# KumarRobotics/top_down_renderer

Hardware: AMD Instinct MI355X
Metric: particle-updates/sec (render+score+resample) (higher is better)
Workload: dtype f32

## Files before the change

include/tdr.h:

```cpp
#ifndef TDR_H_
#define TDR_H_

#include <stddef.h>
#include <stdint.h>

#ifdef __cplusplus
extern "C" {
#endif

#define TDR_OK 0
#define TDR_ERR_ARG (-1)
#define TDR_ERR_HIP (-2)
#define TDR_ERR_NOMEM (-3)

#define TDR_MAX_CLASSES 15
#define TDR_ST_FIELDS 7
enum { TDR_ST_INIT_X = 0, TDR_ST_INIT_Y = 1, TDR_ST_DX = 2, TDR_ST_DY = 3, TDR_ST_THETA = 4, TDR_ST_SCALE = 5,
       TDR_ST_HAVE_INIT = 6 };

typedef struct tdr_state {
  float init_x_px, init_y_px, dx_m, dy_m, theta, scale;
  uint8_t have_init;
  uint8_t pad_[3];
} tdr_state;
// ... 106 lines not shown
                          const int32_t* perm, float uniform_scale, int init_search, float* raw_w, float* workspace,
                          void* stream);

size_t tdr_score_cart_workspace_floats(int ncls, int rows, int cols, int64_t n, int64_t n_total);
int tdr_k_score_cart(const tdr_map_desc* map, const float* scan_pk, int rows, int cols, float res,
                     const tdr_filter_params* fp, float* st, int64_t cap, int64_t n, int64_t n_total,
                     const int32_t* perm, float* raw_w, float* workspace, void* stream);
size_t tdr_score_cart_init_workspace_floats(int ncls, int rows, int cols, int64_t n, int64_t n_total);
int tdr_k_score_cart_init(const tdr_map_desc* map, const float* scan_pk, int rows, int cols, float res,
                          const tdr_filter_params* fp, float* st, int64_t cap, int64_t n, int64_t n_total,
                          float* workspace, void* stream);

int tdr_k_propagate(float* st, int64_t cap, int64_t n, float* last_dist, float tx, float ty, float omega,
                    int scale_freeze, float pos_cov, float theta_cov, const float* z4, uint64_t seed, uint64_t step,
                    int64_t index_base, void* stream);
void* tdr_rng_create(uint32_t seed);
void tdr_rng_destroy(void* rng);
float tdr_rng_uniform_host(void* rng);
int tdr_propagate_normals_host(void* rng, int64_t n, int scale_freeze, float* z4_out);
#define TDR_RNG_STATE_WORDS 640
size_t tdr_rng_dev_workspace_bytes(int64_t n);
int tdr_k_rng_propagate_normals(uint32_t* state, int64_t n, int64_t lo, int64_t hi, int scale_freeze, float* z4_out,
                                void* workspace, void* stream);
int tdr_k_rng_uniform(uint32_t* state, float* out_dev, void* stream);
int tdr_rng_get_state_host(void* rng, uint32_t* words);
int tdr_rng_set_state_host(void* rng, const uint32_t* words);
typedef struct tdr_rng_pipe tdr_rng_pipe;
int tdr_rng_pipe_create(int64_t n_max, tdr_rng_pipe** out);
void tdr_rng_pipe_destroy(tdr_rng_pipe* p);
int tdr_rng_pipe_on_device(const tdr_rng_pipe* p);
int tdr_rng_pipe_from_host(tdr_rng_pipe* p, void* host_rng, void* stream);
int tdr_rng_pipe_to_host(tdr_rng_pipe* p, void* host_rng, void* stream);
int tdr_rng_pipe_normals(tdr_rng_pipe* p, int64_t n, int64_t lo, int64_t hi, int scale_freeze, const float** z4_out,
                         void* stream);
int tdr_rng_pipe_uniform(tdr_rng_pipe* p, const float** shift_out, void* stream);
int tdr_init_particle_host(void* rng, const float* class_maps, int ncls, int rows, int cols, float resolution,
                           const tdr_filter_params* fp, tdr_state* out);
int tdr_init_particles_host(void* rng, const float* class_maps, int ncls, int rows, int cols, float resolution,
                            const tdr_filter_params* fp, int max_num, tdr_state* out, int64_t* n_out);
int64_t tdr_init_particles_count(const tdr_filter_params* fp, int max_num);
size_t tdr_init_workspace_bytes(void);
int tdr_k_init_particles(uint32_t* rng_state_dev, const tdr_map_desc* map, const tdr_filter_params* fp, int max_num,
                         int64_t lo, int64_t hi, float* st, int64_t cap, int64_t* n_out, void* workspace, void* stream);
int tdr_rng_pipe_init_particles(tdr_rng_pipe* p, const tdr_map_desc* map, const tdr_filter_params* fp, int max_num,
                                int64_t lo, int64_t hi, float* st, int64_t cap, int64_t* n_out, void* workspace,
                                void* stream);

#define TDR_UW_INFO_FLOATS 65536
int tdr_k_update_weights(const float* raw_w, const float* last_dist, int64_t n, float* w_out, float* info_out,
                         void* stream);

int tdr_config_prefix_small(int on);
int64_t tdr_prefix_workspace_bytes(int64_t n);
int tdr_k_prefix(const float* w, int64_t n, float* runmax_out, void* workspace, void* stream);
int tdr_k_prefix_mode(const float* w, int64_t n, int mode, float* runmax_out, float* prefix_out, void* workspace,
                      void* stream);
int tdr_k_resample(const float* runmax, int64_t n, int64_t n_new, float shift, int64_t i_begin, int64_t i_end,
                   int32_t* idx_out, void* stream);
int tdr_k_resample_dev(const float* runmax, int64_t n, int64_t n_new, const float* shift_dev, int64_t i_begin, int64_t i_end,
                       int32_t* idx_out, void* stream);
int tdr_k_gather_states(const float* src, int64_t src_cap, int64_t src_shard, const int32_t* idx, int64_t n_new,
                        float* dst, int64_t dst_cap, void* stream);

int tdr_k_shard_pack2(const float* a, const float* b, int64_t nl, float* out, void* stream);
int tdr_k_shard_unpack2(const float* in, int world, int64_t nl, float* a_glob, float* b_glob, void* stream);
int tdr_k_unshard_states(const float* in, int world, int64_t nl, float* st, int64_t cap, void* stream);

int tdr_k_local_map_polar(const tdr_map_desc* map, const float* tab, int nb, int nr, float cx, float cy, float scale,
                          float res, float* dists_out, uint8_t* mask_out, void* stream);
int tdr_k_local_map_cart(const tdr_map_desc* map, int rows, int cols, float cx, float cy, float rot, float res,
                         float* dists_out, uint8_t* mask_out, void* stream);

int tdr_k_active_diffs(const tdr_map_desc* map, const float* tab, int nb, int nr, float res, const float* centres,
                       const int32_t* shifts, int K, int ncand, double* sums_out, void* stream);
int tdr_active_candidates_host(const float* preds, int K, int nb, float* centres, float* dists, float* thetas,
                               int32_t* shifts, int* ntheta_out, int* ndist_out);

#define TDR_MEAN_COV_FLOATS 4800
int tdr_k_mean_cov(const float* st, int64_t cap, int64_t n, const float* about, float* out, void* stream);
int tdr_k_set_scale(float* st, int64_t cap, int64_t n, const float* scale_dev, void* stream);
int tdr_k_save_ml_state(const float* info, const float* st, int64_t cap, int64_t src_shard, int64_t n, float* out12,
                        void* stream);
int tdr_k_shift_init(float* st, int64_t cap, int64_t n, float dx, float dy, void* stream);

int tdr_config_compact(int on);
int tdr_config_shift_uniform(int mode);
float tdr_config_shift_uniform_span(float cells);
int tdr_config_ray_split(int k);
int tdr_config_cart_skip(int on);
int tdr_config_init_mfma(int on);
int tdr_config_uw_waves(int on);
int64_t tdr_shift_uniform_launches(void);

int tdr_profile_enable(int on);
int tdr_profile_score_ms(double* total_ms, int64_t* launches);
int tdr_profile_shares(double* dense_ms, double* scattered_ms, int64_t* scattered_particles);
int tdr_profile_variants(int64_t out[16]);

int64_t tdr_config_tuning(const char* name, int64_t value);
int tdr_su_tail_plan(int nchunks, int k, int q, int row, int* group, int* s0, int* s1);
size_t tdr_k_su_order_workspace_ints(int64_t n, int nb);
int64_t tdr_k_su_order_slots(int64_t n, int nb);
int tdr_k_su_order(const float* st, int64_t cap, int64_t n, const int32_t* perm, int nb, float span, int32_t* workspace,
                   int32_t* slots_out, int32_t* keys_out, int32_t* counts_out, int* bucket_out, void* stream);
int tdr_selftest_score(void);
int tdr_k_selftest_round(const float* x, int64_t n, float limit, int32_t* out, void* stream);
int tdr_libm_variant(void);
int tdr_libm_force_variant(int variant);
int tdr_sincosf_host(const float* x, int64_t n, int variant, float* sin_out, float* cos_out);
int tdr_k_selftest_sincos(const float* x, int64_t n, float* sin_out, float* cos_out, void* stream);
int tdr_logf_host(const float* x, int64_t n, float* out);
int tdr_k_selftest_logf(const float* x, int64_t n, float* out, void* stream);
int tdr_k_selftest_atan2(const float* y, const float* x, int64_t n, float* out, void* stream);

int tdr_k_states_aos_to_soa(const tdr_state* aos, int64_t n, float* st, int64_t cap, void* stream);
int tdr_k_states_soa_to_aos(const float* st, int64_t cap, int64_t n, tdr_state* aos, void* stream);
size_t tdr_locality_tmp_ints(int64_t n, int map_rows, int map_cols);
int tdr_k_locality_order(const float* st, int64_t cap, int64_t n, int map_rows, int map_cols, int32_t* perm_out,
                         int32_t* keys_tmp, void* stream);
size_t tdr_locality_pose_tmp_ints(int64_t n);
int tdr_k_locality_order_pose(const float* st, int64_t cap, int64_t n, int map_rows, int map_cols, float theta_radius,
                              int32_t* perm_out, int32_t* keys_tmp, void* stream);

typedef struct tdr_map tdr_map;
typedef struct tdr_renderer tdr_renderer;
typedef struct tdr_filter tdr_filter;

int tdr_map_create(tdr_map** out);
void tdr_map_destroy(tdr_map* m);
int tdr_map_set(tdr_map* m, const float* class_maps, const uint8_t* class_mask, int ncls, int rows, int cols,
                float resolution, int center_x, int center_y);
int tdr_map_set_labels(tdr_map* m, const uint8_t* label_img, int img_h, int img_w, const int32_t* flatten_lut,
                       int lut_size, int ncls, float resolution, int center_x, int center_y);
int tdr_map_update_labels_incremental(tdr_map* m, const uint8_t* label_img, int img_h, int img_w,
                                      const int32_t* flatten_lut, int lut_size, int ncls, float resolution, int center_x,
                                      int center_y, int64_t* changed_cells);
int tdr_map_patch_labels(tdr_map* m, const uint8_t* patch, int y0, int x0, int h, int w, int center_x, int center_y,
                         int64_t* changed_cells);
int tdr_map_get_desc(const tdr_map* m, tdr_map_desc* out);
int tdr_map_sample_pts_polar(tdr_map* m, int nb, int nr, float ang_res);
int tdr_map_polar_shape(const tdr_map* m, int* nb, int* nr);
int tdr_map_set_window(tdr_map* m, int rows, int cols);
int tdr_map_window_shape(const tdr_map* m, int* rows, int* cols);
int tdr_map_info(const tdr_map* m, int* ncls, int* rows, int* cols, float* resolution, int* have_map);
int tdr_map_center(const tdr_map* m, int* center_x, int* center_y);
int tdr_map_local_map(tdr_map* m, int polar, float cx, float cy, float scale_or_rot, float res, int rows, int cols,
                      float* dists_out, uint8_t* mask_out);
int tdr_map_classes_at_point(const tdr_map* m, int px, int py, uint32_t* class_bits);
int tdr_map_best_rel_pos(tdr_map* m, const float* preds, int K, float best_rel_pos[2], float* best_diff);
int tdr_map_local_geo_map(tdr_map* m, int polar, float cx, float cy, float scale_or_rot, float res, int rows, int cols,
                          float* dists_out);
int tdr_map_load_cache(tdr_map* m, const char* cache_dir, const char* map_path, int num_classes, float resolution,
                       int center_x, int center_y, int* loaded);
int tdr_map_save_cache(tdr_map* m, const char* cache_dir, const char* map_path);
int tdr_map_save_rasters(tdr_map* m, const char* dir);
int tdr_png_read_gray8_host(const char* path, uint8_t* px_out, int64_t capacity, int* w, int* h);
int tdr_png_write_gray8_host(const char* path, const uint8_t* px, int w, int h);
int tdr_map_load_rasters(tdr_map* m, const char* dir, int num_classes, float resolution, int center_x, int center_y);
#define TDR_SVG_NO_KEY 0xFFFFFFFFu
int tdr_svg_parse_host(const char* path, float size_out[2], int64_t* n_poly, int64_t* n_vert, uint32_t* keys_out,
                       int64_t* offsets_out, float* verts_out);
int tdr_map_load_polygons(tdr_map* m, const float* verts, const int64_t* poly_offsets, const int32_t* poly_class,
                          int64_t n_poly, int width, int height, int num_classes, const int32_t* exclusive, int n_excl,
                          float resolution, int center_x, int center_y, uint8_t* planes_out);
int tdr_polygon_planes(const float* verts, const int64_t* poly_offsets, const int32_t* poly_class, int64_t n_poly,
                       int width, int height, int num_classes, const int32_t* exclusive, int n_excl, float resolution,
// ... 153 lines not shown
```

top_down_renderer_amd/_lib.py:

```python
import ctypes as C
import os

_PKG = os.path.dirname(os.path.abspath(__file__))
SO_PATH = os.environ.get("TDR_LIB_PATH") or os.path.join(_PKG, "libtdr_hip.so")

TDR_ST_FIELDS = 7
TDR_MAX_CLASSES = 15
TDR_SVG_NO_KEY = 0xFFFFFFFF


class FilterParamsC(C.Structure):
    _fields_ = [
        ("pos_cov", C.c_float), ("theta_cov", C.c_float), ("regularization", C.c_float),
        ("init_pos_px_x", C.c_float), ("init_pos_px_y", C.c_float), ("init_pos_px_cov", C.c_float),
        ("init_pos_m_x", C.c_float), ("init_pos_m_y", C.c_float),
        ("init_pos_deg_theta", C.c_float), ("init_pos_deg_cov", C.c_float),
        ("force_on_map", C.c_int32),
        ("fixed_scale", C.c_float), ("scale_log_min", C.c_float), ("scale_log_max", C.c_float),
        ("num_classes", C.c_int32),
        ("class_weights", C.c_float * 16),
    ]


class MapDescC(C.Structure):
# ... 99 lines not shown
    "tdr_score_workspace_floats": (C.c_size_t, [_i, _i, _i, _i64, _i64]),
    "tdr_k_score_polar": (_i, [C.POINTER(MapDescC), _vp, _vp, _i, _i, _f, C.POINTER(FilterParamsC), _vp, _i64, _i64,
                               _i64, _vp, _f, _i, _vp, _vp, _vp]),
    "tdr_k_active_diffs": (_i, [C.POINTER(MapDescC), _vp, _i, _i, _f, _vp, _vp, _i, _i, _vp, _vp]),
    "tdr_active_candidates_host": (_i, [_vp, _i, _i, _vp, _vp, _vp, _vp, C.POINTER(_i), C.POINTER(_i)]),
    "tdr_logf_host": (_i, [_vp, _i64, _vp]),
    "tdr_k_selftest_logf": (_i, [_vp, _i64, _vp, _vp]),
    "tdr_rng_pipe_create": (_i, [_i64, C.POINTER(_vp)]),
    "tdr_rng_pipe_destroy": (None, [_vp]),
    "tdr_rng_pipe_on_device": (_i, [_vp]),
    "tdr_rng_pipe_from_host": (_i, [_vp, _vp, _vp]),
    "tdr_rng_pipe_to_host": (_i, [_vp, _vp, _vp]),
    "tdr_rng_pipe_normals": (_i, [_vp, _i64, _i64, _i64, _i, C.POINTER(_vp), _vp]),
    "tdr_rng_pipe_uniform": (_i, [_vp, C.POINTER(_vp), _vp]),
    "tdr_rng_dev_workspace_bytes": (C.c_size_t, [_i64]),
    "tdr_k_rng_propagate_normals": (_i, [_vp, _i64, _i64, _i64, _i, _vp, _vp, _vp]),
    "tdr_k_rng_uniform": (_i, [_vp, _vp, _vp]),
    "tdr_rng_get_state_host": (_i, [_vp, _vp]),
    "tdr_rng_set_state_host": (_i, [_vp, _vp]),
    "tdr_k_resample_dev": (_i, [_vp, _i64, _i64, _vp, _i64, _i64, _vp, _vp]),
    "tdr_score_ctx_create": (_i, [C.POINTER(_vp)]),
    "tdr_score_ctx_destroy": (None, [_vp]),
    "tdr_score_ctx_span": (C.c_float, [_vp]),
    "tdr_score_ctx_trial_calls": (_i64, [_vp]),
    "tdr_config_tuning": (_i64, [C.c_char_p, _i64]),
    "tdr_su_tail_plan": (_i, [_i, _i, _i, _i, C.POINTER(_i), C.POINTER(_i), C.POINTER(_i)]),
    "tdr_k_su_order_workspace_ints": (C.c_size_t, [_i64, _i]),
    "tdr_k_su_order_slots": (_i64, [_i64, _i]),
    "tdr_k_su_order": (_i, [_vp, _i64, _i64, _vp, _i, _f, _vp, _vp, _vp, _vp, C.POINTER(_i), _vp]),
    "tdr_selftest_score": (_i, []),
    "tdr_profile_variants": (_i, [C.POINTER(_i64)]),
    "tdr_score_ctx_set_polar_factors": (_i, [_vp, _vp, _i, _i]),
    "tdr_polar_factors_host": (_i, [_i, _i, _f, _f, _vp]),
    "tdr_k_score_polar_ctx": (_i, [C.POINTER(MapDescC), _vp, _vp, _i, _i, _f, C.POINTER(FilterParamsC), _vp, _i64, _i64,
                                   _i64, _vp, _f, _i, _vp, _vp, _vp, _vp]),
    "tdr_score_geo_workspace_floats": (C.c_size_t, [_i, _i, _i, _i64, _i64]),
    "tdr_k_score_polar_geo": (_i, [C.POINTER(MapDescC), C.POINTER(MapDescC), _vp, _vp, _vp, _f, _f, _i, _i, _f,
                                   C.POINTER(FilterParamsC), _vp, _i64, _i64, _i64, _vp, _f, _i, _vp, _vp, _vp]),
    "tdr_score_cart_workspace_floats": (C.c_size_t, [_i, _i, _i, _i64, _i64]),
    "tdr_k_score_cart": (_i, [C.POINTER(MapDescC), _vp, _i, _i, _f, C.POINTER(FilterParamsC), _vp, _i64, _i64, _i64,
                              _vp, _vp, _vp, _vp]),
    "tdr_score_cart_init_workspace_floats": (C.c_size_t, [_i, _i, _i, _i64, _i64]),
    "tdr_k_score_cart_init": (_i, [C.POINTER(MapDescC), _vp, _i, _i, _f, C.POINTER(FilterParamsC), _vp, _i64, _i64, _i64,
                                   _vp, _vp]),
    "tdr_k_propagate": (_i, [_vp, _i64, _i64, _vp, _f, _f, _f, _i, _f, _f, _vp, _u64, _u64, _i64, _vp]),
    "tdr_rng_create": (_vp, [_u32]),
    "tdr_rng_destroy": (None, [_vp]),
    "tdr_rng_uniform_host": (_f, [_vp]),
    "tdr_propagate_normals_host": (_i, [_vp, _i64, _i, _vp]),
    "tdr_k_update_weights": (_i, [_vp, _vp, _i64, _vp, _vp, _vp]),
    "tdr_prefix_workspace_bytes": (_i64, [_i64]),
    "tdr_k_prefix": (_i, [_vp, _i64, _vp, _vp, _vp]),
    "tdr_k_prefix_mode": (_i, [_vp, _i64, _i, _vp, _vp, _vp, _vp]),
    "tdr_k_resample": (_i, [_vp, _i64, _i64, _f, _i64, _i64, _vp, _vp]),
    "tdr_k_gather_states": (_i, [_vp, _i64, _i64, _vp, _i64, _vp, _i64, _vp]),
    "tdr_init_particles_host": (_i, [_vp, _vp, _i, _i, _i, _f, C.POINTER(FilterParamsC), _i, _vp, C.POINTER(C.c_int64)]),
    "tdr_init_particles_count": (_i64, [C.POINTER(FilterParamsC), _i]),
    "tdr_init_workspace_bytes": (C.c_size_t, []),
    "tdr_k_init_particles": (_i, [_vp, C.POINTER(MapDescC), C.POINTER(FilterParamsC), _i, _i64, _i64, _vp, _i64,
                                  C.POINTER(C.c_int64), _vp, _vp]),
    "tdr_rng_pipe_init_particles": (_i, [_vp, C.POINTER(MapDescC), C.POINTER(FilterParamsC), _i, _i64, _i64, _vp, _i64,
                                         C.POINTER(C.c_int64), _vp, _vp]),
    "tdr_k_mean_cov": (_i, [_vp, _i64, _i64, _vp, _vp, _vp]),
    "tdr_k_sample_ml_states": (_i, [_vp, _i64, _i64, _i, _vp, _vp]),
    "tdr_gmm_fit_host": (_i, [_vp, _i, _i, _i, _vp, _vp, _vp, _vp]),
    "tdr_gmm_select_host": (_i, [_vp, _i, _i64, _vp, _i, _vp, _vp]),
    "tdr_adaptive_count_host": (_i64, [_vp, _i, _i64, _i64]),
    "tdr_filter_compute_gmm": (_i, [_vp]),
    "tdr_filter_get_gmm": (_i, [_vp, _i, _vp, _vp, _vp]),
    "tdr_filter_adaptive_count": (_i64, [_vp]),
    "tdr_filter_step_count": (_i64, [_vp]),
    "tdr_filter_num_gaussians": (_i, [_vp]),
    "tdr_filter_set_num_gaussians": (_i, [_vp, _i]),
    "tdr_gmm_workspace_bytes": (C.c_size_t, [_i, _i]),
    "tdr_gmm_out_doubles": (_i, [_i]),
    "tdr_k_gmm_samples": (_i, [_vp, _i, _vp, _vp]),
    "tdr_k_gmm_fit": (_i, [_vp, _i, _i, _i, _vp, _vp, _vp]),
    "tdr_k_gmm_fit_jobs": (_i, [_vp, _i, _vp]),
    "tdr_k_gmm_pick": (_i, [_vp, _i, _vp]),
    "tdr_gmm_candidates_host": (_i, [_i, _i64, _i, _i, _vp]),
    "tdr_filter_compute_gmm_device": (_i, [_vp]),
    "tdr_batch_compute_gmm": (_i, [_vp, _i, _vp]),
    "tdr_k_save_ml_state": (_i, [_vp, _vp, _i64, _i64, _i64, _vp, _vp]),
    "tdr_k_shard_pack2": (_i, [_vp, _vp, _i64, _vp, _vp]),
    "tdr_k_shard_unpack2": (_i, [_vp, _i, _i64, _vp, _vp, _vp]),
    "tdr_k_unshard_states": (_i, [_vp, _i, _i64, _vp, _i64, _vp]),
    "tdr_comm_rccl_unique_id": (_i, [_vp]),
    "tdr_comm_create_rccl": (_i, [_i, _i, _vp, C.POINTER(_vp)]),
    "tdr_comm_create": (_i, [_i, _i, _vp, C.POINTER(_vp)]),
    "tdr_comm_destroy": (None, [_vp]),
    "tdr_comm_world": (_i, [_vp]),
    "tdr_comm_rank": (_i, [_vp]),
    "tdr_comm_all_gather": (_i, [_vp, _vp, _vp, C.c_size_t, _vp]),
    "tdr_comm_broadcast": (_i, [_vp, _vp, C.c_size_t, _i, _vp]),
    "tdr_filter_create_sharded": (_i, [_vp, _i, C.POINTER(FilterParamsC), _u32, _vp, C.POINTER(_vp)]),
    "tdr_filter_num_local": (_i64, [_vp]),
    "tdr_k_set_scale": (_i, [_vp, _i64, _i64, _vp, _vp]),
    "tdr_k_shift_init": (_i, [_vp, _i64, _i64, _f, _f, _vp]),
    "tdr_k_states_aos_to_soa": (_i, [_vp, _i64, _vp, _i64, _vp]),
    "tdr_k_states_soa_to_aos": (_i, [_vp, _i64, _i64, _vp, _vp]),
    "tdr_profile_enable": (_i, [_i]),
    "tdr_profile_score_ms": (_i, [C.POINTER(C.c_double), C.POINTER(C.c_int64)]),
    "tdr_profile_shares": (_i, [C.POINTER(C.c_double), C.POINTER(C.c_double), C.POINTER(C.c_int64)]),
    "tdr_map_create": (_i, [C.POINTER(_vp)]),
    "tdr_map_destroy": (None, [_vp]),
    "tdr_map_set": (_i, [_vp, _vp, _vp, _i, _i, _i, _f, _i, _i]),
    "tdr_map_set_labels": (_i, [_vp, _vp, _i, _i, _vp, _i, _i, _f, _i, _i]),
    "tdr_filter_update_map_labels": (_i, [_vp, _vp, _i, _i, _vp, _i, _i, _f, _i, _i]),
    "tdr_map_update_labels_incremental": (_i, [_vp, _vp, _i, _i, _vp, _i, _i, _f, _i, _i, C.POINTER(_i64)]),
    "tdr_map_patch_labels": (_i, [_vp, _vp, _i, _i, _i, _i, _i, _i, C.POINTER(_i64)]),
    "tdr_map_get_desc": (_i, [_vp, C.POINTER(MapDescC)]),
    "tdr_filter_update_map_labels_incremental": (_i, [_vp, _vp, _i, _i, _vp, _i, _i, _f, _i, _i, C.POINTER(_i64)]),
    "tdr_filter_patch_map_labels": (_i, [_vp, _vp, _i, _i, _i, _i, _i, _i, C.POINTER(_i64)]),
    "tdr_map_sample_pts_polar": (_i, [_vp, _i, _i, _f]),
    "tdr_map_polar_shape": (_i, [_vp, C.POINTER(_i), C.POINTER(_i)]),
    "tdr_map_set_window": (_i, [_vp, _i, _i]),
    "tdr_map_window_shape": (_i, [_vp, C.POINTER(_i), C.POINTER(_i)]),
    "tdr_map_info": (_i, [_vp, C.POINTER(_i), C.POINTER(_i), C.POINTER(_i), C.POINTER(_f), C.POINTER(_i)]),
    "tdr_map_center": (_i, [_vp, _vp, _vp]),
    "tdr_map_local_map": (_i, [_vp, _i, _f, _f, _f, _f, _i, _i, _vp, _vp]),
    "tdr_k_local_map_polar": (_i, [_vp, _vp, _i, _i, _f, _f, _f, _f, _vp, _vp, _vp]),
    "tdr_k_local_map_cart": (_i, [_vp, _i, _i, _f, _f, _f, _f, _vp, _vp, _vp]),
    "tdr_map_local_geo_map": (_i, [_vp, _i, _f, _f, _f, _f, _i, _i, _vp]),
    "tdr_map_load_cache": (_i, [_vp, C.c_char_p, C.c_char_p, _i, _f, _i, _i, C.POINTER(_i)]),
    "tdr_map_save_cache": (_i, [_vp, C.c_char_p, C.c_char_p]),
    "tdr_k_geo_map_from_map": (_i, [C.POINTER(MapDescC), _i, _vp, _vp, _vp]),
    "tdr_map_classes_at_point": (_i, [_vp, _i, _i, C.POINTER(_u32)]),
    "tdr_map_best_rel_pos": (_i, [_vp, _vp, _i, _vp, _vp]),
    "tdr_renderer_create": (_i, [_vp, C.POINTER(_vp)]),
    "tdr_renderer_destroy": (None, [_vp]),
    "tdr_renderer_render": (_i, [_vp, _i, _vp, _i, _i, _i64, _f, _f, _i, _i, _i, _vp]),
    "tdr_renderer_render_geo": (_i, [_vp, _i, _vp, _i, _i64, _i64, _f, _f, _i, _i, _vp]),
    "tdr_filter_create": (_i, [_vp, _i, C.POINTER(FilterParamsC), _u32, C.POINTER(_vp)]),
    "tdr_filter_create_cart": (_i, [_vp, _i, C.POINTER(FilterParamsC), _u32, C.POINTER(_vp)]),
    "tdr_filter_destroy": (None, [_vp]),
    "tdr_filter_configure": (_i, [_vp, _i, _i]),
    "tdr_filter_initialize_particles": (_i, [_vp]),
    "tdr_filter_set_states": (_i, [_vp, _vp, _i64]),
    "tdr_filter_get_states": (_i, [_vp, _vp, _i64]),
    "tdr_filter_propagate": (_i, [_vp, _f, _f, _f]),
    "tdr_filter_update": (_i, [_vp, _vp, _vp, _f, _i64]),
    "tdr_filter_update_geo": (_i, [_vp, _vp, _vp, _f, _i64]),
    "tdr_filter_compute_weights": (_i, [_vp, _vp, _vp, _f]),
    "tdr_filter_get_raw_weights": (_i, [_vp, _vp, _i64]),
    "tdr_filter_get_last_dist": (_i, [_vp, _vp, _i64]),
    "tdr_filter_propagate_freeze": (_i, [_vp, _f, _f, _f, _i]),
    "tdr_filter_init_one": (_i, [_vp]),
    "tdr_filter_share_rng": (_i, [_vp, _vp]),
    "tdr_init_particle_host": (_i, [_vp, _vp, _i, _i, _i, _f, _vp, _vp]),
    "tdr_filter_get_weights": (_i, [_vp, _vp, _i64]),
    "tdr_filter_get_resample_indices": (_i, [_vp, _vp, _i64]),
    "tdr_filter_mean_cov": (_i, [_vp, _i, _vp, _vp]),
    "tdr_filter_freeze_scale": (_i, [_vp]),
    "tdr_filter_is_scale_frozen": (_i, [_vp]),
    "tdr_filter_scale": (_f, [_vp]),
    "tdr_filter_num_particles": (_i64, [_vp]),
    "tdr_filter_update_map": (_i, [_vp, _vp, _vp, _i, _i, _i, _f, _i, _i]),
    "tdr_batch_step": (_i, [_vp, _i, _vp, _vp]),
    "tdr_batch_last_stats": (_i, [_vp, _vp]),
    "tdr_batch_render_polar": (_i, [_vp, _i, _vp, _f, _i, _i, _i, _vp]),
    "tdr_renderer_get_render": (_i, [_vp, _vp, _vp]),
    "tdr_batch_pose": (_i, [_vp, _i, _vp, _vp]),
    "tdr_viz_plane_words": (C.c_size_t, [_i, _i]),
    "tdr_viz_arrow_host": (_i, [_i, _i, _vp]),
    "tdr_viz_overlay_host": (_i, [_vp, _vp, _i, _vp, _vp, _i, _i, _vp, _i, C.POINTER(_i)]),
    "tdr_k_viz_particles": (_i, [_vp, _i64, _i64, _i, _i, _vp, _vp]),
# ... 39 lines not shown
```

top_down_renderer_amd/csrc/tdr_batch_loop.hip:

```cpp
#include "tdr_common.h"
#include "tdr_raster_dev.h"
#include "tdr_filter_dev.h"
#include "tdr_batch.h"

__global__ __launch_bounds__(256) void batch_raster_keys_kernel(const TdrBatchRasterEntry* __restrict__ tab, int k,
                                                                TdrBatchRasterShape a) {
  const TdrBatchRasterEntry& e = tab[batch_find(k, (int)blockIdx.x, [&](int i) { return tab[i].blk_keys; })];
  const int64_t q = (int64_t)(blockIdx.x - e.blk_keys) * blockDim.x + threadIdx.x;
  if (q >= e.n) return;
  e.keys[q] = raster_key(e.pts, e.stride, e.ioff, q, 1, e.res, a.ang_res, e.lut, a.ncls, a.rows, a.cols);
}

__global__ __launch_bounds__(1024) void batch_raster_kernel(const TdrBatchRasterEntry* __restrict__ tab,
                                                            TdrBatchRasterShape a) {
  extern __shared__ unsigned int cnt[];
  const TdrBatchRasterEntry& e = tab[blockIdx.y];
  const int col0 = blockIdx.x * a.cpt;
  const int ncol = min(a.cpt, a.cols - col0);
  raster_tile_clear(cnt, ncol * a.ncls * a.rows);
  __syncthreads();
  raster_tile_count_keys(cnt, e.keys, e.n, col0, ncol, a.ncls, a.rows);
  __syncthreads();
  raster_tile_write(cnt, col0, ncol, a.ncls, a.rows, a.cols, a.rf, e.img, e.pk);
}

bool tdr_batch_raster_shape(int ncls, int rows, int cols, float ang_res, TdrBatchRasterShape* out) {
  RasterShape sh;
  if (ncls < 1 || ncls > TDR_MAX_CLASSES || rows < 1 || cols < 1 || !raster_shape(ncls, rows, cols, &sh) || !sh.keyed)
    return false;
  TdrBatchRasterShape a;
  a.ang_res = ang_res; a.ncls = ncls; a.rows = rows; a.cols = cols; a.rf = tdr_rec_floats(ncls); a.cpt = sh.cpt;
  *out = a;
  return true;
}

int tdr_batch_raster(const TdrBatchRasterEntry* tab, int k, int blocks_keys, const TdrBatchRasterShape& a, hipStream_t s) {
  if (!tab || k < 1 || blocks_keys < 0) return fail(TDR_ERR_ARG, "batch_raster: bad arguments");
  const size_t lds = (size_t)a.cpt * a.ncls * a.rows * 4;
  static bool attr_set[64] = {false};
  HIP_TRY(raster_allow_lds(reinterpret_cast<const void*>(batch_raster_kernel), lds, attr_set));
  if (blocks_keys > 0)
    hipLaunchKernelGGL(batch_raster_keys_kernel, dim3((unsigned)blocks_keys), dim3(256), 0, s, tab, k, a);
  hipLaunchKernelGGL(batch_raster_kernel, dim3((unsigned)cdiv(a.cols, a.cpt), (unsigned)k), dim3(1024), lds, s, tab, a);
  LAUNCH_CHECK("batch_raster");
  return TDR_OK;
}

static_assert(TDR_BATCH_MC_SINGLE_MAX_N == MC_SINGLE_MAX_N, "the batch splits small / big filters where tdr_k_mean_cov does");

__global__ __launch_bounds__(1024) void batch_mean_cov_kernel(const TdrBatchPoseEntry* __restrict__ tab, int libm_fma) {
  const TdrBatchPoseEntry& e = tab[blockIdx.x];
  mean_cov_body(e.st, e.cap, e.n, nullptr, e.out, libm_fma);
  if (threadIdx.x == 0) e.out[24] = e.st[TDR_ST_SCALE * e.cap];
}
__global__ __launch_bounds__(MC_THREADS) void batch_mc_sums_kernel(const TdrBatchPoseEntry* __restrict__ tab, int libm_fma) {
  const TdrBatchPoseEntry& e = tab[blockIdx.y];
  mc_sums_body(e.st, e.cap, e.n, reinterpret_cast<McScratch*>(e.scratch), libm_fma);
}
__global__ __launch_bounds__(MC_THREADS) void batch_mc_cov_kernel(const TdrBatchPoseEntry* __restrict__ tab) {
  const TdrBatchPoseEntry& e = tab[blockIdx.y];
  mc_cov_body(e.st, e.cap, e.n, nullptr, reinterpret_cast<McScratch*>(e.scratch));
}
__global__ __launch_bounds__(MC_THREADS) void batch_mc_final_kernel(const TdrBatchPoseEntry* __restrict__ tab) {
  const TdrBatchPoseEntry& e = tab[blockIdx.x];
  mc_final_body(e.n, nullptr, reinterpret_cast<const McScratch*>(e.scratch), e.out);
  if (threadIdx.x == 0) e.out[24] = e.st[TDR_ST_SCALE * e.cap];
}

int tdr_batch_pose_launch(const TdrBatchPoseEntry* small, int k_small, const TdrBatchPoseEntry* big, int k_big,
                          hipStream_t s) {
  if (k_small < 0 || k_big < 0 || (k_small && !small) || (k_big && !big)) return fail(TDR_ERR_ARG, "batch_pose: bad arguments");
  const int fma = tdr_libm_fma();
  if (k_small > 0)
    hipLaunchKernelGGL(batch_mean_cov_kernel, dim3((unsigned)k_small), dim3(1024), 0, s, small, fma);
  if (k_big > 0) {
    hipLaunchKernelGGL(batch_mc_sums_kernel, dim3(MC_WGS, (unsigned)k_big), dim3(MC_THREADS), 0, s, big, fma);
    hipLaunchKernelGGL(batch_mc_cov_kernel, dim3(MC_WGS, (unsigned)k_big), dim3(MC_THREADS), 0, s, big);
    hipLaunchKernelGGL(batch_mc_final_kernel, dim3((unsigned)k_big), dim3(MC_THREADS), 0, s, big);
  }
  LAUNCH_CHECK("batch_pose");
  return TDR_OK;
}
```

top_down_renderer_amd/csrc/tdr_common.h:

```cpp
#ifndef TDR_COMMON_H_
#define TDR_COMMON_H_
#include <hip/hip_runtime.h>

#include <cmath>
#include <cstdarg>
#include <cstdint>
#include <cstdio>
#include <cstdlib>
#include <cstring>
#include <limits>
#include <type_traits>
#include <utility>
#include <vector>

#include "tdr.h"
#include "tdr_config.h"

#ifndef TDR_SCORE_U
#define TDR_SCORE_U 4
#endif
#ifndef TDR_INIT_SCAN_LDS
#define TDR_INIT_SCAN_LDS 1
#endif
#ifndef TDR_XCD_SWIZZLE
#define TDR_XCD_SWIZZLE 0
#endif
#ifndef TDR_OOB_ALIAS
#define TDR_OOB_ALIAS 1
#endif

int tdr_fail(int code, const char* fmt, ...);
#define fail tdr_fail
#define HIP_TRY(expr)                                                                       \
  do {                                                                                      \
    hipError_t e_ = (expr);                                                                 \
    if (e_ != hipSuccess) return fail(TDR_ERR_HIP, "%s: %s", #expr, hipGetErrorString(e_)); \
  } while (0)
#define LAUNCH_CHECK(name)                                                                   \
  do {                                                                                       \
    hipError_t e_ = hipGetLastError();                                                       \
    if (e_ != hipSuccess) return fail(TDR_ERR_HIP, "launch %s: %s", name, hipGetErrorString(e_)); \
  } while (0)

int tdr_libm_fma();

static inline int64_t cdiv(int64_t a, int64_t b) { return (a + b - 1) / b; }

template <class F>
static inline int with_flags(F&& f) { return f(); }
template <class F, class... Rest>
static inline int with_flags(F&& f, bool b, Rest... rest) {
  auto next = [&](auto B) { return with_flags([&](auto... bs) { return f(B, bs...); }, rest...); };
  return b ? next(std::true_type{}) : next(std::false_type{});
}
template <class F>
static inline int with_nv4(int rf, const char* who, F&& f) {
  switch (rf / 4) {
    case 1: return f(std::integral_constant<int, 1>{});
    case 2: return f(std::integral_constant<int, 2>{});
    case 3: return f(std::integral_constant<int, 3>{});
    case 4: return f(std::integral_constant<int, 4>{});
    default: return fail(TDR_ERR_ARG, "%s: unsupported record size %d", who, rf);
  }
}

#define PFX_HEAD 2048
#define INI_TILE 2048
#define INI_MAX_TILES 2048
int tdr_chain_total(const float* raw, const float* mean_dev, int kind, int64_t n, float* total_out, void* workspace,
                    hipStream_t st);
int tdr_uw_small(const float* raw, const float* last_dist, int64_t n, float* w, float* info, hipStream_t st);
int tdr_mt_raw_stream(const uint32_t* state, int64_t nblocks, uint32_t* raw, hipStream_t s);
int tdr_mt_advance(const uint32_t* raw, int64_t nblocks, const uint32_t* consumed, uint32_t* state, hipStream_t s);
bool tdr_score_polar_float_form(const tdr_map_desc* map, int nb, int nr, int64_t n, int64_t n_total);
__host__ __device__ inline bool tdr_has_kslot(int ncls, int rf) { return ncls + 2 <= rf; }
uint32_t* tdr_profile_stats_ptr();
#endif
```

top_down_renderer_amd/csrc/tdr_filter.hip:

```cpp
#include <random>

#include <rocprim/device/device_radix_sort.hpp>
using TdrSortConfig = rocprim::radix_sort_config<rocprim::default_config, rocprim::merge_sort_config<512, 512, 4>, rocprim::default_config>;

#include "tdr_common.h"
#include "tdr_filter_dev.h"

__device__ __forceinline__ uint32_t mulhi32(uint32_t a, uint32_t b) { return __umulhi(a, b); }
__device__ void philox4x32_10(uint32_t c[4], uint32_t k0, uint32_t k1) {
#pragma unroll
  for (int r = 0; r < 10; r++) {
    uint32_t hi0 = mulhi32(0xD2511F53u, c[0]), lo0 = 0xD2511F53u * c[0];
    uint32_t hi1 = mulhi32(0xCD9E8D57u, c[2]), lo1 = 0xCD9E8D57u * c[2];
    uint32_t n0 = hi1 ^ c[1] ^ k0, n1 = lo1, n2 = hi0 ^ c[3] ^ k1, n3 = lo0;
    c[0] = n0; c[1] = n1; c[2] = n2; c[3] = n3;
    k0 += 0x9E3779B9u; k1 += 0xBB67AE85u;
  }
}

__global__ void propagate_kernel(float* __restrict__ st, int64_t cap, int64_t n, float* __restrict__ last_dist,
                                 float tx, float ty, float omega, int scale_freeze, float pos_cov, float theta_cov,
                                 const float* __restrict__ z4, uint64_t seed, uint64_t step, int64_t index_base,
                                 int libm_fma) {
  const int64_t p = (int64_t)blockIdx.x * blockDim.x + threadIdx.x;
// ... 81 lines not shown
    st.theta = (float)((double)st.theta * (M_PI / 180));
    st.have_init = 1;
  } else {
    st.theta = 0;
    st.have_init = 0;
  }
  return st;
}
extern "C" int tdr_init_particle_host(void* rng, const float* class_maps, int ncls, int rows, int cols, float resolution,
                                      const tdr_filter_params* fp, tdr_state* out) {
  if (!rng || !class_maps || !fp || !out) return fail(TDR_ERR_ARG, "init_particle: bad arguments");
  if (ncls < 2) return fail(TDR_ERR_ARG, "init_particle: class 1 (road) is required for the on-road test");
  bool any_road = false;
  for (size_t k = 0; k < (size_t)rows * cols && !any_road; k++) any_road = class_maps[(size_t)rows * cols + k] < 1;
  if (!any_road) return fail(TDR_ERR_ARG, "init_particle: the map has no road cell, rejection sampling cannot end");
  *out = draw_particle(*(std::mt19937*)rng, class_maps, ncls, rows, cols, resolution, fp);
  return TDR_OK;
}
extern "C" int tdr_init_particles_host(void* rng, const float* class_maps, int ncls, int rows, int cols,
                                       float resolution, const tdr_filter_params* fp, int max_num, tdr_state* out,
                                       int64_t* n_out) {
  if (!rng || !class_maps || !fp || !out || !n_out || max_num < 0) return fail(TDR_ERR_ARG, "init_particles: bad arguments");
  if (ncls < 2) return fail(TDR_ERR_ARG, "init_particles: class 1 (road) is required for the on-road test");
  std::mt19937& gen = *(std::mt19937*)rng;
  bool any_road = false;
  for (size_t k = 0; k < (size_t)rows * cols && !any_road; k++) any_road = class_maps[(size_t)rows * cols + k] < 1;
  if (!any_road) return fail(TDR_ERR_ARG, "init_particles: the map has no road cell, rejection sampling cannot end");
  const size_t num_at_scale = (fp->fixed_scale < 0) ? 10 : 1;
  int64_t count = 0;
  for (int i = 0; i < (int)((size_t)max_num / num_at_scale); i++) {
    const tdr_state proto = draw_particle(gen, class_maps, ncls, rows, cols, resolution, fp);
    for (float scale = 0; scale < 1; scale += 1. / num_at_scale) {
      tdr_state part = draw_particle(gen, class_maps, ncls, rows, cols, resolution, fp);
      if (fp->fixed_scale < 0) {
        part = proto;
        part.scale = (float)std::pow(10., (double)scale);
      }
      if (count < max_num + 16) out[count] = part;
      count++;
      (void)draw_particle(gen, class_maps, ncls, rows, cols, resolution, fp);
    }
  }
  *n_out = count;
  return TDR_OK;
}

__device__ long long block_sum_ll(long long v, long long* sh) {
  const int lane = threadIdx.x & 63, wave = threadIdx.x >> 6;
  for (int o = 32; o > 0; o >>= 1) v += __shfl_down(v, o, 64);
  __syncthreads();
  if (lane == 0) sh[wave] = v;
  __syncthreads();
  long long t = 0;
  const int nw = blockDim.x >> 6;
  for (int w = 0; w < nw; w++) t += sh[w];
  return t;
}

#define UW_G 256
struct UwScratch {
  double a[UW_G];
  double b[UW_G];
};
__device__ __forceinline__ void uw_chunk(int64_t n, int64_t& lo, int64_t& hi) {
  const int64_t per = (n + UW_G - 1) / UW_G;
  lo = (int64_t)blockIdx.x * per;
  hi = lo + per < n ? lo + per : n;
  if (lo > n) lo = n;
}
__device__ double uw_total(const double* part) {
  __shared__ double stage[UW_G];
  __shared__ double result;
  __syncthreads();
  for (int g = threadIdx.x; g < UW_G; g += blockDim.x) stage[g] = part[g];
  __syncthreads();
  if (threadIdx.x == 0) {
    double t = 0;
    for (int g = 0; g < UW_G; g++) t += stage[g];
    result = t;
  }
  __syncthreads();
  return result;
}
__global__ __launch_bounds__(256) void uw_pass1(const float* __restrict__ raw, int64_t n, UwScratch* s1) {
  __shared__ double shd[4];
  __shared__ long long shl[4];
  int64_t lo, hi;
  uw_chunk(n, lo, hi);
  double s = 0;
  long long c = 0;
  for (int64_t i = lo + threadIdx.x; i < hi; i += 256) {
    const float v = raw[i];
    if (!isnan(v)) { s += (double)v; c++; }
  }
  const double ts = block_sum_d(s, shd);
  const long long tc = block_sum_ll(c, shl);
  if (threadIdx.x == 0) { s1->a[blockIdx.x] = ts; s1->b[blockIdx.x] = (double)tc; }
}
struct UwExact {
  float sum, mean, bsum, pad;
};
__global__ __launch_bounds__(256) void uw_pass2(const float* __restrict__ raw, int64_t n, const UwScratch* s1,
                                                UwScratch* s2, UwExact* ex) {
  __shared__ long long shl[4];
  const float mean = ex->sum / (float)(long long)uw_total(s1->b);
  int64_t lo, hi;
  uw_chunk(n, lo, hi);
  long long cu = 0;
  for (int64_t i = lo + threadIdx.x; i < hi; i += 256) {
    const float v = raw[i];
    if (!isnan(v) && v < mean) cu++;
  }
  const long long tc = block_sum_ll(cu, shl);
  if (threadIdx.x == 0) {
    s2->b[blockIdx.x] = (double)tc;
    if (blockIdx.x == 0) ex->mean = mean;
  }
}
__global__ __launch_bounds__(256) void uw_pass3(const float* __restrict__ raw, int64_t n, const UwExact* ex,
                                                const UwScratch* s2, UwScratch* s3, float* __restrict__ w) {
  __shared__ double shd[4];
  const float sum = ex->sum, mean = ex->mean;
  const long long num_under = (long long)uw_total(s2->b);
  const float bottom = sqrtf(ex->bsum / (float)num_under);
  const bool fallback = (sum == 0.f || num_under < 1);
  const float fill = mean - bottom;
  int64_t lo, hi;
  uw_chunk(n, lo, hi);
  double acc = 0;
  for (int64_t i = lo + threadIdx.x; i < hi; i += 256) {
    float v = raw[i];
    v = fallback ? 1.f : (isnan(v) ? fill : v);
    w[i] = v;
    acc += (double)v;
  }
  const double t = block_sum_d(acc, shd);
  if (threadIdx.x == 0) s3->a[blockIdx.x] = t;
}
__global__ __launch_bounds__(256) void uw_pass4(const float* __restrict__ last_dist, int64_t n, const UwScratch* s3,
                                                UwScratch* s4, float* __restrict__ w) {
  __shared__ double shd[4];
  const float fs1 = (float)uw_total(s3->a);
  const float fn = (float)n;
  int64_t lo, hi;
  uw_chunk(n, lo, hi);
  double acc = 0;
  for (int64_t i = lo + threadIdx.x; i < hi; i += 256) {
    float v = w[i] / fs1;
    const float d = fminf(last_dist[i] * 5.f, 1.f);
    v = d * v + (1.f - d) / fn;
    w[i] = v;
    acc += (double)v;
  }
  const double t = block_sum_d(acc, shd);
  if (threadIdx.x == 0) s4->a[blockIdx.x] = t;
}
__global__ __launch_bounds__(256) void uw_pass5(int64_t n, const UwScratch* s4, UwScratch* s5, float* __restrict__ w) {
  __shared__ float sb[4];
  __shared__ long long si[4];
  const float fs2 = (float)uw_total(s4->a);
  int64_t lo, hi;
  uw_chunk(n, lo, hi);
  float best = -INFINITY;
  long long besti = 0x7fffffffffffffffll;
  for (int64_t i = lo + threadIdx.x; i < hi; i += 256) {
    const float v = w[i] / fs2;
    w[i] = v;
    if (v > best || (v == best && i < besti)) { best = v; besti = i; }
  }
  for (int o = 32; o > 0; o >>= 1) {
    const float ob = __shfl_down(best, o, 64);
    const long long oi = __shfl_down(besti, o, 64);
    if (ob > best || (ob == best && oi < besti)) { best = ob; besti = oi; }
  }
  if ((threadIdx.x & 63) == 0) { sb[threadIdx.x >> 6] = best; si[threadIdx.x >> 6] = besti; }
  __syncthreads();
  if (threadIdx.x == 0) {
    for (int k = 1; k < 4; k++)
      if (sb[k] > best || (sb[k] == best && si[k] < besti)) { best = sb[k]; besti = si[k]; }
    s5->a[blockIdx.x] = (double)best;
    s5->b[blockIdx.x] = (double)besti;
  }
}
__global__ __launch_bounds__(256) void uw_pass6(int64_t n, const UwScratch* s1, const UwScratch* s2,
                                                const UwScratch* s5, const UwExact* ex, float* info) {
  static_assert(UW_G == 256, "one candidate per thread");
  __shared__ float sb[4];
  __shared__ long long si[4];
  float best = (float)s5->a[threadIdx.x];
  long long besti = (long long)s5->b[threadIdx.x];
  if (best != best) { best = -INFINITY; besti = 0x7fffffffffffffffll; }
  for (int o = 32; o > 0; o >>= 1) {
    const float ob = __shfl_down(best, o, 64);
    const long long oi = __shfl_down(besti, o, 64);
    if (ob > best || (ob == best && oi < besti)) { best = ob; besti = oi; }
  }
  if ((threadIdx.x & 63) == 0) { sb[threadIdx.x >> 6] = best; si[threadIdx.x >> 6] = besti; }
  const float sum = ex->sum, mean = ex->mean;
  const long long nv = (long long)uw_total(s1->b), nu = (long long)uw_total(s2->b);
  const float bottom = sqrtf(ex->bsum / (float)nu);
  if (threadIdx.x != 0) return;
  for (int k = 1; k < 4; k++)
    if (sb[k] > best || (sb[k] == best && si[k] < besti)) { best = sb[k]; besti = si[k]; }
  if (besti == 0x7fffffffffffffffll) besti = 0;
  info[0] = __int_as_float((int)besti);
  info[1] = sum; info[2] = mean; info[3] = bottom; info[4] = (sum == 0.f || nu < 1) ? 1.f : 0.f;
  info[5] = (float)nv; info[6] = (float)nu; info[7] = 0.f;
}

#define TDR_UW_SINGLE_MAX_N 32768
extern "C" int tdr_k_update_weights(const float* raw_w, const float* last_dist, int64_t n, float* w_out,
                                    float* info_out, void* stream) {
  if (!raw_w || !last_dist || !w_out || !info_out) return fail(TDR_ERR_ARG, "update_weights: null pointer");
  if (n < 1) return fail(TDR_ERR_ARG, "update_weights: n must be >= 1");
  hipStream_t s = (hipStream_t)stream;
  if (n <= TDR_UW_SINGLE_MAX_N) {
    const int rc = tdr_uw_small(raw_w, last_dist, n, w_out, info_out, s);
    if (rc) return rc;
    LAUNCH_CHECK("update_weights");
    return TDR_OK;
  }
  constexpr size_t kFixed = 8 * sizeof(float) + 64 + 5 * sizeof(UwScratch) + sizeof(UwExact) + 64;
  static_assert(kFixed + 32 * 1024 <= TDR_UW_INFO_FLOATS * sizeof(float), "info scratch");
  UwScratch* sc = reinterpret_cast<UwScratch*>(
      (reinterpret_cast<uintptr_t>(info_out + 8) + 63) & ~(uintptr_t)63);
  UwExact* ex = reinterpret_cast<UwExact*>(sc + 5);
  void* chain_ws = reinterpret_cast<void*>((reinterpret_cast<uintptr_t>(ex + 1) + 63) & ~(uintptr_t)63);
  const size_t chain_room = TDR_UW_INFO_FLOATS * sizeof(float) - kFixed;
  if ((size_t)tdr_prefix_workspace_bytes(n) > chain_room)
    return fail(TDR_ERR_ARG, "update_weights: n = %lld needs more than TDR_UW_INFO_FLOATS of scratch", (long long)n);
  hipLaunchKernelGGL(uw_pass1, dim3(UW_G), dim3(256), 0, s, raw_w, n, sc + 0);
  int rc = tdr_chain_total(raw_w, nullptr, 0, n, &ex->sum, chain_ws, s);
  if (rc) return rc;
  hipLaunchKernelGGL(uw_pass2, dim3(UW_G), dim3(256), 0, s, raw_w, n, (const UwScratch*)(sc + 0), sc + 1, ex);
  rc = tdr_chain_total(raw_w, &ex->mean, 1, n, &ex->bsum, chain_ws, s);
  if (rc) return rc;
  hipLaunchKernelGGL(uw_pass3, dim3(UW_G), dim3(256), 0, s, raw_w, n, (const UwExact*)ex, (const UwScratch*)(sc + 1),
                     sc + 2, w_out);
  hipLaunchKernelGGL(uw_pass4, dim3(UW_G), dim3(256), 0, s, last_dist, n, (const UwScratch*)(sc + 2), sc + 3, w_out);
  hipLaunchKernelGGL(uw_pass5, dim3(UW_G), dim3(256), 0, s, n, (const UwScratch*)(sc + 3), sc + 4, w_out);
  hipLaunchKernelGGL(uw_pass6, dim3(1), dim3(256), 0, s, n, (const UwScratch*)(sc + 0), (const UwScratch*)(sc + 1),
                     (const UwScratch*)(sc + 4), (const UwExact*)ex, info_out);
  LAUNCH_CHECK("update_weights(multi)");
  return TDR_OK;
}

__global__ void resample_kernel(const float* __restrict__ runmax, int64_t n, int64_t n_new, float shift,
                                int64_t i_begin, int64_t i_end, int32_t* __restrict__ idx) {
  const int64_t i = i_begin + (int64_t)blockIdx.x * blockDim.x + threadIdx.x;
  if (i >= i_end) return;
  idx[i - i_begin] = (int32_t)resample_pick(runmax, n, n_new, i, shift);
}

extern "C" int tdr_k_resample(const float* runmax, int64_t n, int64_t n_new, float shift, int64_t i_begin,
                              int64_t i_end, int32_t* idx_out, void* stream) {
  if (!runmax || !idx_out) return fail(TDR_ERR_ARG, "resample: null pointer");
  if (n < 1 || n_new < 1 || i_begin < 0 || i_end > n_new || i_begin > i_end)
    return fail(TDR_ERR_ARG, "resample: bad range");
  if (i_begin == i_end) return TDR_OK;
  hipLaunchKernelGGL(resample_kernel, dim3((unsigned)cdiv(i_end - i_begin, 256)), dim3(256), 0, (hipStream_t)stream,
                     runmax, n, n_new, shift, i_begin, i_end, idx_out);
  LAUNCH_CHECK("resample");
  return TDR_OK;
}

__global__ void resample_dev_kernel(const float* __restrict__ runmax, int64_t n, int64_t n_new, const float* __restrict__ shift_dev,
                                    int64_t i_begin, int64_t i_end, int32_t* __restrict__ idx) {
  const int64_t i = i_begin + (int64_t)blockIdx.x * blockDim.x + threadIdx.x;
  if (i >= i_end) return;
  idx[i - i_begin] = (int32_t)resample_pick(runmax, n, n_new, i, *shift_dev);
}
extern "C" int tdr_k_resample_dev(const float* runmax, int64_t n, int64_t n_new, const float* shift_dev, int64_t i_begin,
                                  int64_t i_end, int32_t* idx_out, void* stream) {
  if (!runmax || !idx_out || !shift_dev) return fail(TDR_ERR_ARG, "resample: null pointer");
  if (n < 1 || n_new < 1 || i_begin < 0 || i_end > n_new || i_begin > i_end)
    return fail(TDR_ERR_ARG, "resample: bad range");
  if (i_begin == i_end) return TDR_OK;
  hipLaunchKernelGGL(resample_dev_kernel, dim3((unsigned)cdiv(i_end - i_begin, 256)), dim3(256), 0, (hipStream_t)stream,
                     runmax, n, n_new, shift_dev, i_begin, i_end, idx_out);
  LAUNCH_CHECK("resample");
  return TDR_OK;
}

__global__ void gather_states_kernel(const float* __restrict__ src, int64_t src_cap, int64_t src_shard,
                                     const int32_t* __restrict__ idx, int64_t n_new, float* __restrict__ dst,
                                     int64_t dst_cap) {
  const int64_t i = (int64_t)blockIdx.x * blockDim.x + threadIdx.x;
  if (i >= n_new) return;
  const int64_t j = idx[i];
  if (src_shard > 0) {
    const int64_t r = j / src_shard, l = j - r * src_shard;
#pragma unroll
    for (int f = 0; f < TDR_ST_FIELDS; f++) dst[f * dst_cap + i] = src[(r * TDR_ST_FIELDS + f) * src_shard + l];
  } else {
    gather_particle(src, src_cap, j, dst, dst_cap, i);
  }
}

extern "C" int tdr_k_gather_states(const float* src, int64_t src_cap, int64_t src_shard, const int32_t* idx,
                                   int64_t n_new, float* dst, int64_t dst_cap, void* stream) {
  if (!src || !idx || !dst) return fail(TDR_ERR_ARG, "gather_states: null pointer");
  if (n_new < 0 || dst_cap < n_new || src_shard < 0) return fail(TDR_ERR_ARG, "gather_states: n_new exceeds capacity");
  if (n_new == 0) return TDR_OK;
  hipLaunchKernelGGL(gather_states_kernel, dim3((unsigned)cdiv(n_new, 256)), dim3(256), 0, (hipStream_t)stream, src,
                     src_cap, src_shard, idx, n_new, dst, dst_cap);
  LAUNCH_CHECK("gather_states");
  return TDR_OK;
}

__device__ __forceinline__ McScratch* mc_scratch(float* out) { return reinterpret_cast<McScratch*>(out + 24); }
__global__ __launch_bounds__(1024) void mean_cov_kernel(const float* __restrict__ st, int64_t cap, int64_t n,
                                                       const float* __restrict__ about, float* __restrict__ out,
                                                       int libm_fma) {
  mean_cov_body(st, cap, n, about, out, libm_fma);
}
__global__ __launch_bounds__(MC_THREADS) void mc_sums_kernel(const float* __restrict__ st, int64_t cap, int64_t n,
                                                             float* __restrict__ out, int libm_fma) {
  mc_sums_body(st, cap, n, mc_scratch(out), libm_fma);
}
__global__ __launch_bounds__(MC_THREADS) void mc_cov_kernel(const float* __restrict__ st, int64_t cap, int64_t n,
                                                            const float* __restrict__ about, float* __restrict__ out) {
  mc_cov_body(st, cap, n, about, mc_scratch(out));
}
__global__ __launch_bounds__(MC_THREADS) void mc_final_kernel(int64_t n, const float* __restrict__ about,
                                                              float* __restrict__ out) {
  mc_final_body(n, about, mc_scratch(out), out);
}

extern "C" int tdr_k_mean_cov(const float* st, int64_t cap, int64_t n, const float* about, float* out, void* stream) {
  if (!st || !out || n < 1 || cap < n) return fail(TDR_ERR_ARG, "mean_cov: bad arguments");
  hipStream_t s = (hipStream_t)stream;
  if (n <= MC_SINGLE_MAX_N) {
    hipLaunchKernelGGL(mean_cov_kernel, dim3(1), dim3(1024), 0, s, st, cap, n, about, out, tdr_libm_fma());
  } else {
    hipLaunchKernelGGL(mc_sums_kernel, dim3(MC_WGS), dim3(MC_THREADS), 0, s, st, cap, n, out, tdr_libm_fma());
    hipLaunchKernelGGL(mc_cov_kernel, dim3(MC_WGS), dim3(MC_THREADS), 0, s, st, cap, n, about, out);
    hipLaunchKernelGGL(mc_final_kernel, dim3(1), dim3(MC_THREADS), 0, s, n, about, out);
  }
  LAUNCH_CHECK("mean_cov");
  return TDR_OK;
}

__global__ void set_scale_kernel(float* __restrict__ st, int64_t cap, int64_t n, const float* __restrict__ scale) {
  const int64_t p = (int64_t)blockIdx.x * blockDim.x + threadIdx.x;
  if (p < n) st[TDR_ST_SCALE * cap + p] = *scale;
}
extern "C" int tdr_k_set_scale(float* st, int64_t cap, int64_t n, const float* scale_dev, void* stream) {
  if (!st || !scale_dev || n < 0 || cap < n) return fail(TDR_ERR_ARG, "set_scale: bad arguments");
  if (n == 0) return TDR_OK;
  hipLaunchKernelGGL(set_scale_kernel, dim3((unsigned)cdiv(n, 256)), dim3(256), 0, (hipStream_t)stream, st, cap, n,
                     scale_dev);
  LAUNCH_CHECK("set_scale");
  return TDR_OK;
}

__global__ void shift_init_kernel(float* __restrict__ st, int64_t cap, int64_t n, float dx, float dy) {
  const int64_t p = (int64_t)blockIdx.x * blockDim.x + threadIdx.x;
  if (p < n) {
    st[TDR_ST_INIT_X * cap + p] += dx;
    st[TDR_ST_INIT_Y * cap + p] += dy;
  }
}
extern "C" int tdr_k_shift_init(float* st, int64_t cap, int64_t n, float dx, float dy, void* stream) {
  if (!st || n < 0 || cap < n) return fail(TDR_ERR_ARG, "shift_init: bad arguments");
  if (n == 0) return TDR_OK;
  hipLaunchKernelGGL(shift_init_kernel, dim3((unsigned)cdiv(n, 256)), dim3(256), 0, (hipStream_t)stream, st, cap, n,
                     dx, dy);
  LAUNCH_CHECK("shift_init");
  return TDR_OK;
}

__global__ void save_ml_state_kernel(const float* __restrict__ info, const float* __restrict__ st, int64_t cap,
                                     int64_t src_shard, int64_t n, float* __restrict__ out) {
  if (threadIdx.x != 0 || blockIdx.x != 0) return;
  const int64_t best = ml_index(info, n);
  float f[TDR_ST_FIELDS];
  if (src_shard > 0) {
    const int64_t r = best / src_shard, l = best - r * src_shard;
#pragma unroll
    for (int k = 0; k < TDR_ST_FIELDS; k++) f[k] = st[(r * TDR_ST_FIELDS + k) * src_shard + l];
  } else {
#pragma unroll
    for (int k = 0; k < TDR_ST_FIELDS; k++) f[k] = st[(int64_t)k * cap + best];
  }
  ml_record(f, out);
}
extern "C" int tdr_k_save_ml_state(const float* info, const float* st, int64_t cap, int64_t src_shard, int64_t n,
                                   float* out12, void* stream) {
  if (!info || !st || !out12 || n < 1 || src_shard < 0 || (src_shard == 0 && cap < n))
    return fail(TDR_ERR_ARG, "save_ml_state: bad arguments");
  hipLaunchKernelGGL(save_ml_state_kernel, dim3(1), dim3(64), 0, (hipStream_t)stream, info, st, cap, src_shard, n,
                     out12);
  LAUNCH_CHECK("save_ml_state");
  return TDR_OK;
}

__global__ void sample_ml_states_kernel(const float* __restrict__ st, int64_t cap, int64_t n, int num,
                                        float* __restrict__ out) {
  const int i = blockIdx.x * blockDim.x + threadIdx.x;
  if (i >= num) return;
  sample_ml_state(st, cap, n, num, i, out + 3 * i);
}
extern "C" int tdr_k_sample_ml_states(const float* st, int64_t cap, int64_t n, int num, float* out, void* stream) {
  if (!st || !out || n < 1 || cap < n || num < 1) return fail(TDR_ERR_ARG, "sample_ml_states: bad arguments");
  hipLaunchKernelGGL(sample_ml_states_kernel, dim3((unsigned)cdiv(num, 256)), dim3(256), 0, (hipStream_t)stream, st,
                     cap, n, num, out);
  LAUNCH_CHECK("sample_ml_states");
  return TDR_OK;
}

__global__ void shard_pack2_kernel(const float* __restrict__ a, const float* __restrict__ b, int64_t nl,
                                   float* __restrict__ out) {
  const int64_t i = (int64_t)blockIdx.x * blockDim.x + threadIdx.x;
  if (i < nl) { out[i] = a[i]; out[nl + i] = b[i]; }
}
__global__ void shard_unpack2_kernel(const float* __restrict__ in, int world, int64_t nl, float* __restrict__ a,
                                     float* __restrict__ b) {
  const int64_t g = (int64_t)blockIdx.x * blockDim.x + threadIdx.x;
  if (g >= (int64_t)world * nl) return;
  const int64_t r = g / nl, l = g - r * nl;
  a[g] = in[(2 * r) * nl + l];
  b[g] = in[(2 * r + 1) * nl + l];
}
__global__ void unshard_states_kernel(const float* __restrict__ in, int world, int64_t nl, float* __restrict__ st,
                                      int64_t cap) {
  const int64_t g = (int64_t)blockIdx.x * blockDim.x + threadIdx.x;
  if (g >= (int64_t)world * nl) return;
  const int64_t r = g / nl, l = g - r * nl;
#pragma unroll
  for (int f = 0; f < TDR_ST_FIELDS; f++) st[f * cap + g] = in[(r * TDR_ST_FIELDS + f) * nl + l];
}
extern "C" int tdr_k_shard_pack2(const float* a, const float* b, int64_t nl, float* out, void* stream) {
  if (!a || !b || !out || nl < 0) return fail(TDR_ERR_ARG, "shard_pack2: bad arguments");
  if (nl == 0) return TDR_OK;
  hipLaunchKernelGGL(shard_pack2_kernel, dim3((unsigned)cdiv(nl, 256)), dim3(256), 0, (hipStream_t)stream, a, b, nl, out);
  LAUNCH_CHECK("shard_pack2");
  return TDR_OK;
}
extern "C" int tdr_k_shard_unpack2(const float* in, int world, int64_t nl, float* a_glob, float* b_glob, void* stream) {
  if (!in || !a_glob || !b_glob || world < 1 || nl < 0) return fail(TDR_ERR_ARG, "shard_unpack2: bad arguments");
  if (nl == 0) return TDR_OK;
  hipLaunchKernelGGL(shard_unpack2_kernel, dim3((unsigned)cdiv((int64_t)world * nl, 256)), dim3(256), 0,
                     (hipStream_t)stream, in, world, nl, a_glob, b_glob);
  LAUNCH_CHECK("shard_unpack2");
  return TDR_OK;
}
extern "C" int tdr_k_unshard_states(const float* in, int world, int64_t nl, float* st, int64_t cap, void* stream) {
  if (!in || !st || world < 1 || nl < 0 || cap < (int64_t)world * nl) return fail(TDR_ERR_ARG, "unshard_states: bad arguments");
  if (nl == 0) return TDR_OK;
  hipLaunchKernelGGL(unshard_states_kernel, dim3((unsigned)cdiv((int64_t)world * nl, 256)), dim3(256), 0,
                     (hipStream_t)stream, in, world, nl, st, cap);
  LAUNCH_CHECK("unshard_states");
  return TDR_OK;
}

__global__ void aos_to_soa_kernel(const tdr_state* __restrict__ aos, int64_t n, float* __restrict__ st, int64_t cap) {
  const int64_t p = (int64_t)blockIdx.x * blockDim.x + threadIdx.x;
  if (p >= n) return;
  const tdr_state s = aos[p];
  st[TDR_ST_INIT_X * cap + p] = s.init_x_px;
  st[TDR_ST_INIT_Y * cap + p] = s.init_y_px;
  st[TDR_ST_DX * cap + p] = s.dx_m;
  st[TDR_ST_DY * cap + p] = s.dy_m;
  st[TDR_ST_THETA * cap + p] = s.theta;
  st[TDR_ST_SCALE * cap + p] = s.scale;
  st[TDR_ST_HAVE_INIT * cap + p] = s.have_init ? 1.f : 0.f;
}
__global__ void soa_to_aos_kernel(const float* __restrict__ st, int64_t cap, int64_t n, tdr_state* __restrict__ aos) {
  const int64_t p = (int64_t)blockIdx.x * blockDim.x + threadIdx.x;
  if (p >= n) return;
  tdr_state s;
  s.init_x_px = st[TDR_ST_INIT_X * cap + p];
  s.init_y_px = st[TDR_ST_INIT_Y * cap + p];
  s.dx_m = st[TDR_ST_DX * cap + p];
  s.dy_m = st[TDR_ST_DY * cap + p];
  s.theta = st[TDR_ST_THETA * cap + p];
// ... 140 lines not shown
```

top_down_renderer_amd/csrc/tdr_host.cpp:

```cpp
#include <sys/stat.h>
#include <cerrno>
#include <hip/hip_runtime.h>

#include <algorithm>
#include <cmath>
#include <cstdarg>
#include <cstdio>
#include <cstring>
#include <limits>
#include <string>
#include <vector>

#include "tdr.h"
#include "tdr_batch.h"
#include "tdr_config.h"
#include "tdr_gmm_dev.h"

bool tdr_score_polar_float_form(const tdr_map_desc* map, int nb, int nr, int64_t n, int64_t n_total);

extern "C" int tdr_set_error(int code, const char* msg);

namespace {

int failh(int code, const char* fmt, ...) {
// ... 1318 lines not shown
static int map_rec16_end(tdr_map* m, hipStream_t s) {
  if (!m->rec16_used) HTRY(hipEventCreateWithFlags(&m->rec16_used, hipEventDisableTiming));
  HTRY(hipEventRecord(m->rec16_used, s));
  return TDR_OK;
}
static int filter_score(tdr_filter* f, const float* scan_imgs, const tdr_renderer* renderer, float res) {
  tdr_map* m = f->map;
  if (!f->cart && (m->nb < 1 || !m->tab.p)) return failh(TDR_ERR_ARG, "filter_update: samplePtsPolar was never called");
  if (f->cart && (m->win_rows < 1 || m->win_cols < 1)) return failh(TDR_ERR_ARG, "filter_update: the map has no window");
  f->fp.num_classes = m->desc.ncls;
  const int ncls = m->desc.ncls, nb = f->cart ? m->win_rows : m->nb, nr = f->cart ? m->win_cols : m->nr;
  const size_t P = (size_t)nb * nr;
  const size_t pk_floats = P * tdr_rec_floats(ncls);
  const float* pk = nullptr;
  if (scan_imgs) {
    TTRY(f->scan_img.resize(P * ncls));
    TTRY(f->scan_pk.resize(pk_floats));
    HTRY(hipMemcpyAsync(f->scan_img.p, scan_imgs, P * ncls * sizeof(float), hipMemcpyHostToDevice, f->stream));
    TTRY(tdr_k_pack_scan(f->scan_img.p, ncls, nb, nr, f->scan_pk.p, f->stream));
    pk = f->scan_pk.p;
  } else if (renderer) {
    if (!renderer->have_scan) return failh(TDR_ERR_ARG, "filter_update: no scan");
    if (renderer->ncls != ncls || renderer->rows != nb || renderer->cols != nr)
      return failh(TDR_ERR_ARG, "filter_update: render shape %dx%dx%d does not match the map's %dx%dx%d",
                   renderer->ncls, renderer->rows, renderer->cols, ncls, nb, nr);
    if (f->cart && renderer->polar) return failh(TDR_ERR_ARG, "filter_update: a Cartesian filter needs a Cartesian render");
    pk = renderer->pk.p;
    TTRY(renderer_wait_render(renderer, f->stream));
  } else if (!(f->comm && f->rank != 0)) {
    return failh(TDR_ERR_ARG, "filter_update: no scan");
  }
  if (f->comm) {
    TTRY(f->pk_recv.resize(pk_floats));
    if (f->rank == 0) HTRY(hipMemcpyAsync(f->pk_recv.p, pk, pk_floats * sizeof(float), hipMemcpyDeviceToDevice, f->stream));
    TTRY(tdr_comm_broadcast(f->comm, f->pk_recv.p, pk_floats * sizeof(float), 0, f->stream));
    pk = f->pk_recv.p;
  }
  const int64_t n = f->nl();
  const int32_t* perm = nullptr;
  if (f->cart) {
    f->states_changed();
    if (f->maybe_uninit) {
      TTRY(f->init_ws.resize(tdr_score_cart_init_workspace_floats(ncls, nb, nr, n, f->n)));
      TTRY(tdr_k_score_cart_init(&m->desc, pk, nb, nr, res, &f->fp, f->st.p, f->cap, n, f->n, f->init_ws.p, f->stream));
      f->maybe_uninit = false;
    }
    if (f->locality_every > 0) {
      TTRY(f->loc_tmp.resize(tdr_locality_pose_tmp_ints(n) + 2));
      TTRY(tdr_k_locality_order_pose(f->st.p, f->cap, n, m->desc.rows, m->desc.cols, (float)(nb + nr) / 16.f, f->perm.p,
                                     f->loc_tmp.p, f->stream));
      perm = f->perm.p;
    }
    TTRY(f->ws.resize(tdr_score_cart_workspace_floats(ncls, nb, nr, n, f->n)));
    TTRY(tdr_k_score_cart(&m->desc, pk, nb, nr, res, &f->fp, f->st.p, f->cap, n, f->n, perm, f->raw_w.p, f->ws.p, f->stream));
    if (renderer && !scan_imgs) TTRY(renderer_note_read(renderer, f->stream));
    return TDR_OK;
  }
  if (f->locality_every > 0) {
    TTRY(f->loc_tmp.resize(tdr_locality_tmp_ints(n, m->desc.rows, m->desc.cols)));
    TTRY(tdr_k_locality_order(f->st.p, f->cap, n, m->desc.rows, m->desc.cols, f->perm.p, f->loc_tmp.p, f->stream));
    perm = f->perm.p;
  }
  f->states_changed();
  TTRY(f->ws.resize(tdr_score_workspace_floats(ncls, nb, nr, n, f->n)));
  if (f->maybe_uninit) TTRY(map_rec16_alloc(m, f->n));
  const bool uses_rec16 = f->maybe_uninit && m->desc.rec16 && f->n >= tdr_cfg().rec16_min;
  if (uses_rec16) TTRY(map_rec16_begin(m, f->stream));
  TTRY(tdr_score_ctx_set_polar_factors(f->score_ctx, m->fac.p, nb, nr));
  TTRY(tdr_k_score_polar_ctx(&m->desc, m->tab.p, pk, nb, nr, res, &f->fp, f->st.p, f->cap, n, f->n, perm, f->uniform_scale,
                             f->maybe_uninit ? 1 : 0, f->raw_w.p, f->ws.p, f->score_ctx, f->stream));
  if (uses_rec16) TTRY(map_rec16_end(m, f->stream));
  if (renderer && !scan_imgs) TTRY(renderer_note_read(renderer, f->stream));
  if (f->maybe_uninit && !(f->fp.force_on_map || f->fp.fixed_scale < 0)) f->maybe_uninit = false;
  return TDR_OK;
}
static int filter_resample(tdr_filter* f, int64_t n_target) {
  const int64_t n = f->n, nl = f->nl();
  int64_t n_new = n;
  if (n_target >= 0) n_new = std::max<int64_t>(1, std::min<int64_t>(n_target, f->n_max));
  n_new = std::max<int64_t>(f->world, n_new - n_new % f->world);
  const int64_t nl_new = n_new / f->world, i0 = (int64_t)f->rank * nl_new;
  TTRY(f->ml_dev.resize(12));
  TTRY(tdr_k_prefix(f->w.p, n, f->runmax.p, f->pfx_ws.p, f->stream));
  if (rng_on_device(f)) {
    const float* shift_dev = nullptr;
    TTRY(tdr_rng_pipe_uniform(f->pipe, &shift_dev, f->stream));
    TTRY(tdr_k_resample_dev(f->runmax.p, n, n_new, shift_dev, i0, i0 + nl_new, f->idx.p, f->stream));
  } else {
    const float shift = tdr_rng_uniform_host(f->rng);
    TTRY(tdr_k_resample(f->runmax.p, n, n_new, shift, i0, i0 + nl_new, f->idx.p, f->stream));
  }
  if (f->comm) {
    for (int k = 0; k < TDR_ST_FIELDS; k++)
      HTRY(hipMemcpyAsync(f->st_send.p + (size_t)k * nl, f->st.p + (size_t)k * f->cap, (size_t)nl * sizeof(float),
                          hipMemcpyDeviceToDevice, f->stream));
    TTRY(tdr_comm_all_gather(f->comm, f->st_send.p, f->st_all.p, (size_t)TDR_ST_FIELDS * nl * sizeof(float), f->stream));
    TTRY(tdr_k_gather_states(f->st_all.p, 0, nl, f->idx.p, nl_new, f->st_new.p, f->cap, f->stream));
    TTRY(tdr_k_save_ml_state(f->info.p, f->st_all.p, 0, nl, n, f->ml_dev.p, f->stream));
  } else {
    TTRY(tdr_k_gather_states(f->st.p, f->cap, 0, f->idx.p, n_new, f->st_new.p, f->cap, f->stream));
    TTRY(tdr_k_save_ml_state(f->info.p, f->st.p, f->cap, 0, n, f->ml_dev.p, f->stream));
  }
  f->have_ml = true;
  f->states_changed();
  std::swap(f->st.p, f->st_new.p);
  f->n = n_new;
  f->step++;
  return TDR_OK;
}
static int filter_global_states(tdr_filter* f, const float** st, int64_t* cap) {
  if (!f->comm) {
    *st = f->st.p;
    *cap = f->cap;
    return TDR_OK;
  }
  const int64_t nl = f->nl();
  for (int k = 0; k < TDR_ST_FIELDS; k++)
    HTRY(hipMemcpyAsync(f->st_send.p + (size_t)k * nl, f->st.p + (size_t)k * f->cap, (size_t)nl * sizeof(float),
                        hipMemcpyDeviceToDevice, f->stream));
  TTRY(tdr_comm_all_gather(f->comm, f->st_send.p, f->st_all.p, (size_t)TDR_ST_FIELDS * nl * sizeof(float), f->stream));
  TTRY(tdr_k_unshard_states(f->st_all.p, f->world, nl, f->st_glob.p, f->n_max, f->stream));
  *st = f->st_glob.p;
  *cap = f->n_max;
  return TDR_OK;
}

int tdr_filter_get_weights(tdr_filter* f, float* out, int64_t n) {
  if (!f || !out || n < 0 || n > f->n_max) return failh(TDR_ERR_ARG, "filter_get_weights: bad arguments");
  HTRY(hipMemcpy(out, f->w.p, (size_t)n * sizeof(float), hipMemcpyDeviceToHost));
  return TDR_OK;
}
int tdr_filter_get_resample_indices(tdr_filter* f, int32_t* out, int64_t n) {
  if (!f || !out || n < 0 || n > f->nl()) return failh(TDR_ERR_ARG, "filter_get_resample_indices: bad arguments");
  HTRY(hipMemcpy(out, f->idx.p, (size_t)n * sizeof(int32_t), hipMemcpyDeviceToHost));
  return TDR_OK;
}

int tdr_filter_mean_cov(tdr_filter* f, int about_max, float state[4], float cov[16]) {
  if (!f) return failh(TDR_ERR_ARG, "filter_mean_cov: null filter");
  if (cov) std::memset(cov, 0, 16 * sizeof(float));
  if (state) std::memset(state, 0, 4 * sizeof(float));
  if (f->n < 1) return TDR_OK;
  float out[24];
  const float* gst = nullptr;
  int64_t gcap = 0;
  if (about_max || !f->mean_cov_valid) TTRY(filter_global_states(f, &gst, &gcap));
  if (!about_max) {
    if (!f->mean_cov_valid) {
      TTRY(tdr_k_mean_cov(gst, gcap, f->n, nullptr, f->stats.p, f->stream));
      HTRY(hipMemcpy(f->mean_cov_host, f->stats.p, sizeof(out), hipMemcpyDeviceToHost));
      f->mean_cov_valid = true;
    }
    std::memcpy(out, f->mean_cov_host, sizeof(out));
    if (state) std::memcpy(state, out, 4 * sizeof(float));
  } else {
    float ref[4] = {0, 0, 0, 0};
    if (!f->have_ml) return failh(TDR_ERR_ARG, "filter_mean_cov: no update yet, there is no max-likelihood particle");
    TTRY(tdr_k_mean_cov(gst, gcap, f->n, f->ml_dev.p + 8, f->stats.p, f->stream));
    HTRY(hipMemcpyAsync(out, f->stats.p, sizeof(out), hipMemcpyDeviceToHost, f->stream));
    HTRY(hipMemcpyAsync(ref, f->ml_dev.p + 8, sizeof(ref), hipMemcpyDeviceToHost, f->stream));
    HTRY(hipStreamSynchronize(f->stream));
    if (state) std::memcpy(state, ref, sizeof(ref));
  }
  if (cov) std::memcpy(cov, out + 4, 16 * sizeof(float));
  return TDR_OK;
}

int tdr_filter_freeze_scale(tdr_filter* f) {
  if (!f) return failh(TDR_ERR_ARG, "filter_freeze_scale: null filter");
  if (f->scale_frozen || f->n < 1) return TDR_OK;
  const float* gst = nullptr;
  int64_t gcap = 0;
  TTRY(filter_global_states(f, &gst, &gcap));
  TTRY(tdr_k_mean_cov(gst, gcap, f->n, nullptr, f->stats.p, f->stream));
  f->states_changed();
  TTRY(tdr_k_set_scale(f->st.p, f->cap, f->nl(), f->stats.p + 20, f->stream));
  float gm = 0;
  HTRY(hipMemcpy(&gm, f->stats.p + 20, sizeof(float), hipMemcpyDeviceToHost));
  f->scale_frozen = true;
  f->uniform_scale = gm;
  return TDR_OK;
}
int tdr_filter_is_scale_frozen(const tdr_filter* f) { return f && f->scale_frozen; }
float tdr_filter_scale(tdr_filter* f) {
// ... 856 lines not shown
```

top_down_renderer_amd/csrc/tdr_prefix.hip:

```cpp
#include "tdr_common.h"
#include "tdr_batch.h"

#define TDR_PFX_BLOCK 4096
__global__ __launch_bounds__(64) void prefix_serial_kernel(const float* __restrict__ w, int64_t n,
                                                           float* __restrict__ runmax) {
  __shared__ float4 buf4[TDR_PFX_BLOCK / 4];
  float* buf = reinterpret_cast<float*>(buf4);
  const int lane = threadIdx.x;
  float run = 0.f;
  float carry_max = -INFINITY;
  for (int64_t base = 0; base < n; base += TDR_PFX_BLOCK) {
    const int cnt = (int)min((int64_t)TDR_PFX_BLOCK, n - base);
    for (int t = lane; t < TDR_PFX_BLOCK; t += 64) buf[t] = (t < cnt) ? w[base + t] : 0.f;
    __builtin_amdgcn_s_waitcnt(0);
    __builtin_amdgcn_wave_barrier();
    if (lane == 0) {
      const int q4 = (cnt + 3) / 4;
#pragma unroll 4
      for (int q = 0; q < q4; q++) {
        float4 v = buf4[q];
        run = run + v.x; v.x = run;
        run = run + v.y; v.y = run;
        run = run + v.z; v.z = run;
        run = run + v.w; v.w = run;
// ... 987 lines not shown
    pfx_walk_chunk(w, lo, cnt, runmax, prefix_opt, r, carry, head_len);
  });
}
__global__ __launch_bounds__(PFXM_THREADS) void pfx_chunk_fill_kernel(const float* __restrict__ w, int64_t n,
                                                                      const PfxChunk* __restrict__ ch,
                                                                      float* __restrict__ runmax,
                                                                      float* __restrict__ prefix_opt) {
  __shared__ PfxPair shp[PFXM_THREADS / 64];
  const int c = blockIdx.x;
  const PfxChunk hdr = ch[c];
  if (!hdr.accepted) return;
  const long long lo = (long long)c * PFXM_CHUNK;
  const int cnt = (int)min((long long)PFXM_CHUNK, (long long)n - lo);
  const PfxRunSum a{{w}, CHAIN_RUNSUM, 0.f};
  const int t0 = threadIdx.x * PFXM_K;
  float wv[PFXM_K];
  a.load_items(lo, cnt, t0, wv);
  const ChainWg<PFXM_THREADS, float> sc{shp, nullptr};
  unsigned st[PFXM_K];
  (void)chain_step<false, PfxRunSum>(wv, t0, 0, cnt, hdr.r0, sc, st);
  float val[PFXM_K];
#pragma unroll
  for (int k = 0; k < PFXM_K; k++) val[k] = chain_mant(__float_as_uint(hdr.r0) >> 23, st[k]);
  const float carry = hdr.carry0;
  if (t0 + PFXM_K <= cnt && ((lo & 3) == 0)) {
    float4* o = reinterpret_cast<float4*>(runmax + lo + t0);
#pragma unroll
    for (int k = 0; k < PFXM_K / 4; k++)
      o[k] = make_float4(fmaxf(carry, val[4 * k]), fmaxf(carry, val[4 * k + 1]), fmaxf(carry, val[4 * k + 2]),
                         fmaxf(carry, val[4 * k + 3]));
    if (prefix_opt) {
      float4* q = reinterpret_cast<float4*>(prefix_opt + lo + t0);
#pragma unroll
      for (int k = 0; k < PFXM_K / 4; k++) q[k] = make_float4(val[4 * k], val[4 * k + 1], val[4 * k + 2], val[4 * k + 3]);
    }
  } else {
#pragma unroll
    for (int k = 0; k < PFXM_K; k++)
      if (t0 + k < cnt) {
        runmax[lo + t0 + k] = fmaxf(carry, val[k]);
        if (prefix_opt) prefix_opt[lo + t0 + k] = val[k];
      }
  }
}

struct ChainSrc {
  const float* raw;
  const float* mean;
  int kind;
};
__device__ __forceinline__ ChainStat chain_stat(const ChainSrc& s) { return {{s.raw}, s.kind, s.kind ? *s.mean : 0.f}; }
__global__ __launch_bounds__(PFXW_THREADS) void chain_sum_kernel(ChainSrc s, int64_t n, PfxChunk* __restrict__ ch) {
  chain_sum_body<PFXW_THREADS, CHAIN_K>(chain_stat(s), n, ch);
}
__global__ __launch_bounds__(PFXW_THREADS) void chain_summary_kernel(ChainSrc s, int64_t n, PfxChunk* __restrict__ ch,
                                                                    int c_first) {
  chain_summary_body<PFXW_THREADS, CHAIN_K>(chain_stat(s), n, ch, c_first);
}
template <class A>
__device__ __forceinline__ void chain_walk_chunk(const A& a, long long lo, int cnt, float& r, int pos) {
  __shared__ PfxPair shp[PFXW_THREADS / 64];
  __shared__ ChainWgStop<double> stp;
  const int t0 = threadIdx.x * CHAIN_K;
  double xv[CHAIN_K];
  a.load_items(lo, cnt, t0, xv);
  const ChainWg<PFXW_THREADS, double> sc{shp, &stp};
  ChainNoSink sink;
  r = chain_walk(a, xv, t0, pos, cnt, r, sc, sink);
}
__global__ __launch_bounds__(PFXW_THREADS) void chain_walk_kernel(ChainSrc s, int64_t n, const PfxChunk* __restrict__ ch,
                                                                 int nch, float* __restrict__ total_out, int c_first,
                                                                 const float* __restrict__ r_first) {
  const ChainStat a = chain_stat(s);
  const int hn = c_first > 0 ? 0 : (int)min((long long)CHAIN_HEAD, (long long)n);
  float r = chain_head_serial<PFXW_THREADS>(a, hn, c_first > 0 ? *r_first : 0.f), carry = 0.f;
  chain_walk_chunks<false>(ch, nch, c_first, r, carry, [&](int c) {
    const long long lo = (long long)c * PFXM_CHUNK;
    chain_walk_chunk(a, lo, (int)min((long long)PFXM_CHUNK, (long long)n - lo), r, c == 0 ? hn : 0);
  });
  if (threadIdx.x == 0) *total_out = r;
}
#define CHAIN_HEAD_N 32768
static int chain_head_chunks(int64_t n) { return (tdr_cfg().pfx_small && n >= CHAIN_HEAD_N) ? CHAIN_HEAD_N / PFXM_CHUNK : 0; }
static int chain_head_launch(const float* raw, const float* mean_dev, int kind, int n_head, float* r_out, hipStream_t st);
int tdr_chain_total(const float* raw, const float* mean_dev, int kind, int64_t n, float* total_out, void* workspace,
                    hipStream_t st) {
  const int64_t nch64 = cdiv(n, (int64_t)PFXM_CHUNK);
  if (nch64 > (1 << 24)) return fail(TDR_ERR_ARG, "chain_total: n too large");
  const int nch = (int)nch64;
  PfxChunk* ch = reinterpret_cast<PfxChunk*>(workspace);
  ChainSrc s{raw, mean_dev, kind};
  const int c_first = chain_head_chunks(n);
  hipLaunchKernelGGL(chain_sum_kernel, dim3(nch), dim3(PFXW_THREADS), 0, st, s, n, ch);
  if (nch > c_first)
    hipLaunchKernelGGL(chain_summary_kernel, dim3(nch - c_first), dim3(PFXW_THREADS), 0, st, s, n, ch, c_first);
  float* r_first = reinterpret_cast<float*>(&ch[0].r0);
  if (c_first > 0) {
    const int rc = chain_head_launch(raw, mean_dev, kind, c_first * PFXM_CHUNK, r_first, st);
    if (rc) return rc;
  }
  hipLaunchKernelGGL(chain_walk_kernel, dim3(1), dim3(PFXW_THREADS), 0, st, s, n, (const PfxChunk*)ch, nch, total_out,
                     c_first, (const float*)r_first);
  return TDR_OK;
}

__device__ __forceinline__ float uws_chain_total(int kind, int n, float mean) {
  const UwsWgAdd a{{}, kind, mean};
  const int hn = min(CHAIN_HEAD, n);
  float r = chain_head_serial<PFXW_THREADS>(a, hn, 0.f);
  UW_STAMP(kind ? 5 : 2);
  const int nch = (n + PFXM_CHUNK - 1) / PFXM_CHUNK;
  for (int c = 0; c < nch; c++) {
    const int lo = c * PFXM_CHUNK;
    const int cnt = min((int)PFXM_CHUNK, n - lo);
    if (c == 0 && hn >= cnt) continue;
    chain_walk_chunk(a, lo, cnt, r, c == 0 ? hn : 0);
  }
  return r;
}
#define UWS_THREADS 1024
#define UWS_DUAL_SLOTS 8
#define UWS_DUAL_FLAG 0x100
struct UwsShared {
  double csum[64];
  int code[64];
  unsigned d0[64], d1[64];
  uint4 dual[UWS_DUAL_SLOTS][64];
  double shd[UWS_THREADS / 64];
  float total;
};
template <class A>
__device__ __forceinline__ float uws_wave_walk(const A& a, int lo, int cnt, float r, int pos) {
  const auto ad = a.as_double();
  const int t0 = (threadIdx.x & 63) * CHAIN_K;
  double xv[CHAIN_K];
  ad.load_items(lo, cnt, t0, xv);
  ChainNoSink sink;
  return chain_walk(ad, xv, t0, pos, cnt, r, ChainWave<false>{}, sink);
}
template <class A>
__device__ __forceinline__ float uws_wave_dual(const A& a, int lo, int cnt, float r, const uint4* pq, int& pos) {
  const int lane = threadIdx.x & 63, t0 = lane * CHAIN_K;
  const unsigned rb = __float_as_uint(r), re = rb >> 23, R = (rb & 0x7FFFFFu) | 0x800000u;
  const uint4 v = pq[lane];
  const unsigned after = R + ((R & 1u) ? v.y : v.x);
  const unsigned long long cross = __ballot(after >= (1u << 24));
  pos = cnt;
  if (cross == 0ull) return chain_mant(re, (unsigned)__builtin_amdgcn_readlane((int)after, 63));
  const int L = __ffsll((long long)cross) - 1;
  float rl = chain_mant(re, L > 0 ? (unsigned)__builtin_amdgcn_readlane((int)after, L - 1) : R);
  typename A::value_t x[CHAIN_K];
  a.load_items(lo, cnt, t0, x);
#pragma unroll
  for (int k = 0; k < CHAIN_K; k++) rl = chain_add(rl, x[k]);
  const float r2 = __uint_as_float((unsigned)__builtin_amdgcn_readlane((int)__float_as_uint(rl), L));
  const unsigned rb2 = __float_as_uint(r2), R2 = (rb2 & 0x7FFFFFu) | 0x800000u;
  const int next = (L + 1) * CHAIN_K;
  if (next >= cnt) return r2;
  pos = next;
  if ((rb2 >> 23) != re + 1u) return r2;
  const unsigned qL = (unsigned)__builtin_amdgcn_readlane((int)v.z, L);
  if (qL != (unsigned)__builtin_amdgcn_readlane((int)v.w, L)) return r2;
  const unsigned q63 = (unsigned)__builtin_amdgcn_readlane((int)(((R2 + qL) & 1u) ? v.w : v.z), 63);
  if (q63 >= PFXM_SAT || R2 + (q63 - qL) >= (1u << 24)) return r2;
  pos = cnt;
  return chain_mant(re + 1u, R2 + (q63 - qL));
}
template <class A>
__device__ __forceinline__ float uws_chain_total_waves(const A& a, int n, UwsShared& sh, float* rin = nullptr) {
  const int kind = a.kind;
  constexpr int NW = UWS_THREADS / 64;
  const int lane = threadIdx.x & 63, wave = __builtin_amdgcn_readfirstlane(threadIdx.x >> 6), t0 = lane * CHAIN_K;
  const int nwc = (n + UWS_WC - 1) / UWS_WC;
  float r = 0.f;
  if (wave == 0) {
    r = kind == CHAIN_RUNSUM ? chain_head_lanes<true>(a, min(UWS_WC, n)) : chain_head_lanes<false>(a, min(UWS_WC, n));
  } else {
    int my_code;
    {
      const double own = lane < nwc ? sh.csum[lane] : 0.0;
      const double after = uws_wave_scan_d(own), before = after - own;
      const int re_b = (int)(__float_as_uint((float)before) >> 23), re_a = (int)(__float_as_uint((float)after) >> 23);
      const bool inr = lane >= 1 && lane < nwc && re_b >= PFXM_RE_MIN && re_a <= PFXM_RE_MAX;
      const bool dualc = inr && re_a == re_b + 1;
      const unsigned long long dm = __ballot(dualc);
// ... 345 lines not shown
  (void)chain_walk(a, x, t0, 0, cnt, r, ChainWave<true>{}, sink);
#pragma unroll
  for (int k = 0; k < CHAIN_K; k++)
    if (t0 + k < cnt) uws_lraw[uws_idx(lo + t0 + k)] = sink.pv[k];
}
__device__ __forceinline__ void pfx_small_body(const float* __restrict__ w, int n, float* __restrict__ runmax,
                                               float* __restrict__ prefix_opt,
                                               float* __restrict__ tail) {
  extern __shared__ float uws_lraw[];
  float* const lraw = uws_lraw;
  __shared__ PfsShared sh;
  constexpr int nt = UWS_THREADS, NW = UWS_THREADS / 64;
  const int tid = threadIdx.x, lane = tid & 63, wave = __builtin_amdgcn_readfirstlane(tid >> 6);
  const int nwc = (n + UWS_WC - 1) / UWS_WC;
  if (tid == 0) sh.irregular = 0;
  pfx_sync();
  bool irr = false;
  for (int c = wave; c < nwc; c += NW) {
    const int base = c * UWS_WC + lane;
    float v[CHAIN_K];
#pragma unroll
    for (int m = 0; m < CHAIN_K; m++) v[m] = base + 64 * m < n ? w[base + 64 * m] : 0.f;
    double acc = 0;
#pragma unroll
    for (int m = 0; m < CHAIN_K; m++) {
      if (base + 64 * m < n) lraw[uws_idx(base + 64 * m)] = v[m];
      irr |= !(v[m] >= 0.f);
      acc += (double)v[m];
    }
    acc = uws_wave_scan_d(acc);
    if (lane == 63) sh.u.csum[c] = acc;
  }
  if (__ballot(irr) != 0ull && lane == 0) atomicOr(&sh.irregular, 1);
  pfx_sync();
  const float total = uws_chain_total_waves(UwsAddF{{}, CHAIN_RUNSUM, 0.f}, n, sh.u, sh.rin);
  for (int c = 1 + wave; c < nwc; c += NW) pfs_wave_fill(c * UWS_WC, min(UWS_WC, n - c * UWS_WC), sh.rin[c]);
  pfx_sync();
  if (sh.irregular == 0) {
    if (tail && tid == 0) { tail[0] = total; tail[1] = total; }
    for (int i = tid; i < n; i += nt) {
      const float v = lraw[uws_idx(i)];
      runmax[i] = v;
      if (prefix_opt) prefix_opt[i] = v;
    }
    return;
  }
  const int t0 = lane * CHAIN_K;
  for (int c = wave; c < nwc; c += NW) {
    const int lo = c * UWS_WC, cnt = min(UWS_WC, n - lo);
    float m = -INFINITY;
#pragma unroll
    for (int k = 0; k < CHAIN_K; k++) {
      const float v = lraw[uws_idx(lo + t0 + k)];
      if (t0 + k < cnt && v == v) m = fmaxf(m, v);
    }
    m = pfs_wave_scan_max(m);
    if (lane == 63) sh.cmax[c] = m;
  }
  pfx_sync();
  const float before = pfs_wave_scan_max(lane < nwc ? sh.cmax[lane] : -INFINITY);
  if (tail && tid == 63) { tail[0] = total; tail[1] = before; }
  for (int c = wave; c < nwc; c += NW) {
    const int lo = c * UWS_WC, cnt = min(UWS_WC, n - lo);
    const float carry = c > 0 ? __uint_as_float((unsigned)__builtin_amdgcn_readlane((int)__float_as_uint(before), c - 1)) : -INFINITY;
    float pv[CHAIN_K], lm[CHAIN_K];
    float m = -INFINITY;
#pragma unroll
    for (int k = 0; k < CHAIN_K; k++) {
      pv[k] = lraw[uws_idx(lo + t0 + k)];
      if (t0 + k < cnt && pv[k] == pv[k]) m = fmaxf(m, pv[k]);
      lm[k] = m;
    }
    const float incl = pfs_wave_scan_max(m);
    float ex = __uint_as_float((unsigned)__builtin_amdgcn_update_dpp((int)0xFF800000u, (int)__float_as_uint(incl), 0x138, 0xF, 0xF, false));
    ex = fmaxf(ex, carry);
#pragma unroll
    for (int k = 0; k < CHAIN_K; k++)
      if (t0 + k < cnt) {
        runmax[lo + t0 + k] = fmaxf(lm[k], ex);
        if (prefix_opt) prefix_opt[lo + t0 + k] = pv[k];
      }
  }
}
__global__ __launch_bounds__(UWS_THREADS) void pfx_small_kernel(const float* __restrict__ w, int n,
                                                                float* __restrict__ runmax, float* __restrict__ prefix_opt,
                                                                float* __restrict__ tail) {
  pfx_small_body(w, n, runmax, prefix_opt, tail);
}
__global__ __launch_bounds__(UWS_THREADS) void pfx_small_batch_kernel(const TdrBatchEntry* __restrict__ tab) {
  const TdrBatchEntry& e = tab[blockIdx.x];
  pfx_small_body(e.w_out, (int)e.n, e.runmax_out, nullptr, nullptr);
}
#define TDR_PFX_SMALL_MAX_N 32768
static int pfx_small(const float* w, int64_t n, float* runmax, float* prefix_opt, hipStream_t st, float* tail = nullptr) {
  if (n < 1 || n > TDR_PFX_SMALL_MAX_N) return fail(TDR_ERR_ARG, "pfx_small: n out of range");
  const size_t lds = ((size_t)n + (size_t)(n >> 5) + 1 + UWS_PAD) * sizeof(float);
  static bool attr_set[64] = {false};
  int dev = 0;
  if (hipGetDevice(&dev) != hipSuccess || dev < 0) dev = 0;
  if (dev >= 64 || !attr_set[dev]) {
    if (hipFuncSetAttribute(reinterpret_cast<const void*>(pfx_small_kernel), hipFuncAttributeMaxDynamicSharedMemorySize,
                            133 * 1024) != hipSuccess)
      return fail(TDR_ERR_HIP, "pfx_small: cannot raise the dynamic LDS limit");
    if (dev < 64) attr_set[dev] = true;
  }
  hipLaunchKernelGGL(pfx_small_kernel, dim3(1), dim3(UWS_THREADS), lds, st, w, (int)n, runmax, prefix_opt, tail);
  return TDR_OK;
}

template <int KIND>
__global__ __launch_bounds__(UWS_THREADS) void chain_head_kernel(const float* __restrict__ raw, const float* __restrict__ mean_dev,
                                                                 int n, float* __restrict__ r_out) {
  extern __shared__ float uws_lraw[];
  __shared__ UwsShared ush;
  const int tid = threadIdx.x, lane = tid & 63, nwc = (n + UWS_WC - 1) / UWS_WC;
  const float mean = KIND ? *mean_dev : 0.f;
  for (int c = tid >> 6; c < nwc; c += UWS_THREADS / 64) {
    const int base = c * UWS_WC + lane;
    float v[CHAIN_K];
#pragma unroll
    for (int m = 0; m < CHAIN_K; m++) v[m] = base + 64 * m < n ? raw[base + 64 * m] : __uint_as_float(0x7FC00000u);
    double acc = 0;
#pragma unroll
    for (int m = 0; m < CHAIN_K; m++) {
      if (base + 64 * m < n) uws_lraw[uws_idx(base + 64 * m)] = v[m];
      const bool take = KIND == 0 ? v[m] == v[m] : (v[m] == v[m] && v[m] < mean);
      double x = (double)(KIND == 0 ? v[m] : v[m] - mean);
      if (KIND) x = x * x;
      acc += take ? x : 0.0;
    }
    acc = uws_wave_scan_d(acc);
    if (lane == 63) ush.csum[c] = acc;
  }
  pfx_sync();
  float r;
  if constexpr (KIND == CHAIN_SUM) r = uws_chain_total_waves(UwsAddF{{}, CHAIN_SUM, 0.f}, n, ush);
  else r = uws_chain_total_waves(UwsAddD{{}, CHAIN_BOTTOM, mean}, n, ush);
  if (tid == 0) *r_out = r;
}
static int chain_head_launch(const float* raw, const float* mean_dev, int kind, int n_head, float* r_out, hipStream_t st) {
  const size_t lds = ((size_t)n_head + (size_t)(n_head >> 5) + 1 + UWS_PAD) * sizeof(float);
  static bool attr_set[64] = {false};
  int dev = 0;
  if (hipGetDevice(&dev) != hipSuccess || dev < 0) dev = 0;
  if (dev >= 64 || !attr_set[dev]) {
    if (hipFuncSetAttribute(reinterpret_cast<const void*>(chain_head_kernel<0>), hipFuncAttributeMaxDynamicSharedMemorySize,
                            133 * 1024) != hipSuccess ||
        hipFuncSetAttribute(reinterpret_cast<const void*>(chain_head_kernel<1>), hipFuncAttributeMaxDynamicSharedMemorySize,
                            133 * 1024) != hipSuccess)
      return fail(TDR_ERR_HIP, "chain_head: cannot raise the dynamic LDS limit");
    if (dev < 64) attr_set[dev] = true;
  }
  if (kind == 0)
    hipLaunchKernelGGL(chain_head_kernel<0>, dim3(1), dim3(UWS_THREADS), lds, st, raw, mean_dev, n_head, r_out);
  else
    hipLaunchKernelGGL(chain_head_kernel<1>, dim3(1), dim3(UWS_THREADS), lds, st, raw, mean_dev, n_head, r_out);
  return TDR_OK;
}

#define TDR_PFX_MULTI_MIN_N 6144
#define TDR_PFX_EXACT_MIN_N 24576
#define TDR_PFX_SMALL_MIN_N 256
extern "C" int64_t tdr_prefix_workspace_bytes(int64_t n) {
  return n < 1 ? 0 : (int64_t)sizeof(PfxChunk) * cdiv(n, (int64_t)PFXM_CHUNK);
}
static int prefix_multi(const float* w, int64_t n, float* runmax_out, float* prefix_out, void* workspace,
                        hipStream_t st) {
  const int64_t nch64 = cdiv(n, (int64_t)PFXM_CHUNK);
  if (nch64 > (1 << 24)) return fail(TDR_ERR_ARG, "prefix: n too large");
  const int nch = (int)nch64;
  PfxChunk* ch = reinterpret_cast<PfxChunk*>(workspace);
  const int c_first = chain_head_chunks(n);
  float* tail = reinterpret_cast<float*>(&ch[0].sum);
  hipLaunchKernelGGL(pfx_chunk_sum_kernel, dim3(nch), dim3(PFXM_THREADS), 0, st, w, n, ch);
  if (nch > c_first)
    hipLaunchKernelGGL(pfx_chunk_summary_kernel, dim3(nch - c_first), dim3(PFXM_THREADS), 0, st, w, n, ch, c_first);
  if (c_first > 0) {
    const int rc = pfx_small(w, (int64_t)c_first * PFXM_CHUNK, runmax_out, prefix_out, st, tail);
    if (rc) return rc;
  }
  const int head_len = tdr_cfg().pfx_head;
  hipLaunchKernelGGL(pfx_walk_kernel, dim3(1), dim3(PFXW_THREADS), 0, st, w, n, ch, nch, runmax_out, prefix_out,
                     head_len, c_first, (const float*)tail);
  hipLaunchKernelGGL(pfx_chunk_fill_kernel, dim3(nch), dim3(PFXM_THREADS), 0, st, w, n, (const PfxChunk*)ch,
                     runmax_out, prefix_out);
  return TDR_OK;
}
extern "C" int tdr_k_prefix(const float* w, int64_t n, float* runmax_out, void* workspace, void* stream) {
  if (!w || !runmax_out || n < 1) return fail(TDR_ERR_ARG, "prefix: bad arguments");
  if (tdr_cfg().pfx_small && n >= TDR_PFX_SMALL_MIN_N && n <= TDR_PFX_SMALL_MAX_N) {
    const int rc = pfx_small(w, n, runmax_out, nullptr, (hipStream_t)stream);
    if (rc) return rc;
  } else if (workspace && n >= TDR_PFX_MULTI_MIN_N) {
    const int rc = prefix_multi(w, n, runmax_out, nullptr, workspace, (hipStream_t)stream);
    if (rc) return rc;
  } else if (n < TDR_PFX_EXACT_MIN_N)
    hipLaunchKernelGGL(prefix_serial_kernel, dim3(1), dim3(64), 0, (hipStream_t)stream, w, n, runmax_out);
  else
    hipLaunchKernelGGL(prefix_exact_kernel, dim3(1), dim3(PFX_THREADS), 0, (hipStream_t)stream, w, n, runmax_out,
                       (float*)nullptr);
  LAUNCH_CHECK("prefix");
  return TDR_OK;
}
extern "C" int tdr_k_prefix_mode(const float* w, int64_t n, int mode, float* runmax_out, float* prefix_out,
                                 void* workspace, void* stream) {
  if (!w || !runmax_out || n < 1) return fail(TDR_ERR_ARG, "prefix_mode: bad arguments");
  if (mode == 2 && !workspace) return fail(TDR_ERR_ARG, "prefix_mode: mode 2 needs a workspace");
  if (mode == 3) {
    const int rc = pfx_small(w, n, runmax_out, prefix_out, (hipStream_t)stream);
    if (rc) return rc;
  } else if (mode == 0)
    hipLaunchKernelGGL(prefix_serial_kernel, dim3(1), dim3(64), 0, (hipStream_t)stream, w, n, runmax_out);
  else if (mode == 2) {
    const int rc = prefix_multi(w, n, runmax_out, prefix_out, workspace, (hipStream_t)stream);
    if (rc) return rc;
  } else
    hipLaunchKernelGGL(prefix_exact_kernel, dim3(1), dim3(PFX_THREADS), 0, (hipStream_t)stream, w, n, runmax_out,
                       prefix_out);
  LAUNCH_CHECK("prefix_mode");
  return TDR_OK;
}

static int batch_lds_attr(const void* fn) {
  return hipFuncSetAttribute(fn, hipFuncAttributeMaxDynamicSharedMemorySize, 133 * 1024) == hipSuccess ? TDR_OK
         : fail(TDR_ERR_HIP, "batch: cannot raise the dynamic LDS limit");
}
int tdr_batch_update_weights(const TdrBatchEntry* tab, int k, int64_t n_max, hipStream_t st) {
  if (!tab || k < 1 || n_max < 1 || n_max > 32768) return fail(TDR_ERR_ARG, "batch_update_weights: bad arguments");
  const size_t lds = ((size_t)n_max + (size_t)(n_max >> 5) + 1 + UWS_PAD) * sizeof(float);
  if (tdr_cfg().uw_waves) {
    if (int rc = batch_lds_attr(reinterpret_cast<const void*>(uw_small_batch_kernel<true>))) return rc;
    hipLaunchKernelGGL(uw_small_batch_kernel<true>, dim3((unsigned)k), dim3(UWS_THREADS), lds, st, tab);
  } else {
    if (int rc = batch_lds_attr(reinterpret_cast<const void*>(uw_small_batch_kernel<false>))) return rc;
    hipLaunchKernelGGL(uw_small_batch_kernel<false>, dim3((unsigned)k), dim3(PFXW_THREADS), lds, st, tab);
  }
  LAUNCH_CHECK("batch_update_weights");
  return TDR_OK;
}
int tdr_batch_prefix(const TdrBatchEntry* tab, int k, int64_t n_max, hipStream_t st) {
  if (!tab || k < 1 || n_max < 1 || n_max > TDR_PFX_SMALL_MAX_N) return fail(TDR_ERR_ARG, "batch_prefix: bad arguments");
  const size_t lds = ((size_t)n_max + (size_t)(n_max >> 5) + 1 + UWS_PAD) * sizeof(float);
  if (int rc = batch_lds_attr(reinterpret_cast<const void*>(pfx_small_batch_kernel))) return rc;
  hipLaunchKernelGGL(pfx_small_batch_kernel, dim3((unsigned)k), dim3(UWS_THREADS), lds, st, tab);
  LAUNCH_CHECK("batch_prefix");
  return TDR_OK;
}
```

top_down_renderer_amd/csrc/tdr_raster.hip:

```cpp
#include "tdr_common.h"
#include "tdr_raster_dev.h"

struct RasterArgs {
  const float* pts;
  int stride, ioff;
  int64_t n;
  float res, ang_res;
  const int32_t* lut;
  int ncls, rows, cols, rf, cpt, polar;
  float* img;
  float* pk;
  uint32_t* keys;
};
__global__ __launch_bounds__(256) void raster_keys_kernel(RasterArgs a) {
  const int64_t k = (int64_t)blockIdx.x * blockDim.x + threadIdx.x;
  if (k >= a.n) return;
  a.keys[k] = raster_key(a.pts, a.stride, a.ioff, k, a.polar, a.res, a.ang_res, a.lut, a.ncls, a.rows, a.cols);
}

__global__ __launch_bounds__(1024) void raster_kernel(RasterArgs a) {
  extern __shared__ unsigned int cnt[];
  const int col0 = blockIdx.x * a.cpt;
  const int ncol = min(a.cpt, a.cols - col0);
  raster_tile_clear(cnt, ncol * a.ncls * a.rows);
  __shared__ int lut_s[256];
  if (threadIdx.x < 256) lut_s[threadIdx.x] = a.lut[threadIdx.x];
  __syncthreads();
  if (a.keys) {
    raster_tile_count_keys(cnt, a.keys, a.n, col0, ncol, a.ncls, a.rows);
  } else
  for (int64_t k = threadIdx.x; k < a.n; k += blockDim.x) {
    float x, y, cf;
    raster_point(a.pts, a.stride, a.ioff, k, x, y, cf);
    int row, col;
    if (!raster_bin(a.polar, a.res, a.ang_res, a.rows, a.cols, x, y, row, col)) continue;
    col -= col0;
    if (col < 0 || col >= ncol) continue;
    const int c = raster_class(lut_s, a.ncls, cf);
    if (c < 0) continue;
    atomicAdd(&cnt[(col * a.ncls + c) * a.rows + row], 1u);
  }
  __syncthreads();
  raster_tile_write(cnt, col0, ncol, a.ncls, a.rows, a.cols, a.rf, a.img, a.pk);
}

extern "C" int64_t tdr_raster_workspace_bytes(int64_t n) { return n < 1 ? 0 : 4 * n; }
static int launch_raster(const float* pts, int stride, int ioff, int64_t n, float res, float ang_res,
                         const int32_t* lut, int ncls, int rows, int cols, int polar, float* img, float* pk,
                         void* workspace, void* stream) {
  if (ncls < 1 || ncls > TDR_MAX_CLASSES || rows < 1 || cols < 1) return fail(TDR_ERR_ARG, "raster: bad image shape");
  if (n < 0 || (n > 0 && !pts) || !lut) return fail(TDR_ERR_ARG, "raster: null points / lut");
  if (stride < 3 || ioff < 0 || ioff >= stride) return fail(TDR_ERR_ARG, "raster: bad point stride / offset");
  if (!(res > 0.f) || (polar && !(ang_res > 0.f))) return fail(TDR_ERR_ARG, "raster: resolution must be > 0");
  RasterShape sh;
  if (!raster_shape(ncls, rows, cols, &sh)) return fail(TDR_ERR_ARG, "raster: ncls*rows too large for one LDS tile (152 KB)");
  RasterArgs a;
  a.pts = pts; a.stride = stride; a.ioff = ioff; a.n = n; a.res = res; a.ang_res = ang_res; a.lut = lut;
  a.ncls = ncls; a.rows = rows; a.cols = cols; a.rf = tdr_rec_floats(ncls); a.polar = polar; a.img = img; a.pk = pk;
  a.cpt = sh.cpt;
  static bool attr_set[64] = {false};
  HIP_TRY(raster_allow_lds(reinterpret_cast<const void*>(raster_kernel), sh.lds, attr_set));
  a.keys = nullptr;
  if (workspace && n > 0 && sh.keyed) {
    a.keys = reinterpret_cast<uint32_t*>(workspace);
    hipLaunchKernelGGL(raster_keys_kernel, dim3((unsigned)cdiv(n, 256)), dim3(256), 0, (hipStream_t)stream, a);
  }
  hipLaunchKernelGGL(raster_kernel, dim3((unsigned)cdiv(cols, a.cpt)), dim3(1024), sh.lds, (hipStream_t)stream, a);
  LAUNCH_CHECK("raster");
  return TDR_OK;
}

extern "C" int tdr_k_raster_polar(const float* pts, int stride, int ioff, int64_t n, float res, float ang_res,
                                  const int32_t* lut256, int ncls, int nb, int nr, float* img_out, float* pk_out,
                                  void* workspace, void* stream) {
  return launch_raster(pts, stride, ioff, n, res, ang_res, lut256, ncls, nb, nr, 1, img_out, pk_out, workspace, stream);
}
extern "C" int tdr_k_raster_cart(const float* pts, int stride, int ioff, int64_t n, float res, const int32_t* lut256,
                                 int ncls, int rows, int cols, float* img_out, float* pk_out, void* workspace,
                                 void* stream) {
  return launch_raster(pts, stride, ioff, n, res, 1.f, lut256, ncls, rows, cols, 0, img_out, pk_out, workspace, stream);
}

__global__ void pack_scan_kernel(const float* __restrict__ img, int ncls, int rows, int cols, int rf,
                                 float* __restrict__ pk) {
  int64_t t = (int64_t)blockIdx.x * blockDim.x + threadIdx.x;
  int64_t P = (int64_t)rows * cols;
  if (t >= P) return;
  float* o = pk + t * rf;
  float tot = 0.f;
  for (int c = 0; c < ncls; c++) {
    float v = img[(int64_t)c * P + t];
    o[c] = v;
    tot += v;
  }
  for (int c = ncls; c < rf - 1; c++) o[c] = 0.f;
  if (tdr_has_kslot(ncls, rf)) o[rf - 2] = 1.f;
  o[rf - 1] = tot;
}
extern "C" int tdr_k_pack_scan(const float* img, int ncls, int nb, int nr, float* pk_out, void* stream) {
  if (!img || !pk_out || ncls < 1 || ncls > TDR_MAX_CLASSES || nb < 1 || nr < 1)
    return fail(TDR_ERR_ARG, "pack_scan: bad arguments");
  int64_t P = (int64_t)nb * nr;
  hipLaunchKernelGGL(pack_scan_kernel, dim3((unsigned)cdiv(P, 256)), dim3(256), 0, (hipStream_t)stream, img, ncls, nb,
                     nr, tdr_rec_floats(ncls), pk_out);
  LAUNCH_CHECK("pack_scan");
  return TDR_OK;
}

__global__ void selftest_atan2_kernel(const float* __restrict__ y, const float* __restrict__ x, int64_t n,
                                      float* __restrict__ out) {
  const int64_t i = (int64_t)blockIdx.x * blockDim.x + threadIdx.x;
  if (i < n) out[i] = tdr_atan2f(y[i], x[i]);
}
extern "C" int tdr_k_selftest_atan2(const float* y, const float* x, int64_t n, float* out, void* stream) {
  if (!y || !x || !out || n < 1) return fail(TDR_ERR_ARG, "selftest_atan2: bad arguments");
  hipLaunchKernelGGL(selftest_atan2_kernel, dim3((unsigned)cdiv(n, 256)), dim3(256), 0, (hipStream_t)stream, y, x, n, out);
  LAUNCH_CHECK("selftest_atan2");
  return TDR_OK;
}
```

top_down_renderer_amd/csrc/tdr_raster_dev.h:

```cpp
#ifndef TDR_RASTER_DEV_H_
#define TDR_RASTER_DEV_H_
#include <algorithm>

#include "tdr_common.h"
#include "tdr_atan2f.h"

#define RASTER_NO_BIN 0xFFFFFFFFu
#define RASTER_KEY_MAX_COLS 4095
#define RASTER_KEY_MAX_ROWS 65535

__device__ __forceinline__ void raster_point(const float* __restrict__ pts, int stride, int ioff, int64_t q, float& x,
                                             float& y, float& cf) {
  const float* p = pts + q * stride;
  if (stride == 4 && ioff == 3) {
    float4 v = *reinterpret_cast<const float4*>(p);
    x = v.x; y = v.y; cf = v.w;
  } else {
    x = p[0]; y = p[1]; cf = p[ioff];
  }
}
__device__ __forceinline__ bool raster_bin(int polar, float res, float ang_res, int rows, int cols, float x, float y,
                                           int& row, int& col) {
  if (x == 0.f && y == 0.f) return false;
  if (!(fabsf(x) < INFINITY) || !(fabsf(y) < INFINITY)) return false;
  if (polar) {
    float theta = tdr_atan2f(x, y);
    float r = sqrtf(x * x + y * y);
    row = (int)(roundf(theta / ang_res) + (float)(rows / 2));
    col = (int)roundf(r / res);
  } else {
    col = (int)(roundf(x / res) + (float)(cols / 2));
    row = (int)(roundf(y / res) + (float)(rows / 2));
  }
  return row >= 0 && row < rows && col >= 0 && col < cols;
}
__device__ __forceinline__ int raster_class(const int32_t* lut, int ncls, float cf) {
  const int pc = (cf == cf) ? (int)cf : -1;
  if (pc < 0 || pc > 255) return -1;
  const int c = lut[pc];
  return (c >= 0 && c < ncls) ? c : -1;
}
__device__ __forceinline__ uint32_t raster_key(const float* __restrict__ pts, int stride, int ioff, int64_t q, int polar,
                                               float res, float ang_res, const int32_t* __restrict__ lut, int ncls, int rows,
                                               int cols) {
  float x, y, cf;
  raster_point(pts, stride, ioff, q, x, y, cf);
  int row, col;
  if (!raster_bin(polar, res, ang_res, rows, cols, x, y, row, col)) return RASTER_NO_BIN;
  const int c = raster_class(lut, ncls, cf);
  return c < 0 ? RASTER_NO_BIN : ((uint32_t)col << 20) | ((uint32_t)c << 16) | (uint32_t)row;
}

__device__ __forceinline__ void raster_tile_clear(unsigned int* cnt, int tile) {
  for (int t = threadIdx.x; t < tile; t += blockDim.x) cnt[t] = 0;
}
__device__ __forceinline__ void raster_tile_count_keys(unsigned int* cnt, const uint32_t* __restrict__ keys, int64_t n,
                                                       int col0, int ncol, int ncls, int rows) {
  for (int64_t q = threadIdx.x; q < n; q += blockDim.x) {
    const uint32_t key = keys[q];
    const int col = (int)(key >> 20) - col0;
    if (key == RASTER_NO_BIN || col < 0 || col >= ncol) continue;
    atomicAdd(&cnt[(col * ncls + (int)((key >> 16) & 15u)) * rows + (int)(key & 0xFFFFu)], 1u);
  }
}
__device__ __forceinline__ void raster_tile_write(const unsigned int* cnt, int col0, int ncol, int ncls, int rows, int cols,
                                                  int rf, float* __restrict__ img, float* __restrict__ pk) {
  const int tile = ncol * ncls * rows;
  const int64_t P = (int64_t)rows * cols;
  if (img) {
    for (int t = threadIdx.x; t < tile; t += blockDim.x) {
      int row = t % rows, cc = t / rows;
      int c = cc % ncls, col = cc / ncls;
      img[(int64_t)c * P + row + (int64_t)rows * (col0 + col)] = (float)cnt[t];
    }
  }
  if (pk) {
    const int bins = ncol * rows;
    for (int t = threadIdx.x; t < bins; t += blockDim.x) {
      int row = t % rows, col = t / rows;
      float* o = pk + ((int64_t)(col0 + col) * rows + row) * rf;
      unsigned int tot = 0;
      for (int c = 0; c < ncls; c++) {
        unsigned int v = cnt[(col * ncls + c) * rows + row];
        o[c] = (float)v;
        tot += v;
      }
      for (int c = ncls; c < rf - 1; c++) o[c] = 0.f;
      if (tdr_has_kslot(ncls, rf)) o[rf - 2] = 1.f;
      o[rf - 1] = (float)tot;
    }
  }
}

#define RASTER_MAX_LDS (152 * 1024)
struct RasterShape {
  int cpt;
  size_t lds;
  bool keyed;
};
static inline bool raster_shape(int ncls, int rows, int cols, RasterShape* out) {
  const int64_t per_col = (int64_t)ncls * rows * 4;
  if (per_col > RASTER_MAX_LDS) return false;
  int cpt = (int)std::max<int64_t>(1, (64 * 1024) / per_col);
  cpt = std::min(cpt, cols);
  while (cpt > 1 && cdiv(cols, cpt) < 32) cpt = (cpt + 1) / 2;
  out->cpt = cpt;
  out->lds = (size_t)cpt * per_col;
  out->keyed = cols <= RASTER_KEY_MAX_COLS && rows <= RASTER_KEY_MAX_ROWS;
  return true;
}
static inline hipError_t raster_allow_lds(const void* kernel, size_t lds, bool* attr_set) {
  if (lds <= 64 * 1024) return hipSuccess;
  int dev = 0;
  if (hipGetDevice(&dev) != hipSuccess || dev < 0) dev = 0;
  if (dev < 64 && attr_set[dev]) return hipSuccess;
  const hipError_t e = hipFuncSetAttribute(kernel, hipFuncAttributeMaxDynamicSharedMemorySize, RASTER_MAX_LDS);
  if (e == hipSuccess && dev < 64) attr_set[dev] = true;
  return e;
}

#endif
```

top_down_renderer_amd/csrc/tdr_score.hip:

```cpp

#include "tdr_common.h"
#include "tdr_batch.h"
#include "tdr_sincosf.h"

struct ScoreArgs {
  const float* rec;
  int rows, cols;
  float resolution;
  const float* tab;
  const float* utab = nullptr;
  const float* scan_pk;
  int nb, nr;
  float res;
  const float* st;
  int64_t cap, n;
  const int32_t* order;
  const int32_t* count = nullptr;
  const int32_t* slot_base = nullptr;
  int use_theta_override = 0;
  float theta_override = 0.f;
  int only_uninit = 0;
  int group, nchunks;
  int64_t npad;
  float* part;
// ... 463 lines not shown
    for (int b = 0; b < FIN_B; b++)
#pragma unroll
      for (int k = 0; k < FIN_S; k++)
        if (k < a.ncls + 2) v[b][k] = a.part[(int64_t)(c0 + b) * cstride + (int64_t)slot_row(k) * a.npad + slot];
#pragma unroll
    for (int b = 0; b < FIN_B; b++)
#pragma unroll
      for (int k = 0; k < FIN_S; k++)
        if (k < a.ncls + 2) tot[k] += (double)v[b][k];
  }
  for (; c0 < cend; c0++) {
#pragma unroll
    for (int k = 0; k < FIN_S; k++)
      if (k < a.ncls + 2) tot[k] += (double)a.part[(int64_t)c0 * cstride + (int64_t)slot_row(k) * a.npad + slot];
  }
  if (T > 1) {
    for (int sft = T >> 1; sft >= 1; sft >>= 1)
#pragma unroll
      for (int k = 0; k < FIN_S; k++)
        if (k < a.ncls + 2) tot[k] += __shfl_xor(tot[k], sft, 64);
    if (t != 0) return;
  }
  double known = 0, norm = 0;
#pragma unroll
  for (int k = 0; k < FIN_S; k++) {
    if (k == a.ncls) norm = tot[k];
    if (k == a.ncls + 1) known = tot[k];
  }
  float cost;
  if ((float)known / (float)a.P < 0.5) {
    cost = __builtin_nanf("");
  } else {
    cost = 0.f;
#pragma unroll
    for (int k = 0; k < TDR_MAX_CLASSES; k++)
      if (k < a.ncls) cost = (float)((double)cost + (double)(float)tot[k] * 0.01 * (double)a.fp.class_weights[k]);
    float normf = (float)norm;
    if (a.gpart) {
      double g[2] = {0, 0};
      const int64_t gstride = (int64_t)5 * a.npad;
      for (int c0g = 0; c0g < a.gnchunks; c0g++) {
        g[0] += (double)a.gpart[(int64_t)c0g * gstride + slot];
        g[1] += (double)a.gpart[(int64_t)c0g * gstride + a.npad + slot];
      }
      cost = (float)((double)cost + (double)(float)g[0] * 0.01);
      normf = normf + a.gsum0;
      cost = (float)((double)cost + (double)(float)g[1] * 0.01);
      normf = normf + a.gsum1;
    }
    cost = cost / normf;
  }
  if (a.mode == 0) {
    a.raw_w[p] = (float)(1. / (double)(cost + a.fp.regularization));
  } else {
    float best = a.first ? 3.402823466e+38f : a.best_cost[slot];
    float bt = a.first ? 0.f : a.best_theta[slot];
    if (cost < best) { best = cost; bt = a.theta_override; }
    a.best_cost[slot] = best;
    a.best_theta[slot] = bt;
  }
}
__global__ __launch_bounds__(256) void score_finalize_kernel(FinalizeArgs a) {
  score_finalize_body(a, (int64_t)blockIdx.x * blockDim.x + threadIdx.x);
}
__global__ __launch_bounds__(256) void score_finalize_batch_kernel(const FinalizeArgs* __restrict__ args,
                                                                   const int32_t* __restrict__ blk, int k) {
  const int e = batch_find(k, (int)blockIdx.x, [&](int i) { return blk[i]; });
  const FinalizeArgs a = args[e];
  score_finalize_body(a, (int64_t)(blockIdx.x - (unsigned)blk[e]) * blockDim.x + threadIdx.x);
}

__global__ __launch_bounds__(256) void score_finalize_exact_kernel(FinalizeArgs a) {
  __shared__ unsigned long long red[3][TDR_MAX_CLASSES + 2][64];
  if (int_form_off(a.inexact)) return;
  const int lane = threadIdx.x & 63, t = threadIdx.x >> 6;
  const int64_t nslots = (int64_t)a.counts[2];
  if ((int64_t)blockIdx.x * 64 >= nslots) return;
  const int64_t slot = min((int64_t)blockIdx.x * 64 + lane, nslots - 1);
  const int rows = 2 * a.ncls + 2;
  const int nch = slot < (int64_t)a.counts[0] ? a.nchunks : a.ray_split;
  unsigned long long tot[TDR_MAX_CLASSES], norm = 0, known = 0;
#pragma unroll
  for (int k = 0; k < TDR_MAX_CLASSES; k++) tot[k] = 0;
  for (int c = t; c < nch; c += 4) {
    const uint32_t* o = a.ipart + (int64_t)c * rows * a.npad + slot;
#pragma unroll
    for (int k = 0; k < TDR_MAX_CLASSES; k++)
      if (k < a.ncls)
        tot[k] += (unsigned long long)o[(int64_t)(2 * k) * a.npad] | ((unsigned long long)o[(int64_t)(2 * k + 1) * a.npad] << 32);
    norm += o[(int64_t)(2 * a.ncls) * a.npad];
    known += o[(int64_t)(2 * a.ncls + 1) * a.npad];
  }
  if (t > 0) {
#pragma unroll
    for (int k = 0; k < TDR_MAX_CLASSES; k++)
      if (k < a.ncls) red[t - 1][k][lane] = tot[k];
    red[t - 1][TDR_MAX_CLASSES][lane] = norm;
    red[t - 1][TDR_MAX_CLASSES + 1][lane] = known;
  }
  __syncthreads();
  if (t > 0 || (int64_t)blockIdx.x * 64 + lane >= nslots) return;
  for (int u = 0; u < 3; u++) {
#pragma unroll
    for (int k = 0; k < TDR_MAX_CLASSES; k++)
      if (k < a.ncls) tot[k] += red[u][k][lane];
    norm += red[u][TDR_MAX_CLASSES][lane];
    known += red[u][TDR_MAX_CLASSES + 1][lane];
  }
  const int64_t p = a.order[slot];
  if (p < 0) return;
  const float scale = a.st[TDR_ST_SCALE * a.cap + p];
  const float cx = a.st[TDR_ST_DX * a.cap + p] * scale + a.st[TDR_ST_INIT_X * a.cap + p];
  const float cy = a.st[TDR_ST_DY * a.cap + p] * scale + a.st[TDR_ST_INIT_Y * a.cap + p];
  if (particle_gated(a.gate, cx, cy, scale)) {
    a.raw_w[p] = 0.f;
    return;
  }
  float cost;
  if ((float)known / (float)a.P < 0.5) {
    cost = __builtin_nanf("");
  } else {
    const int q = (int)a.dict_tail[0];
    cost = 0.f;
#pragma unroll
    for (int k = 0; k < TDR_MAX_CLASSES; k++)
      if (k < a.ncls) {
        const float dot = (float)ldexp((double)tot[k], -q);
        cost = (float)((double)cost + (double)dot * 0.01 * (double)a.fp.class_weights[k]);
      }
    cost = cost / (float)norm;
  }
  a.raw_w[p] = (float)(1. / (double)(cost + a.fp.regularization));
}

static int finalize_tlog(int nchunks, int64_t nslots) {
  int tl = 0;
  while (tl < 4 && (nchunks >> (tl + 1)) >= 4 && (nslots << (tl + 1)) <= 131072) tl++;
  return tl;
}
static void launch_finalize(FinalizeArgs& f, int64_t nslots, hipStream_t s) {
  f.tlog = finalize_tlog(f.nchunks, nslots);
  hipLaunchKernelGGL(score_finalize_kernel, dim3((unsigned)cdiv(nslots << f.tlog, 256)), dim3(256), 0, s, f);
}

#define TDR_CART_WAVE_MUL 2
static void choose_chunks(int64_t n, int nr, int& rpc, int& nchunks, int target_mul = 1) {
  int64_t nbatches = cdiv(std::max<int64_t>(n, 1), 64);
  int64_t want = std::max<int64_t>(1, cdiv(tdr_cfg().score_waves * target_mul, nbatches));
  nchunks = (int)std::min<int64_t>(nr, want);
  rpc = (int)cdiv(nr, nchunks);
  nchunks = (int)cdiv(nr, rpc);
}

__global__ void utab_kernel(const float* __restrict__ tab, int64_t n2, float scale, float res,
                            float* __restrict__ utab) {
  const int64_t k = (int64_t)blockIdx.x * blockDim.x + threadIdx.x;
  if (k < n2) utab[k] = (tab[k] * scale) * res;
}

static int score_group_rings(int nb, int nr, int rf, int64_t n_total) {
  const int forced = tdr_cfg().score_group;
  const int64_t ring_bytes = std::max<int64_t>((int64_t)nb * rf * 4, 1);
  int g = (int)std::min<int64_t>(8, (32 * 1024) / ring_bytes);
  const int64_t chunks_wanted = cdiv(2048, cdiv(std::max<int64_t>(n_total, 1), 256));
  g = (int)std::min<int64_t>(g, std::max<int64_t>(1, nr / std::max<int64_t>(chunks_wanted, 1)));
  if (forced > 0) g = forced;
  g = std::max(1, std::min<int>(g, (int)((60 * 1024) / ring_bytes)));
  if (g >= TDR_SCORE_U) g -= g % TDR_SCORE_U;
  return std::max(g, 1);
}
extern "C" int tdr_cmap_words(int ncls);
struct ScoreWs {
  int group, nchunks;
  int su_group, su_nchunks;
// ... 671 lines not shown
```

top_down_renderer_amd/kernels.py:

```python
import ctypes as C

import numpy as np
import torch

from . import _lib
from ._lib import FilterParamsC, MapDescC, check


def _ptr(t):
    return C.c_void_p(t.data_ptr()) if t is not None else C.c_void_p(0)


class ScoreCtx:

    def __init__(self, lib, handle):
        self.lib, self.handle = lib, handle

    def span(self):
        return float(self.lib.tdr_score_ctx_span(self.handle))

    def trial_calls(self):
        return int(self.lib.tdr_score_ctx_trial_calls(self.handle))

    def __del__(self):
# ... 455 lines not shown
        pk = self.empty((nr * nb * self.lib.tdr_rec_floats(ncls),))
        check(self.lib.tdr_k_pack_scan(_ptr(img), ncls, nb, nr, _ptr(pk), self.stream()))
        return pk

    def _workspace(self, ncls, nb, nr, n, n_total=0):
        need = int(self.lib.tdr_score_workspace_floats(ncls, nb, nr, n, n_total))
        if self._ws is None or self._ws.numel() < need:
            self._ws = self.empty((need,))
        return self._ws

    def score_ctx_create(self):
        h = C.c_void_p(0)
        check(self.lib.tdr_score_ctx_create(C.byref(h)))
        return ScoreCtx(self.lib, h)

    def score(self, m, scan_pk, res, fp, st, n, raw_w, perm=None, init_search=False, uniform_scale=0.0, n_total=0, ctx=None):
        ws = self._workspace(m.ncls, m.nb, m.nr, n, n_total)
        cap = st.shape[1]
        if init_search and max(n, n_total) >= int(self.lib.tdr_config_rec16_min_particles(-1)):
            m.init_scratch(self)
        if ctx is not None:
            check(self.lib.tdr_score_ctx_set_polar_factors(ctx.handle, _ptr(getattr(m, "fac", None)), m.nb, m.nr))
        check(self.lib.tdr_k_score_polar_ctx(C.byref(m.desc), _ptr(m.tab), _ptr(scan_pk), m.nb, m.nr, C.c_float(res),
                                             C.byref(fp), _ptr(st), cap, n, n_total, _ptr(perm), C.c_float(uniform_scale),
                                             int(bool(init_search)), _ptr(raw_w), _ptr(ws),
                                             ctx.handle if ctx is not None else C.c_void_p(0), self.stream()))

    def score_geo(self, m, gm, scan_pk, geo_pk, geo_sums, res, fp, st, n, raw_w, perm=None, init_search=False,
                  uniform_scale=0.0):
        need = int(self.lib.tdr_score_geo_workspace_floats(m.ncls, m.nb, m.nr, n, 0))
        if self._ws is None or self._ws.numel() < need:
            self._ws = self.empty((need,))
        check(self.lib.tdr_k_score_polar_geo(C.byref(m.desc), C.byref(gm.desc), _ptr(m.tab), _ptr(scan_pk), _ptr(geo_pk),
                                             C.c_float(geo_sums[0]), C.c_float(geo_sums[1]), m.nb, m.nr, C.c_float(res),
                                             C.byref(fp), _ptr(st), st.shape[1], n, 0, _ptr(perm),
                                             C.c_float(uniform_scale), int(bool(init_search)), _ptr(raw_w),
                                             _ptr(self._ws), self.stream()))

    def score_cart(self, m, scan_pk, rows, cols, res, fp, st, n, raw_w, perm=None, n_total=0):
        need = int(self.lib.tdr_score_cart_workspace_floats(m.ncls, rows, cols, n, n_total))
        if self._ws is None or self._ws.numel() < need:
            self._ws = self.empty((need,))
        check(self.lib.tdr_k_score_cart(C.byref(m.desc), _ptr(scan_pk), rows, cols, C.c_float(res), C.byref(fp),
                                        _ptr(st), st.shape[1], n, n_total, _ptr(perm), _ptr(raw_w), _ptr(self._ws),
                                        self.stream()))

    def score_cart_init(self, m, scan_pk, rows, cols, res, fp, st, n, n_total=0):
        need = int(self.lib.tdr_score_cart_init_workspace_floats(m.ncls, rows, cols, n, n_total))
        if self._init_ws is None or self._init_ws.numel() < need:
            self._init_ws = self.empty((need,))
        check(self.lib.tdr_k_score_cart_init(C.byref(m.desc), _ptr(scan_pk), rows, cols, C.c_float(res), C.byref(fp),
                                             _ptr(st), st.shape[1], n, n_total, _ptr(self._init_ws), self.stream()))

    def propagate(self, st, n, last_dist, tx, ty, omega, scale_freeze, pos_cov, theta_cov, z4=None, seed=0, step=0,
                  index_base=0):
        check(self.lib.tdr_k_propagate(_ptr(st), st.shape[1], n, _ptr(last_dist), C.c_float(tx), C.c_float(ty),
                                       C.c_float(omega), int(scale_freeze), C.c_float(pos_cov), C.c_float(theta_cov),
                                       _ptr(z4), seed, step, index_base, self.stream()))

    def update_weights(self, raw_w, last_dist, n, w_out, info):
        check(self.lib.tdr_k_update_weights(_ptr(raw_w), _ptr(last_dist), n, _ptr(w_out), _ptr(info), self.stream()))

    def prefix_workspace(self, n):
        need = int(self.lib.tdr_prefix_workspace_bytes(n))
        if self._pws is None or self._pws.numel() < need:
            self._pws = self.empty((need,), torch.uint8)
        return self._pws

    def prefix(self, w, n, runmax):
        check(self.lib.tdr_k_prefix(_ptr(w), n, _ptr(runmax), _ptr(self.prefix_workspace(n)), self.stream()))

    def resample(self, runmax, n, n_new, shift, i_begin, i_end, idx):
        check(self.lib.tdr_k_resample(_ptr(runmax), n, n_new, C.c_float(shift), i_begin, i_end, _ptr(idx),
                                      self.stream()))

    def gather_states(self, src, idx, n_new, dst, src_shard=0):
        src_cap = src.shape[1] if src.dim() == 2 else 0
        check(self.lib.tdr_k_gather_states(_ptr(src), src_cap, src_shard, _ptr(idx), n_new, _ptr(dst), dst.shape[1],
                                           self.stream()))

    def save_ml_state(self, info, st, n, out12, src_shard=0):
        cap = st.shape[1] if (st.dim() == 2 and src_shard == 0) else 0
        check(self.lib.tdr_k_save_ml_state(_ptr(info), _ptr(st), cap, src_shard, n, _ptr(out12), self.stream()))

    def mean_cov(self, st, n, about=None):
        out = self.empty((4800,))
        check(self.lib.tdr_k_mean_cov(_ptr(st), st.shape[1], n, _ptr(about), _ptr(out), self.stream()))
        return out

    def sample_ml_states(self, st, n, num):
        out = self.empty((num, 3))
        check(self.lib.tdr_k_sample_ml_states(_ptr(st), st.shape[1], n, num, _ptr(out), self.stream()))
        return out

    def gmm_select(self, samples, num_particles, num_gaussians, max_k=32):
        x = np.ascontiguousarray(samples, np.float64)
        k = C.c_int(int(num_gaussians))
        means = np.zeros((max_k, 3), np.float32)
        covs = np.zeros((max_k, 9), np.float32)
        check(self.lib.tdr_gmm_select_host(x.ctypes.data_as(C.c_void_p), len(x), int(num_particles), C.byref(k), max_k,
                                           means.ctypes.data_as(C.c_void_p), covs.ctypes.data_as(C.c_void_p)))
        return k.value, means[: k.value].copy(), covs[: k.value].reshape(-1, 3, 3).copy()

    def gmm_samples(self, ml3, num):
        out = self.empty((num, 4), torch.float64)
        check(self.lib.tdr_k_gmm_samples(_ptr(ml3), num, _ptr(out), self.stream()))
        return out

    def gmm_fit(self, samples, k, max_iter=100):
        m = samples.shape[0]
        out = self.zeros((int(self.lib.tdr_gmm_out_doubles(k)),), torch.float64)
        ws = self.empty((max(1, int(self.lib.tdr_gmm_workspace_bytes(m, k)) // 8),), torch.float64)
        check(self.lib.tdr_k_gmm_fit(_ptr(samples), m, k, max_iter, _ptr(out), _ptr(ws), self.stream()))
        o = out.cpu().numpy()
        return o[:k].copy(), o[k:5 * k].reshape(k, 4).copy(), o[5 * k:21 * k].reshape(k, 4, 4).copy(), float(o[21 * k]), \
            int(o[21 * k + 1])

    def gmm_candidates(self, num_gaussians, num_particles, m, max_k=_lib.GMM_MAX_K):
        cand = (C.c_int * 3)()
        check(self.lib.tdr_gmm_candidates_host(int(num_gaussians), int(num_particles), int(m), int(max_k), cand))
        return list(cand)

    def gmm_select_device(self, ml3, num, num_particles, num_gaussians):
        import math
        x = self.gmm_samples(ml3, num)
        cand = self.gmm_candidates(num_gaussians, num_particles, num)
        jobs, pick, keep = [], _lib.GmmPickJobC(), []
        pick.k = cand[0]
        for j, kc in enumerate(cand):
            if not kc:
                continue
            out = self.zeros((21 * kc + 2,), torch.float64)
            ws = self.empty((num * kc,), torch.float64)
            keep += [out, ws]
            jobs.append(_lib.GmmJobC(x.data_ptr(), num, kc, 100, 0, out.data_ptr(), ws.data_ptr()))
            pick.cand[j] = out.data_ptr()
        rec = self.zeros((_lib.GMM_RECORD_DOUBLES,), torch.float64)
        pick.record = rec.data_ptr()
        jobs_c = (_lib.GmmJobC * len(jobs))(*jobs)
        jobs_d = self.to_device(np.frombuffer(bytes(jobs_c), np.uint8))
        pick_d = self.to_device(np.frombuffer(bytes(pick), np.uint8))
        check(self.lib.tdr_k_gmm_fit_jobs(_ptr(jobs_d), len(jobs), self.stream()))
        check(self.lib.tdr_k_gmm_pick(_ptr(pick_d), 1, self.stream()))
        r = rec.cpu().numpy()
        k = int(r[0])
        if not 1 <= k <= _lib.GMM_MAX_K:
            raise _lib.TdrError("gmm_select_device: the device fit left no mixture")
        o = r[2:2 + 8 * k].reshape(k, 8)
        means = np.zeros((k, 3), np.float32)
        covs = np.zeros((k, 3, 3), np.float32)
        means[:, 0], means[:, 1] = o[:, 0], o[:, 1]
        means[:, 2] = [math.atan2(a, b) for a, b in zip(o[:, 3], o[:, 2])]
        covs[:, :2, :2] = o[:, 4:8].reshape(k, 2, 2)
        covs[:, 2, 2] = 1
        return k, means, covs

    def viz_planes(self, H, W):
        words = int(self.lib.tdr_viz_plane_words(H, W))
        if words == 0:
            raise _lib.TdrError(f"no picture of {H} x {W} pixels")
        return self.zeros((4 * words,), torch.int32)

    def viz_draw(self, st, n, background, planes, segs, out_h, out_w, out=None):
        H, W = int(background.shape[0]), int(background.shape[1])
        if out is None:
            out = self.empty((out_h, out_w, 3), torch.uint8)
        planes.zero_()
        check(self.lib.tdr_k_viz_particles(_ptr(st), st.shape[1], n, H, W, _ptr(planes), self.stream()))
        if len(segs):
            segs_d = self.to_device(np.ascontiguousarray(segs, np.int32))
            check(self.lib.tdr_k_viz_segments(_ptr(segs_d), len(segs), H, W, _ptr(planes), self.stream()))
        check(self.lib.tdr_k_viz_compose(_ptr(background), H, W, _ptr(planes), out_h, out_w, _ptr(out), self.stream()))
        return out

    def set_scale(self, st, n, scale_dev):
        check(self.lib.tdr_k_set_scale(_ptr(st), st.shape[1], n, _ptr(scale_dev), self.stream()))

    def shift_init(self, st, n, dx, dy):
        check(self.lib.tdr_k_shift_init(_ptr(st), st.shape[1], n, C.c_float(dx), C.c_float(dy), self.stream()))

    def locality_order(self, st, n, rows, cols, perm):
        need = int(self.lib.tdr_locality_tmp_ints(n, rows, cols))
        tmp = self.empty((need,), torch.int32)
        check(self.lib.tdr_k_locality_order(_ptr(st), st.shape[1], n, rows, cols, _ptr(perm), _ptr(tmp),
                                            self.stream()))

    def locality_order_pose(self, st, n, rows, cols, perm, theta_radius):
        need = int(self.lib.tdr_locality_pose_tmp_ints(n))
        tmp = self.empty((need + 2,), torch.int32)
        check(self.lib.tdr_k_locality_order_pose(_ptr(st), st.shape[1], n, rows, cols, C.c_float(theta_radius),
                                                 _ptr(perm), _ptr(tmp), self.stream()))

    def states_to_device(self, states_aos, st, n):
        raw = self.to_device(np.ascontiguousarray(states_aos).view(np.uint8).reshape(-1))
        check(self.lib.tdr_k_states_aos_to_soa(_ptr(raw), n, _ptr(st), st.shape[1], self.stream()))
        self.synchronize()

    def states_to_host(self, st, n, dtype):
        raw = self.empty((n * 28,), torch.uint8)
        check(self.lib.tdr_k_states_soa_to_aos(_ptr(st), st.shape[1], n, _ptr(raw), self.stream()))
        return raw.cpu().numpy().view(dtype).reshape(-1).copy()

    def su_order(self, st, n, nb, span, perm=None, workspace=None):
        need = int(self.lib.tdr_k_su_order_workspace_ints(n, nb))
        if workspace is None:
            workspace = self.empty((need,), torch.int32)
        if workspace.numel() < need:
            raise ValueError(f"su_order: workspace of {workspace.numel()} words, {need} needed")
        slots = self.empty((int(self.lib.tdr_k_su_order_slots(n, nb)),), torch.int32)
        keys = self.empty((n,), torch.int32)
        counts = self.empty((3,), torch.int32)
        bucket = C.c_int(-1)
        check(self.lib.tdr_k_su_order(_ptr(st), st.shape[1], n, _ptr(perm) if perm is not None else None, nb,
                                      C.c_float(span), _ptr(workspace), _ptr(slots), _ptr(keys), _ptr(counts), C.byref(bucket),
                                      self.stream()))
        return slots, keys, counts, bool(bucket.value)

    def tuning(self, name, value=-1):
        return int(self.lib.tdr_config_tuning(name.encode(), value))

    def rng_create(self, seed):
        return C.c_void_p(self.lib.tdr_rng_create(C.c_uint32(seed & 0xFFFFFFFF)))

    device_rng = True

    def rng_state_to_device(self, rng):
        words = np.zeros(640, np.uint32)
        check(self.lib.tdr_rng_get_state_host(rng, words.ctypes.data_as(C.c_void_p)))
        return self.to_device(words.view(np.int32))

    def rng_state_to_host(self, rng, state_dev):
        words = np.ascontiguousarray(state_dev.cpu().numpy()).view(np.uint32)
        check(self.lib.tdr_rng_set_state_host(rng, words.ctypes.data_as(C.c_void_p)))

    def rng_propagate_normals_dev(self, state_dev, n, lo, hi, scale_freeze, z4_out, n_max):
        need = int(self.lib.tdr_rng_dev_workspace_bytes(max(n, n_max)))
        if getattr(self, "_rws", None) is None or self._rws.numel() < need:
            self._rws = self.empty((need,), torch.uint8)
        check(self.lib.tdr_k_rng_propagate_normals(_ptr(state_dev), n, lo, hi, int(scale_freeze), _ptr(z4_out),
                                                   _ptr(self._rws), self.stream()))

    def rng_uniform_dev(self, state_dev, out_dev):
        check(self.lib.tdr_k_rng_uniform(_ptr(state_dev), _ptr(out_dev), self.stream()))

    def resample_dev(self, runmax, n, n_new, shift_dev, i_begin, i_end, idx):
        check(self.lib.tdr_k_resample_dev(_ptr(runmax), n, n_new, _ptr(shift_dev), i_begin, i_end, _ptr(idx), self.stream()))

    def rng_pipe_create(self, n_max):
        h = C.c_void_p(0)
        check(self.lib.tdr_rng_pipe_create(n_max, C.byref(h)))
        return RngPipe(self, h)

    def rng_uniform(self, rng):
        return float(self.lib.tdr_rng_uniform_host(rng))

    def init_particles(self, rng, maps_cm_host, ncls, rows, cols, resolution, fp, max_num, dtype):
        out = np.zeros(max_num + 16, dtype)
        n = C.c_int64(0)
        check(self.lib.tdr_init_particles_host(rng, maps_cm_host.ctypes.data_as(C.c_void_p), ncls, rows, cols,
                                               C.c_float(resolution), C.byref(fp), max_num,
                                               out.ctypes.data_as(C.c_void_p), C.byref(n)))
        return out[: min(n.value, max_num + 16)].copy()

    def init_particles_count(self, fp, max_num):
        return int(self.lib.tdr_init_particles_count(C.byref(fp), max_num))

    def init_particles_dev(self, state_dev, dmap, fp, max_num, lo, hi, st):
        n = C.c_int64(0)
        ws = self.empty((int(self.lib.tdr_init_workspace_bytes()),), torch.uint8)
        check(self.lib.tdr_k_init_particles(_ptr(state_dev), C.byref(dmap.desc), C.byref(fp), max_num, lo, hi, _ptr(st),
                                            st.shape[1], C.byref(n), _ptr(ws), self.stream()))
        return n.value

    def propagate_normals(self, rng, n, scale_freeze):
        z = np.empty((n, 4), np.float32)
        check(self.lib.tdr_propagate_normals_host(rng, n, int(scale_freeze), z.ctypes.data_as(C.c_void_p)))
        return z
```

top_down_renderer_amd/particle_filter.py:

```python
import ctypes as C
import math
from dataclasses import dataclass, field

import numpy as np
import torch

from ._lib import FilterParamsC
from .synth import STATE_DTYPE


@dataclass
class FilterParams:
    pos_cov: float = 0.3
    theta_cov: float = math.pi / 100
    regularization: float = 0.15
    init_pos_px_x: float = -1.0
    init_pos_px_y: float = -1.0
    init_pos_px_cov: float = -1.0
    init_pos_m_x: float = float("inf")
    init_pos_m_y: float = float("inf")
    init_pos_deg_theta: float = float("inf")
    init_pos_deg_cov: float = 10.0
    force_on_map: bool = False
    fixed_scale: float = -1.0
# ... 196 lines not shown
        elif self.parity_rng:
            self._rng_to_host()
            z = self.k.propagate_normals(self.gen_, n, self.scale_frozen_)
            z_dev = self.k.to_device(z[self.comm.rank * nl:(self.comm.rank + 1) * nl])
        self.k.propagate(self.st, nl, self.last_dist, float(trans[0]), float(trans[1]), float(omega),
                         self.scale_frozen_, p.pos_cov, p.theta_cov, z4=z_dev, seed=self.seed, step=self.prop_calls_,
                         index_base=self.comm.rank * nl)
        self.prop_calls_ += 1

    def update(self, top_down_scan, top_down_geo=None, res=1.0, n_target=None, covs=None, shift=None):
        if self.num_particles_ == 0:
            return
        k, m, comm = self.k, self.map_, self.comm
        n, nl = self.num_particles_, self.n_local
        scan_pk = m.scan_handle(top_down_scan)
        comm.broadcast(scan_pk, 0)

        if self.locality_every and (self.perm is None or self.step_ % self.locality_every == 0):
            if self.perm is None:
                self.perm = k.zeros((self.cap_local,), torch.int32)
            if getattr(m, "polar", True):
                k.locality_order(self.st, nl, m.rows, m.cols, self.perm)
            else:
                wr, wc = m.window_shape()
                k.locality_order_pose(self.st, nl, m.rows, m.cols, self.perm, theta_radius=(wr + wc) / 16.0)
        if getattr(m, "polar", True) and self.use_geometric_cost and top_down_geo is not None:
            geo = np.stack([np.asarray(g, np.float32).reshape(m.nb, m.nr, order="A").ravel(order="F")
                            for g in top_down_geo[:2]])
            geo_pk = k.pack_scan(k.to_device(geo), 2, m.nb, m.nr)
            sums = (float(np.float32(geo[0].astype(np.float64).sum())), float(np.float32(geo[1].astype(np.float64).sum())))
            k.score_geo(m.dev, m.geo_dev(), scan_pk, geo_pk, sums, float(res), self.fp_c, self.st, nl, self.raw_w,
                        perm=self.perm if self.locality_every else None, init_search=self._maybe_uninit,
                        uniform_scale=self._uniform_scale)
        elif getattr(m, "polar", True):
            k.score(m.dev, scan_pk, float(res), self.fp_c, self.st, nl, self.raw_w,
                    perm=self.perm if self.locality_every else None, init_search=self._maybe_uninit,
                    uniform_scale=self._uniform_scale, n_total=n, ctx=self.score_ctx)
        else:
            rows, cols = m.window_shape()
            if self._maybe_uninit:
                k.score_cart_init(m.dev, scan_pk, rows, cols, float(res), self.fp_c, self.st, nl, n_total=n)
            k.score_cart(m.dev, scan_pk, rows, cols, float(res), self.fp_c, self.st, nl, self.raw_w,
                         perm=self.perm if self.locality_every else None, n_total=n)
        if not getattr(m, "polar", True) or not (self.params_.force_on_map or self.params_.fixed_scale < 0):
            self._maybe_uninit = False
        self._n_raw = nl

        if comm.active:
            self.xchg_in[0, :nl].copy_(self.raw_w[:nl])
            self.xchg_in[1, :nl].copy_(self.last_dist[:nl])
            xin = self.xchg_in[:, :nl].contiguous()
            xout = self.xchg_out.view(-1)[: comm.world * 2 * nl]
            comm.all_gather(xout, xin.view(-1))
            xo = xout.view(comm.world, 2, nl)
            self.raw_glob[:n].view(comm.world, nl).copy_(xo[:, 0, :])
            self.ld_glob[:n].view(comm.world, nl).copy_(xo[:, 1, :])
            raw_glob, ld_glob = self.raw_glob, self.ld_glob
        else:
            raw_glob, ld_glob = self.raw_w, self.last_dist
        st_work, sa = None, None
        if comm.active:
            sa = self.st_all[: comm.world * 7 * nl]
            self._st_send = self.st[:, :nl].contiguous().view(-1)
            st_work = comm.all_gather(sa, self._st_send, async_op=True)
        k.update_weights(raw_glob, ld_glob, n, self.weights_, self.info)
        self._n_weights = n

        n_new = n
        if covs is not None:
            acc = 0
            for c in covs:
                ev = np.linalg.eigvals(np.asarray(c, np.float32)[:2, :2]).real.astype(np.float32)
                acc += int(np.float32(np.sqrt(ev[0])) * np.float32(np.sqrt(ev[1])))
            n_new = min(max(acc, 3 * n // 4 + 10), self.max_num_particles_)
        elif n_target is not None:
            n_new = min(int(n_target), self.max_num_particles_)
        n_new = max(comm.world, (n_new // comm.world) * comm.world)

        k.prefix(self.weights_, n, self.runmax)
        nl_new = n_new // comm.world
        i0 = comm.rank * nl_new
        if shift is None and self._rng_on_device:
            self._shift_dev = self._pipe.uniform()
            k.resample_dev(self.runmax, n, n_new, self._shift_dev, i0, i0 + nl_new, self.idx)
        else:
            if shift is None:
                shift = k.rng_uniform(self.gen_)
            k.resample(self.runmax, n, n_new, float(shift), i0, i0 + nl_new, self.idx)
        if comm.active:
            if st_work is not None:
                st_work.wait()
            k.gather_states(sa, self.idx, nl_new, self.st_new, src_shard=nl)
            self._save_ml_state(sa, nl)
        else:
            k.gather_states(self.st, self.idx, nl_new, self.st_new)
            self._save_ml_state(None, nl)
        self.st, self.st_new = self.st_new, self.st
        self.num_particles_ = n_new
        self.perm = None if n_new != n else self.perm
        self.step_ += 1
        self._last_shift = None if shift is None else float(shift)

    def _save_ml_state(self, st_all, nl):
        if self._ml_buf is None:
            self._ml_buf = self.k.zeros((12,))
        if st_all is not None:
            self.k.save_ml_state(self.info, st_all, self.num_particles_, self._ml_buf, src_shard=nl)
        else:
            self.k.save_ml_state(self.info, self.st, self.num_particles_, self._ml_buf)
        self._ml_fields = self._ml_buf[:7]

    def resample_indices(self):
        return self.idx[: self.n_local].cpu().numpy().copy()

    def _argmax(self):
        return int(self.info[:1].cpu().view(torch.int32).item())

    def _global_states(self):
        nl = self.n_local
        if not self.comm.active:
            return self.st, nl, 0
        sa = self.st_all[: self.comm.world * 7 * nl]
        self.comm.all_gather(sa, self.st[:, :nl].contiguous().view(-1))
        full = sa.view(self.comm.world, 7, nl).permute(1, 0, 2).contiguous().view(7, -1)
        return full, self.num_particles_, 0

    def meanLikelihood(self):
        st, n, _ = self._global_states()
        return self.k.mean_cov(st, n)[:4].cpu().numpy().copy()

    def computeGMM(self, device=False):
        st, n, _ = self._global_states()
        if n < 1:
            return
        num = min(1000, n)
        if device:
            ml3 = self.k.sample_ml_states(st, n, num)
            self.num_gaussians_, self.gmm_means_, self.gmm_covs_ = self.k.gmm_select_device(ml3, num, n, self.num_gaussians_)
            return
        h = self.k.sample_ml_states(st, n, num).cpu().numpy()
        x = np.empty((num, 4), np.float64)
        x[:, 0], x[:, 1] = h[:, 0], h[:, 1]
        x[:, 2] = np.float32(50) * np.cos(h[:, 2])
        x[:, 3] = np.float32(50) * np.sin(h[:, 2])
        self.num_gaussians_, self.gmm_means_, self.gmm_covs_ = self.k.gmm_select(x, n, self.num_gaussians_)

    def adaptiveCount(self):
        k = len(self.gmm_means_)
        if k == 0:
            return self.num_particles_
        covs = np.ascontiguousarray(self.gmm_covs_, np.float32)
        return int(self.k.lib.tdr_adaptive_count_host(covs.ctypes.data_as(C.c_void_p), k, self.num_particles_,
                                                      self.max_num_particles_))

    def getGMM(self):
        return self.gmm_means_.copy(), self.gmm_covs_.copy()

    def computeMeanCov(self):
        if self.num_particles_ < 1:
            return np.zeros((4, 4), np.float32)
        st, n, _ = self._global_states()
        return self.k.mean_cov(st, n)[4:20].cpu().numpy().reshape(4, 4).copy()

    def maxLikelihood(self):
        if self._ml_fields is None:
            raise RuntimeError("maxLikelihood: no update yet, there is no max-likelihood particle")
        s = self._ml_fields.cpu().numpy()
        sc = np.float32(s[5])
        return np.asarray([np.float32(s[2] * sc + s[0]), np.float32(s[3] * sc + s[1]), s[4], sc], np.float32)

    def computeCov(self):
        st, n, _ = self._global_states()
        ref = self.k.to_device(self.maxLikelihood())
        return self.k.mean_cov(st, n, about=ref)[4:20].cpu().numpy().reshape(4, 4).copy()

    def freezeScale(self):
        if not self.scale_frozen_:
            st, n, _ = self._global_states()
            out = self.k.mean_cov(st, n)
# ... 67 lines not shown
```

Measured before the change: 23.55 million.

## Fuse resample/gather/ML-save, merge weight-update passes, vectorize raster key counting

Fuses resample index selection, state gather and ML-state save into one kernel when running on a single device, replacing three launches. The weight-update statistics passes are merged into the chunked prefix workspace, so valid and under-mean counts come from the chain passes instead of separate reduction kernels. Raster key counting now reads uint4 vectors and uses more column tiles when keys are present. The score reduction loads two chunks per iteration. Together these cut launch count and memory traffic, in exchange for more scratch space and more complex code paths.

```diff
diff --git a/include/tdr.h b/include/tdr.h
--- a/include/tdr.h
+++ b/include/tdr.h
@@ -212,6 +212,9 @@
 int tdr_k_save_ml_state(const float* info, const float* st, int64_t cap, int64_t src_shard, int64_t n, float* out12,
                         void* stream);
 int tdr_k_shift_init(float* st, int64_t cap, int64_t n, float dx, float dy, void* stream);
+int tdr_k_resample_gather(const float* runmax, int64_t n, int64_t n_new, const float* shift_dev, float shift,
+                          int64_t i_begin, int64_t i_end, int32_t* idx_out, const float* src, int64_t src_cap,
+                          int64_t src_shard, float* dst, int64_t dst_cap, const float* info, float* out12, void* stream);
 
 int tdr_config_compact(int on);
 int tdr_config_shift_uniform(int mode);
diff --git a/top_down_renderer_amd/_lib.py b/top_down_renderer_amd/_lib.py
--- a/top_down_renderer_amd/_lib.py
+++ b/top_down_renderer_amd/_lib.py
@@ -205,6 +205,7 @@
     "tdr_filter_compute_gmm_device": (_i, [_vp]),
     "tdr_batch_compute_gmm": (_i, [_vp, _i, _vp]),
     "tdr_k_save_ml_state": (_i, [_vp, _vp, _i64, _i64, _i64, _vp, _vp]),
+    "tdr_k_resample_gather": (_i, [_vp, _i64, _i64, _vp, _f, _i64, _i64, _vp, _vp, _i64, _i64, _vp, _i64, _vp, _vp, _vp]),
     "tdr_k_shard_pack2": (_i, [_vp, _vp, _i64, _vp, _vp]),
     "tdr_k_shard_unpack2": (_i, [_vp, _i, _i64, _vp, _vp, _vp]),
     "tdr_k_unshard_states": (_i, [_vp, _i, _i64, _vp, _i64, _vp]),
diff --git a/top_down_renderer_amd/csrc/tdr_batch_loop.hip b/top_down_renderer_amd/csrc/tdr_batch_loop.hip
--- a/top_down_renderer_amd/csrc/tdr_batch_loop.hip
+++ b/top_down_renderer_amd/csrc/tdr_batch_loop.hip
@@ -26,7 +26,7 @@
 
 bool tdr_batch_raster_shape(int ncls, int rows, int cols, float ang_res, TdrBatchRasterShape* out) {
   RasterShape sh;
-  if (ncls < 1 || ncls > TDR_MAX_CLASSES || rows < 1 || cols < 1 || !raster_shape(ncls, rows, cols, &sh) || !sh.keyed)
+  if (ncls < 1 || ncls > TDR_MAX_CLASSES || rows < 1 || cols < 1 || !raster_shape(ncls, rows, cols, true, &sh) || !sh.keyed)
     return false;
   TdrBatchRasterShape a;
   a.ang_res = ang_res; a.ncls = ncls; a.rows = rows; a.cols = cols; a.rf = tdr_rec_floats(ncls); a.cpt = sh.cpt;
diff --git a/top_down_renderer_amd/csrc/tdr_common.h b/top_down_renderer_amd/csrc/tdr_common.h
--- a/top_down_renderer_amd/csrc/tdr_common.h
+++ b/top_down_renderer_amd/csrc/tdr_common.h
@@ -68,7 +68,13 @@
 #define INI_TILE 2048
 #define INI_MAX_TILES 2048
 int tdr_chain_total(const float* raw, const float* mean_dev, int kind, int64_t n, float* total_out, void* workspace,
-                    hipStream_t st);
+                    bool have_sums, hipStream_t st);
+struct UwExact {
+  float sum, mean, bsum, pad;
+};
+int tdr_uw_chunk_pass1(const float* raw, int64_t n, void* workspace, int* cnt_valid, hipStream_t st);
+int tdr_uw_chunk_pass2(const float* raw, int64_t n, UwExact* ex, const int* cnt_valid, void* workspace, int* cnt_under,
+                       hipStream_t st);
 int tdr_uw_small(const float* raw, const float* last_dist, int64_t n, float* w, float* info, hipStream_t st);
 int tdr_mt_raw_stream(const uint32_t* state, int64_t nblocks, uint32_t* raw, hipStream_t s);
 int tdr_mt_advance(const uint32_t* raw, int64_t nblocks, const uint32_t* consumed, uint32_t* state, hipStream_t s);
diff --git a/top_down_renderer_amd/csrc/tdr_filter.hip b/top_down_renderer_amd/csrc/tdr_filter.hip
--- a/top_down_renderer_amd/csrc/tdr_filter.hip
+++ b/top_down_renderer_amd/csrc/tdr_filter.hip
@@ -187,46 +187,18 @@
   __syncthreads();
   return result;
 }
-__global__ __launch_bounds__(256) void uw_pass1(const float* __restrict__ raw, int64_t n, UwScratch* s1) {
+__device__ long long uw_count_total(const int* __restrict__ cnt, int nch, long long* shl) {
+  long long c = 0;
+  for (int j = threadIdx.x; j < nch; j += blockDim.x) c += cnt[j];
+  return block_sum_ll(c, shl);
+}
+__global__ __launch_bounds__(256) void uw_pass3(const float* __restrict__ raw, int64_t n, const UwExact* ex,
+                                                const int* __restrict__ cnt_under, int nch, UwScratch* s3,
+                                                float* __restrict__ w) {
   __shared__ double shd[4];
   __shared__ long long shl[4];
-  int64_t lo, hi;
-  uw_chunk(n, lo, hi);
-  double s = 0;
-  long long c = 0;
-  for (int64_t i = lo + threadIdx.x; i < hi; i += 256) {
-    const float v = raw[i];
-    if (!isnan(v)) { s += (double)v; c++; }
-  }
-  const double ts = block_sum_d(s, shd);
-  const long long tc = block_sum_ll(c, shl);
-  if (threadIdx.x == 0) { s1->a[blockIdx.x] = ts; s1->b[blockIdx.x] = (double)tc; }
-}
-struct UwExact {
-  float sum, mean, bsum, pad;
-};
-__global__ __launch_bounds__(256) void uw_pass2(const float* __restrict__ raw, int64_t n, const UwScratch* s1,
-                                                UwScratch* s2, UwExact* ex) {
-  __shared__ long long shl[4];
-  const float mean = ex->sum / (float)(long long)uw_total(s1->b);
-  int64_t lo, hi;
-  uw_chunk(n, lo, hi);
-  long long cu = 0;
-  for (int64_t i = lo + threadIdx.x; i < hi; i += 256) {
-    const float v = raw[i];
-    if (!isnan(v) && v < mean) cu++;
-  }
-  const long long tc = block_sum_ll(cu, shl);
-  if (threadIdx.x == 0) {
-    s2->b[blockIdx.x] = (double)tc;
-    if (blockIdx.x == 0) ex->mean = mean;
-  }
-}
-__global__ __launch_bounds__(256) void uw_pass3(const float* __restrict__ raw, int64_t n, const UwExact* ex,
-                                                const UwScratch* s2, UwScratch* s3, float* __restrict__ w) {
-  __shared__ double shd[4];
   const float sum = ex->sum, mean = ex->mean;
-  const long long num_under = (long long)uw_total(s2->b);
+  const long long num_under = uw_count_total(cnt_under, nch, shl);
   const float bottom = sqrtf(ex->bsum / (float)num_under);
   const bool fallback = (sum == 0.f || num_under < 1);
   const float fill = mean - bottom;
@@ -260,6 +232,32 @@
   const double t = block_sum_d(acc, shd);
   if (threadIdx.x == 0) s4->a[blockIdx.x] = t;
 }
+__device__ __forceinline__ void uw_write_info(const UwScratch* s5, const int* __restrict__ cnt_valid,
+                                              const int* __restrict__ cnt_under, int nch, const UwExact* ex, float* info) {
+  static_assert(UW_G == 256, "one candidate per thread");
+  __shared__ float sb[4];
+  __shared__ long long si[4];
+  __shared__ long long shl[4];
+  float best = (float)s5->a[threadIdx.x];
+  long long besti = (long long)s5->b[threadIdx.x];
+  if (best != best) { best = -INFINITY; besti = 0x7fffffffffffffffll; }
+  for (int o = 32; o > 0; o >>= 1) {
+    const float ob = __shfl_down(best, o, 64);
+    const long long oi = __shfl_down(besti, o, 64);
+    if (ob > best || (ob == best && oi < besti)) { best = ob; besti = oi; }
+  }
+  if ((threadIdx.x & 63) == 0) { sb[threadIdx.x >> 6] = best; si[threadIdx.x >> 6] = besti; }
+  const float sum = ex->sum, mean = ex->mean;
+  const long long nv = uw_count_total(cnt_valid, nch, shl), nu = uw_count_total(cnt_under, nch, shl);
+  const float bottom = sqrtf(ex->bsum / (float)nu);
+  if (threadIdx.x != 0) return;
+  for (int k = 1; k < 4; k++)
+    if (sb[k] > best || (sb[k] == best && si[k] < besti)) { best = sb[k]; besti = si[k]; }
+  if (besti == 0x7fffffffffffffffll) besti = 0;
+  info[0] = __int_as_float((int)besti);
+  info[1] = sum; info[2] = mean; info[3] = bottom; info[4] = (sum == 0.f || nu < 1) ? 1.f : 0.f;
+  info[5] = (float)nv; info[6] = (float)nu; info[7] = 0.f;
+}
 __global__ __launch_bounds__(256) void uw_pass5(int64_t n, const UwScratch* s4, UwScratch* s5, float* __restrict__ w) {
   __shared__ float sb[4];
   __shared__ long long si[4];
@@ -287,30 +285,9 @@
     s5->b[blockIdx.x] = (double)besti;
   }
 }
-__global__ __launch_bounds__(256) void uw_pass6(int64_t n, const UwScratch* s1, const UwScratch* s2,
-                                                const UwScratch* s5, const UwExact* ex, float* info) {
-  static_assert(UW_G == 256, "one candidate per thread");
-  __shared__ float sb[4];
-  __shared__ long long si[4];
-  float best = (float)s5->a[threadIdx.x];
-  long long besti = (long long)s5->b[threadIdx.x];
-  if (best != best) { best = -INFINITY; besti = 0x7fffffffffffffffll; }
-  for (int o = 32; o > 0; o >>= 1) {
-    const float ob = __shfl_down(best, o, 64);
-    const long long oi = __shfl_down(besti, o, 64);
-    if (ob > best || (ob == best && oi < besti)) { best = ob; besti = oi; }
-  }
-  if ((threadIdx.x & 63) == 0) { sb[threadIdx.x >> 6] = best; si[threadIdx.x >> 6] = besti; }
-  const float sum = ex->sum, mean = ex->mean;
-  const long long nv = (long long)uw_total(s1->b), nu = (long long)uw_total(s2->b);
-  const float bottom = sqrtf(ex->bsum / (float)nu);
-  if (threadIdx.x != 0) return;
-  for (int k = 1; k < 4; k++)
-    if (sb[k] > best || (sb[k] == best && si[k] < besti)) { best = sb[k]; besti = si[k]; }
-  if (besti == 0x7fffffffffffffffll) besti = 0;
-  info[0] = __int_as_float((int)besti);
-  info[1] = sum; info[2] = mean; info[3] = bottom; info[4] = (sum == 0.f || nu < 1) ? 1.f : 0.f;
-  info[5] = (float)nv; info[6] = (float)nu; info[7] = 0.f;
+__global__ __launch_bounds__(256) void uw_pass6(const UwScratch* s5, const int* __restrict__ cnt_valid,
+                                                const int* __restrict__ cnt_under, int nch, const UwExact* ex, float* info) {
+  uw_write_info(s5, cnt_valid, cnt_under, nch, ex, info);
 }
 
 #define TDR_UW_SINGLE_MAX_N 32768
@@ -325,27 +302,32 @@
     LAUNCH_CHECK("update_weights");
     return TDR_OK;
   }
-  constexpr size_t kFixed = 8 * sizeof(float) + 64 + 5 * sizeof(UwScratch) + sizeof(UwExact) + 64;
-  static_assert(kFixed + 32 * 1024 <= TDR_UW_INFO_FLOATS * sizeof(float), "info scratch");
+  constexpr size_t kFixed = 8 * sizeof(float) + 64 + 3 * sizeof(UwScratch) + sizeof(UwExact) + 64;
+  static_assert(kFixed + 40 * 1024 <= TDR_UW_INFO_FLOATS * sizeof(float), "info scratch");
   UwScratch* sc = reinterpret_cast<UwScratch*>(
       (reinterpret_cast<uintptr_t>(info_out + 8) + 63) & ~(uintptr_t)63);
-  UwExact* ex = reinterpret_cast<UwExact*>(sc + 5);
+  UwExact* ex = reinterpret_cast<UwExact*>(sc + 3);
   void* chain_ws = reinterpret_cast<void*>((reinterpret_cast<uintptr_t>(ex + 1) + 63) & ~(uintptr_t)63);
   const size_t chain_room = TDR_UW_INFO_FLOATS * sizeof(float) - kFixed;
-  if ((size_t)tdr_prefix_workspace_bytes(n) > chain_room)
+  const int64_t nch = tdr_prefix_workspace_bytes(n) / 32;
+  if ((size_t)tdr_prefix_workspace_bytes(n) + (size_t)nch * 2 * sizeof(int) > chain_room)
     return fail(TDR_ERR_ARG, "update_weights: n = %lld needs more than TDR_UW_INFO_FLOATS of scratch", (long long)n);
-  hipLaunchKernelGGL(uw_pass1, dim3(UW_G), dim3(256), 0, s, raw_w, n, sc + 0);
-  int rc = tdr_chain_total(raw_w, nullptr, 0, n, &ex->sum, chain_ws, s);
+  int* cnt_valid = reinterpret_cast<int*>(reinterpret_cast<char*>(chain_ws) + tdr_prefix_workspace_bytes(n));
+  int* cnt_under = cnt_valid + nch;
+  int rc = tdr_uw_chunk_pass1(raw_w, n, chain_ws, cnt_valid, s);
   if (rc) return rc;
-  hipLaunchKernelGGL(uw_pass2, dim3(UW_G), dim3(256), 0, s, raw_w, n, (const UwScratch*)(sc + 0), sc + 1, ex);
-  rc = tdr_chain_total(raw_w, &ex->mean, 1, n, &ex->bsum, chain_ws, s);
+  rc = tdr_chain_total(raw_w, nullptr, 0, n, &ex->sum, chain_ws, true, s);
   if (rc) return rc;
-  hipLaunchKernelGGL(uw_pass3, dim3(UW_G), dim3(256), 0, s, raw_w, n, (const UwExact*)ex, (const UwScratch*)(sc + 1),
-                     sc + 2, w_out);
-  hipLaunchKernelGGL(uw_pass4, dim3(UW_G), dim3(256), 0, s, last_dist, n, (const UwScratch*)(sc + 2), sc + 3, w_out);
-  hipLaunchKernelGGL(uw_pass5, dim3(UW_G), dim3(256), 0, s, n, (const UwScratch*)(sc + 3), sc + 4, w_out);
-  hipLaunchKernelGGL(uw_pass6, dim3(1), dim3(256), 0, s, n, (const UwScratch*)(sc + 0), (const UwScratch*)(sc + 1),
-                     (const UwScratch*)(sc + 4), (const UwExact*)ex, info_out);
+  rc = tdr_uw_chunk_pass2(raw_w, n, ex, cnt_valid, chain_ws, cnt_under, s);
+  if (rc) return rc;
+  rc = tdr_chain_total(raw_w, &ex->mean, 1, n, &ex->bsum, chain_ws, true, s);
+  if (rc) return rc;
+  hipLaunchKernelGGL(uw_pass3, dim3(UW_G), dim3(256), 0, s, raw_w, n, (const UwExact*)ex, (const int*)cnt_under, (int)nch,
+                     sc + 0, w_out);
+  hipLaunchKernelGGL(uw_pass4, dim3(UW_G), dim3(256), 0, s, last_dist, n, (const UwScratch*)(sc + 0), sc + 1, w_out);
+  hipLaunchKernelGGL(uw_pass5, dim3(UW_G), dim3(256), 0, s, n, (const UwScratch*)(sc + 1), sc + 2, w_out);
+  hipLaunchKernelGGL(uw_pass6, dim3(1), dim3(256), 0, s, (const UwScratch*)(sc + 2), (const int*)cnt_valid,
+                     (const int*)cnt_under, (int)nch, (const UwExact*)ex, info_out);
   LAUNCH_CHECK("update_weights(multi)");
   return TDR_OK;
 }
@@ -387,12 +369,8 @@
   return TDR_OK;
 }
 
-__global__ void gather_states_kernel(const float* __restrict__ src, int64_t src_cap, int64_t src_shard,
-                                     const int32_t* __restrict__ idx, int64_t n_new, float* __restrict__ dst,
-                                     int64_t dst_cap) {
-  const int64_t i = (int64_t)blockIdx.x * blockDim.x + threadIdx.x;
-  if (i >= n_new) return;
-  const int64_t j = idx[i];
+__device__ __forceinline__ void gather_state(const float* __restrict__ src, int64_t src_cap, int64_t src_shard, int64_t j,
+                                             float* __restrict__ dst, int64_t dst_cap, int64_t i) {
   if (src_shard > 0) {
     const int64_t r = j / src_shard, l = j - r * src_shard;
 #pragma unroll
@@ -400,6 +378,13 @@
   } else {
     gather_particle(src, src_cap, j, dst, dst_cap, i);
   }
+}
+__global__ void gather_states_kernel(const float* __restrict__ src, int64_t src_cap, int64_t src_shard,
+                                     const int32_t* __restrict__ idx, int64_t n_new, float* __restrict__ dst,
+                                     int64_t dst_cap) {
+  const int64_t i = (int64_t)blockIdx.x * blockDim.x + threadIdx.x;
+  if (i >= n_new) return;
+  gather_state(src, src_cap, src_shard, idx[i], dst, dst_cap, i);
 }
 
 extern "C" int tdr_k_gather_states(const float* src, int64_t src_cap, int64_t src_shard, const int32_t* idx,
@@ -475,9 +460,8 @@
   return TDR_OK;
 }
 
-__global__ void save_ml_state_kernel(const float* __restrict__ info, const float* __restrict__ st, int64_t cap,
-                                     int64_t src_shard, int64_t n, float* __restrict__ out) {
-  if (threadIdx.x != 0 || blockIdx.x != 0) return;
+__device__ __forceinline__ void save_ml_state(const float* __restrict__ info, const float* __restrict__ st, int64_t cap,
+                                              int64_t src_shard, int64_t n, float* __restrict__ out) {
   const int64_t best = ml_index(info, n);
   float f[TDR_ST_FIELDS];
   if (src_shard > 0) {
@@ -490,6 +474,11 @@
   }
   ml_record(f, out);
 }
+__global__ void save_ml_state_kernel(const float* __restrict__ info, const float* __restrict__ st, int64_t cap,
+                                     int64_t src_shard, int64_t n, float* __restrict__ out) {
+  if (threadIdx.x != 0 || blockIdx.x != 0) return;
+  save_ml_state(info, st, cap, src_shard, n, out);
+}
 extern "C" int tdr_k_save_ml_state(const float* info, const float* st, int64_t cap, int64_t src_shard, int64_t n,
                                    float* out12, void* stream) {
   if (!info || !st || !out12 || n < 1 || src_shard < 0 || (src_shard == 0 && cap < n))
@@ -497,6 +486,36 @@
   hipLaunchKernelGGL(save_ml_state_kernel, dim3(1), dim3(64), 0, (hipStream_t)stream, info, st, cap, src_shard, n,
                      out12);
   LAUNCH_CHECK("save_ml_state");
+  return TDR_OK;
+}
+
+__global__ __launch_bounds__(256) void resample_gather_kernel(const float* __restrict__ runmax, int64_t n, int64_t n_new,
+                                                              const float* __restrict__ shift_dev, float shift,
+                                                              int64_t i_begin, int64_t i_end, int32_t* __restrict__ idx,
+                                                              const float* __restrict__ src, int64_t src_cap,
+                                                              int64_t src_shard, float* __restrict__ dst, int64_t dst_cap,
+                                                              const float* __restrict__ info, float* __restrict__ out12) {
+  const int64_t i = i_begin + (int64_t)blockIdx.x * blockDim.x + threadIdx.x;
+  if (i < i_end) {
+    const int64_t j = resample_pick(runmax, n, n_new, i, shift_dev ? *shift_dev : shift);
+    idx[i - i_begin] = (int32_t)j;
+    gather_state(src, src_cap, src_shard, j, dst, dst_cap, i - i_begin);
+  }
+  if (blockIdx.x == 0 && threadIdx.x == 0) save_ml_state(info, src, src_cap, src_shard, n, out12);
+}
+extern "C" int tdr_k_resample_gather(const float* runmax, int64_t n, int64_t n_new, const float* shift_dev, float shift,
+                                     int64_t i_begin, int64_t i_end, int32_t* idx_out, const float* src, int64_t src_cap,
+                                     int64_t src_shard, float* dst, int64_t dst_cap, const float* info, float* out12,
+                                     void* stream) {
+  if (!runmax || !idx_out || !src || !dst || !info || !out12) return fail(TDR_ERR_ARG, "resample_gather: null pointer");
+  if (n < 1 || n_new < 1 || i_begin < 0 || i_end > n_new || i_begin > i_end)
+    return fail(TDR_ERR_ARG, "resample_gather: bad range");
+  if (src_shard < 0 || (src_shard == 0 && src_cap < n) || dst_cap < i_end - i_begin || dst == src)
+    return fail(TDR_ERR_ARG, "resample_gather: bad state buffers");
+  const unsigned blocks = (unsigned)std::max<int64_t>(1, cdiv(i_end - i_begin, 256));
+  hipLaunchKernelGGL(resample_gather_kernel, dim3(blocks), dim3(256), 0, (hipStream_t)stream, runmax, n, n_new, shift_dev,
+                     shift, i_begin, i_end, idx_out, src, src_cap, src_shard, dst, dst_cap, info, out12);
+  LAUNCH_CHECK("resample_gather");
   return TDR_OK;
 }
 
diff --git a/top_down_renderer_amd/csrc/tdr_host.cpp b/top_down_renderer_amd/csrc/tdr_host.cpp
--- a/top_down_renderer_amd/csrc/tdr_host.cpp
+++ b/top_down_renderer_amd/csrc/tdr_host.cpp
@@ -1424,15 +1424,13 @@
   const int64_t nl_new = n_new / f->world, i0 = (int64_t)f->rank * nl_new;
   TTRY(f->ml_dev.resize(12));
   TTRY(tdr_k_prefix(f->w.p, n, f->runmax.p, f->pfx_ws.p, f->stream));
-  if (rng_on_device(f)) {
-    const float* shift_dev = nullptr;
-    TTRY(tdr_rng_pipe_uniform(f->pipe, &shift_dev, f->stream));
-    TTRY(tdr_k_resample_dev(f->runmax.p, n, n_new, shift_dev, i0, i0 + nl_new, f->idx.p, f->stream));
-  } else {
-    const float shift = tdr_rng_uniform_host(f->rng);
-    TTRY(tdr_k_resample(f->runmax.p, n, n_new, shift, i0, i0 + nl_new, f->idx.p, f->stream));
-  }
+  const float* shift_dev = nullptr;
+  float shift = 0.f;
+  if (rng_on_device(f)) TTRY(tdr_rng_pipe_uniform(f->pipe, &shift_dev, f->stream));
+  else shift = tdr_rng_uniform_host(f->rng);
   if (f->comm) {
+    if (shift_dev) TTRY(tdr_k_resample_dev(f->runmax.p, n, n_new, shift_dev, i0, i0 + nl_new, f->idx.p, f->stream));
+    else TTRY(tdr_k_resample(f->runmax.p, n, n_new, shift, i0, i0 + nl_new, f->idx.p, f->stream));
     for (int k = 0; k < TDR_ST_FIELDS; k++)
       HTRY(hipMemcpyAsync(f->st_send.p + (size_t)k * nl, f->st.p + (size_t)k * f->cap, (size_t)nl * sizeof(float),
                           hipMemcpyDeviceToDevice, f->stream));
@@ -1440,8 +1438,8 @@
     TTRY(tdr_k_gather_states(f->st_all.p, 0, nl, f->idx.p, nl_new, f->st_new.p, f->cap, f->stream));
     TTRY(tdr_k_save_ml_state(f->info.p, f->st_all.p, 0, nl, n, f->ml_dev.p, f->stream));
   } else {
-    TTRY(tdr_k_gather_states(f->st.p, f->cap, 0, f->idx.p, n_new, f->st_new.p, f->cap, f->stream));
-    TTRY(tdr_k_save_ml_state(f->info.p, f->st.p, f->cap, 0, n, f->ml_dev.p, f->stream));
+    TTRY(tdr_k_resample_gather(f->runmax.p, n, n_new, shift_dev, shift, 0, n_new, f->idx.p, f->st.p, f->cap, 0, f->st_new.p,
+                               f->cap, f->info.p, f->ml_dev.p, f->stream));
   }
   f->have_ml = true;
   f->states_changed();
diff --git a/top_down_renderer_amd/csrc/tdr_prefix.hip b/top_down_renderer_amd/csrc/tdr_prefix.hip
--- a/top_down_renderer_amd/csrc/tdr_prefix.hip
+++ b/top_down_renderer_amd/csrc/tdr_prefix.hip
@@ -1093,25 +1093,91 @@
 }
 #define CHAIN_HEAD_N 32768
 static int chain_head_chunks(int64_t n) { return (tdr_cfg().pfx_small && n >= CHAIN_HEAD_N) ? CHAIN_HEAD_N / PFXM_CHUNK : 0; }
-static int chain_head_launch(const float* raw, const float* mean_dev, int kind, int n_head, float* r_out, hipStream_t st);
+static int chain_head_launch(const float* raw, const float* mean_dev, int kind, int n_head, float* r_out, int64_t n,
+                             PfxChunk* ch, int nch, hipStream_t st);
 int tdr_chain_total(const float* raw, const float* mean_dev, int kind, int64_t n, float* total_out, void* workspace,
-                    hipStream_t st) {
+                    bool have_sums, hipStream_t st) {
   const int64_t nch64 = cdiv(n, (int64_t)PFXM_CHUNK);
   if (nch64 > (1 << 24)) return fail(TDR_ERR_ARG, "chain_total: n too large");
   const int nch = (int)nch64;
   PfxChunk* ch = reinterpret_cast<PfxChunk*>(workspace);
   ChainSrc s{raw, mean_dev, kind};
   const int c_first = chain_head_chunks(n);
-  hipLaunchKernelGGL(chain_sum_kernel, dim3(nch), dim3(PFXW_THREADS), 0, st, s, n, ch);
-  if (nch > c_first)
-    hipLaunchKernelGGL(chain_summary_kernel, dim3(nch - c_first), dim3(PFXW_THREADS), 0, st, s, n, ch, c_first);
+  if (!have_sums) hipLaunchKernelGGL(chain_sum_kernel, dim3(nch), dim3(PFXW_THREADS), 0, st, s, n, ch);
   float* r_first = reinterpret_cast<float*>(&ch[0].r0);
   if (c_first > 0) {
-    const int rc = chain_head_launch(raw, mean_dev, kind, c_first * PFXM_CHUNK, r_first, st);
+    const int rc = chain_head_launch(raw, mean_dev, kind, c_first * PFXM_CHUNK, r_first, n, ch, nch, st);
     if (rc) return rc;
+  } else if (nch > c_first) {
+    hipLaunchKernelGGL(chain_summary_kernel, dim3(nch - c_first), dim3(PFXW_THREADS), 0, st, s, n, ch, c_first);
   }
   hipLaunchKernelGGL(chain_walk_kernel, dim3(1), dim3(PFXW_THREADS), 0, st, s, n, (const PfxChunk*)ch, nch, total_out,
                      c_first, (const float*)r_first);
+  return TDR_OK;
+}
+
+template <int NT>
+__device__ __forceinline__ int uw_wg_sum_int(int v, int* sh) {
+#pragma unroll
+  for (int o = 32; o >= 1; o >>= 1) v += __shfl_xor(v, o, 64);
+  pfx_sync();
+  if ((threadIdx.x & 63) == 0) sh[threadIdx.x >> 6] = v;
+  pfx_sync();
+  int t = 0;
+  for (int k = 0; k < NT / 64; k++) t += sh[k];
+  return t;
+}
+template <bool BELOW>
+__device__ __forceinline__ int uw_chunk_count(const float* __restrict__ raw, int64_t n, float mean, int* sh) {
+  const long long lo = (long long)blockIdx.x * PFXM_CHUNK;
+  const int cnt = (int)min((long long)PFXM_CHUNK, (long long)n - lo);
+  const ChainAddend<float, ChainGlobal, CHAIN_BOUND_22> plain{{raw}, CHAIN_RUNSUM, 0.f};
+  float v[CHAIN_K];
+  const int t0 = threadIdx.x * CHAIN_K;
+  plain.load_items(lo, cnt, t0, v);
+  int c = 0;
+#pragma unroll
+  for (int k = 0; k < CHAIN_K; k++) c += (t0 + k < cnt && v[k] == v[k] && (!BELOW || v[k] < mean)) ? 1 : 0;
+  return uw_wg_sum_int<PFXW_THREADS>(c, sh);
+}
+__global__ __launch_bounds__(PFXW_THREADS) void uw_chunk_pass1_kernel(const float* __restrict__ raw, int64_t n,
+                                                                     PfxChunk* __restrict__ ch, int* __restrict__ cnt_valid) {
+  __shared__ int shc[PFXW_THREADS / 64];
+  const int c = uw_chunk_count<false>(raw, n, 0.f, shc);
+  if (threadIdx.x == 0) cnt_valid[blockIdx.x] = c;
+  chain_sum_body<PFXW_THREADS, CHAIN_K>(ChainStat{{raw}, CHAIN_SUM, 0.f}, n, ch);
+}
+__global__ __launch_bounds__(PFXW_THREADS) void uw_chunk_pass2_kernel(const float* __restrict__ raw, int64_t n,
+                                                                     UwExact* __restrict__ ex,
+                                                                     const int* __restrict__ cnt_valid,
+                                                                     PfxChunk* __restrict__ ch, int* __restrict__ cnt_under) {
+  __shared__ int shc[PFXW_THREADS / 64];
+  __shared__ long long shv[PFXW_THREADS / 64];
+  long long nv = 0;
+  for (int j = threadIdx.x; j < (int)gridDim.x; j += PFXW_THREADS) nv += cnt_valid[j];
+#pragma unroll
+  for (int o = 32; o >= 1; o >>= 1) nv += __shfl_xor(nv, o, 64);
+  if ((threadIdx.x & 63) == 0) shv[threadIdx.x >> 6] = nv;
+  pfx_sync();
+  nv = 0;
+  for (int k = 0; k < PFXW_THREADS / 64; k++) nv += shv[k];
+  const float mean = ex->sum / (float)nv;
+  const int c = uw_chunk_count<true>(raw, n, mean, shc);
+  if (threadIdx.x == 0) {
+    cnt_under[blockIdx.x] = c;
+    if (blockIdx.x == 0) ex->mean = mean;
+  }
+  chain_sum_body<PFXW_THREADS, CHAIN_K>(ChainStat{{raw}, CHAIN_BOTTOM, mean}, n, ch);
+}
+int tdr_uw_chunk_pass1(const float* raw, int64_t n, void* workspace, int* cnt_valid, hipStream_t st) {
+  hipLaunchKernelGGL(uw_chunk_pass1_kernel, dim3((unsigned)cdiv(n, (int64_t)PFXM_CHUNK)), dim3(PFXW_THREADS), 0, st, raw, n,
+                     reinterpret_cast<PfxChunk*>(workspace), cnt_valid);
+  return TDR_OK;
+}
+int tdr_uw_chunk_pass2(const float* raw, int64_t n, UwExact* ex, const int* cnt_valid, void* workspace, int* cnt_under,
+                       hipStream_t st) {
+  hipLaunchKernelGGL(uw_chunk_pass2_kernel, dim3((unsigned)cdiv(n, (int64_t)PFXM_CHUNK)), dim3(PFXW_THREADS), 0, st, raw, n,
+                     ex, cnt_valid, reinterpret_cast<PfxChunk*>(workspace), cnt_under);
   return TDR_OK;
 }
 
@@ -1623,9 +1689,17 @@
       }
   }
 }
+static_assert(PFXM_THREADS % 64 == 0 && PFXW_THREADS % 64 == 0 && PFXM_THREADS <= UWS_THREADS && PFXW_THREADS <= UWS_THREADS,
+              "summary blocks: whole waves of the head's workgroup");
 __global__ __launch_bounds__(UWS_THREADS) void pfx_small_kernel(const float* __restrict__ w, int n,
                                                                 float* __restrict__ runmax, float* __restrict__ prefix_opt,
-                                                                float* __restrict__ tail) {
+                                                                float* __restrict__ tail, int64_t n_all,
+                                                                PfxChunk* __restrict__ ch, int c_first) {
+  if (blockIdx.x > 0) {
+    if (threadIdx.x < PFXM_THREADS)
+      chain_summary_body<PFXM_THREADS, PFXM_K>(PfxRunSum{{w}, CHAIN_RUNSUM, 0.f}, n_all, ch, c_first - 1);
+    return;
+  }
   pfx_small_body(w, n, runmax, prefix_opt, tail);
 }
 __global__ __launch_bounds__(UWS_THREADS) void pfx_small_batch_kernel(const TdrBatchEntry* __restrict__ tab) {
@@ -1633,7 +1707,8 @@
   pfx_small_body(e.w_out, (int)e.n, e.runmax_out, nullptr, nullptr);
 }
 #define TDR_PFX_SMALL_MAX_N 32768
-static int pfx_small(const float* w, int64_t n, float* runmax, float* prefix_opt, hipStream_t st, float* tail = nullptr) {
+static int pfx_small(const float* w, int64_t n, float* runmax, float* prefix_opt, hipStream_t st, float* tail = nullptr,
+                     int64_t n_all = 0, PfxChunk* ch = nullptr, int nch = 0) {
   if (n < 1 || n > TDR_PFX_SMALL_MAX_N) return fail(TDR_ERR_ARG, "pfx_small: n out of range");
   const size_t lds = ((size_t)n + (size_t)(n >> 5) + 1 + UWS_PAD) * sizeof(float);
   static bool attr_set[64] = {false};
@@ -1645,17 +1720,25 @@
       return fail(TDR_ERR_HIP, "pfx_small: cannot raise the dynamic LDS limit");
     if (dev < 64) attr_set[dev] = true;
   }
-  hipLaunchKernelGGL(pfx_small_kernel, dim3(1), dim3(UWS_THREADS), lds, st, w, (int)n, runmax, prefix_opt, tail);
+  const int c_first = ch ? (int)(n / PFXM_CHUNK) : 0;
+  hipLaunchKernelGGL(pfx_small_kernel, dim3(1 + (ch ? (unsigned)std::max(0, nch - c_first) : 0u)), dim3(UWS_THREADS), lds,
+                     st, w, (int)n, runmax, prefix_opt, tail, n_all, ch, c_first);
   return TDR_OK;
 }
 
 template <int KIND>
 __global__ __launch_bounds__(UWS_THREADS) void chain_head_kernel(const float* __restrict__ raw, const float* __restrict__ mean_dev,
-                                                                 int n, float* __restrict__ r_out) {
+                                                                 int n, float* __restrict__ r_out, int64_t n_all,
+                                                                 PfxChunk* __restrict__ ch, int c_first) {
+  const float mean = KIND ? *mean_dev : 0.f;
+  if (blockIdx.x > 0) {
+    if (threadIdx.x < PFXW_THREADS)
+      chain_summary_body<PFXW_THREADS, CHAIN_K>(ChainStat{{raw}, KIND, mean}, n_all, ch, c_first - 1);
+    return;
+  }
   extern __shared__ float uws_lraw[];
   __shared__ UwsShared ush;
   const int tid = threadIdx.x, lane = tid & 63, nwc = (n + UWS_WC - 1) / UWS_WC;
-  const float mean = KIND ? *mean_dev : 0.f;
   for (int c = tid >> 6; c < nwc; c += UWS_THREADS / 64) {
     const int base = c * UWS_WC + lane;
     float v[CHAIN_K];
@@ -1679,7 +1762,8 @@
   else r = uws_chain_total_waves(UwsAddD{{}, CHAIN_BOTTOM, mean}, n, ush);
   if (tid == 0) *r_out = r;
 }
-static int chain_head_launch(const float* raw, const float* mean_dev, int kind, int n_head, float* r_out, hipStream_t st) {
+static int chain_head_launch(const float* raw, const float* mean_dev, int kind, int n_head, float* r_out, int64_t n,
+                             PfxChunk* ch, int nch, hipStream_t st) {
   const size_t lds = ((size_t)n_head + (size_t)(n_head >> 5) + 1 + UWS_PAD) * sizeof(float);
   static bool attr_set[64] = {false};
   int dev = 0;
@@ -1692,10 +1776,12 @@
       return fail(TDR_ERR_HIP, "chain_head: cannot raise the dynamic LDS limit");
     if (dev < 64) attr_set[dev] = true;
   }
+  const int c_first = n_head / PFXM_CHUNK;
+  const dim3 grid(1 + (unsigned)std::max(0, nch - c_first));
   if (kind == 0)
-    hipLaunchKernelGGL(chain_head_kernel<0>, dim3(1), dim3(UWS_THREADS), lds, st, raw, mean_dev, n_head, r_out);
+    hipLaunchKernelGGL(chain_head_kernel<0>, grid, dim3(UWS_THREADS), lds, st, raw, mean_dev, n_head, r_out, n, ch, c_first);
   else
-    hipLaunchKernelGGL(chain_head_kernel<1>, dim3(1), dim3(UWS_THREADS), lds, st, raw, mean_dev, n_head, r_out);
+    hipLaunchKernelGGL(chain_head_kernel<1>, grid, dim3(UWS_THREADS), lds, st, raw, mean_dev, n_head, r_out, n, ch, c_first);
   return TDR_OK;
 }
 
@@ -1712,13 +1798,14 @@
   const int nch = (int)nch64;
   PfxChunk* ch = reinterpret_cast<PfxChunk*>(workspace);
   const int c_first = chain_head_chunks(n);
-  float* tail = reinterpret_cast<float*>(&ch[0].sum);
+  float* tail = reinterpret_cast<float*>(&ch[0].r0);
+  static_assert(offsetof(PfxChunk, carry0) == offsetof(PfxChunk, r0) + sizeof(float), "tail: sum, maximum");
   hipLaunchKernelGGL(pfx_chunk_sum_kernel, dim3(nch), dim3(PFXM_THREADS), 0, st, w, n, ch);
-  if (nch > c_first)
+  if (c_first > 0) {
+    const int rc = pfx_small(w, (int64_t)c_first * PFXM_CHUNK, runmax_out, prefix_out, st, tail, n, ch, nch);
+    if (rc) return rc;
+  } else if (nch > c_first) {
     hipLaunchKernelGGL(pfx_chunk_summary_kernel, dim3(nch - c_first), dim3(PFXM_THREADS), 0, st, w, n, ch, c_first);
-  if (c_first > 0) {
-    const int rc = pfx_small(w, (int64_t)c_first * PFXM_CHUNK, runmax_out, prefix_out, st, tail);
-    if (rc) return rc;
   }
   const int head_len = tdr_cfg().pfx_head;
   hipLaunchKernelGGL(pfx_walk_kernel, dim3(1), dim3(PFXW_THREADS), 0, st, w, n, ch, nch, runmax_out, prefix_out,
diff --git a/top_down_renderer_amd/csrc/tdr_raster.hip b/top_down_renderer_amd/csrc/tdr_raster.hip
--- a/top_down_renderer_amd/csrc/tdr_raster.hip
+++ b/top_down_renderer_amd/csrc/tdr_raster.hip
@@ -53,7 +53,7 @@
   if (stride < 3 || ioff < 0 || ioff >= stride) return fail(TDR_ERR_ARG, "raster: bad point stride / offset");
   if (!(res > 0.f) || (polar && !(ang_res > 0.f))) return fail(TDR_ERR_ARG, "raster: resolution must be > 0");
   RasterShape sh;
-  if (!raster_shape(ncls, rows, cols, &sh)) return fail(TDR_ERR_ARG, "raster: ncls*rows too large for one LDS tile (152 KB)");
+  if (!raster_shape(ncls, rows, cols, workspace && n > 0, &sh)) return fail(TDR_ERR_ARG, "raster: ncls*rows too large for one LDS tile (152 KB)");
   RasterArgs a;
   a.pts = pts; a.stride = stride; a.ioff = ioff; a.n = n; a.res = res; a.ang_res = ang_res; a.lut = lut;
   a.ncls = ncls; a.rows = rows; a.cols = cols; a.rf = tdr_rec_floats(ncls); a.polar = polar; a.img = img; a.pk = pk;
diff --git a/top_down_renderer_amd/csrc/tdr_raster_dev.h b/top_down_renderer_amd/csrc/tdr_raster_dev.h
--- a/top_down_renderer_amd/csrc/tdr_raster_dev.h
+++ b/top_down_renderer_amd/csrc/tdr_raster_dev.h
@@ -54,14 +54,37 @@
 __device__ __forceinline__ void raster_tile_clear(unsigned int* cnt, int tile) {
   for (int t = threadIdx.x; t < tile; t += blockDim.x) cnt[t] = 0;
 }
+__device__ __forceinline__ void raster_tile_count_key(unsigned int* cnt, uint32_t key, int col0, int ncol, int ncls,
+                                                      int rows) {
+  const int col = (int)(key >> 20) - col0;
+  if (key == RASTER_NO_BIN || col < 0 || col >= ncol) return;
+  atomicAdd(&cnt[(col * ncls + (int)((key >> 16) & 15u)) * rows + (int)(key & 0xFFFFu)], 1u);
+}
+#define RASTER_KEY_VECS 4
 __device__ __forceinline__ void raster_tile_count_keys(unsigned int* cnt, const uint32_t* __restrict__ keys, int64_t n,
                                                        int col0, int ncol, int ncls, int rows) {
-  for (int64_t q = threadIdx.x; q < n; q += blockDim.x) {
-    const uint32_t key = keys[q];
-    const int col = (int)(key >> 20) - col0;
-    if (key == RASTER_NO_BIN || col < 0 || col >= ncol) continue;
-    atomicAdd(&cnt[(col * ncls + (int)((key >> 16) & 15u)) * rows + (int)(key & 0xFFFFu)], 1u);
+  const int64_t to16 = (int64_t)((4u - (unsigned)((reinterpret_cast<uintptr_t>(keys) >> 2) & 3u)) & 3u);
+  const int64_t head = to16 < n ? to16 : n;
+  const int64_t nv = (n - head) >> 2;
+  if ((int64_t)threadIdx.x < head) raster_tile_count_key(cnt, keys[threadIdx.x], col0, ncol, ncls, rows);
+  const uint4* __restrict__ kv = reinterpret_cast<const uint4*>(keys + head);
+  for (int64_t q = threadIdx.x; q < nv; q += (int64_t)RASTER_KEY_VECS * blockDim.x) {
+    uint4 v[RASTER_KEY_VECS];
+#pragma unroll
+    for (int u = 0; u < RASTER_KEY_VECS; u++) {
+      const int64_t qu = q + (int64_t)u * blockDim.x;
+      v[u] = qu < nv ? kv[qu] : make_uint4(RASTER_NO_BIN, RASTER_NO_BIN, RASTER_NO_BIN, RASTER_NO_BIN);
+    }
+#pragma unroll
+    for (int u = 0; u < RASTER_KEY_VECS; u++) {
+      raster_tile_count_key(cnt, v[u].x, col0, ncol, ncls, rows);
+      raster_tile_count_key(cnt, v[u].y, col0, ncol, ncls, rows);
+      raster_tile_count_key(cnt, v[u].z, col0, ncol, ncls, rows);
+      raster_tile_count_key(cnt, v[u].w, col0, ncol, ncls, rows);
+    }
   }
+  const int64_t tail = head + 4 * nv + threadIdx.x;
+  if (tail < n) raster_tile_count_key(cnt, keys[tail], col0, ncol, ncls, rows);
 }
 __device__ __forceinline__ void raster_tile_write(const unsigned int* cnt, int col0, int ncol, int ncls, int rows, int cols,
                                                   int rf, float* __restrict__ img, float* __restrict__ pk) {
@@ -98,15 +121,17 @@
   size_t lds;
   bool keyed;
 };
-static inline bool raster_shape(int ncls, int rows, int cols, RasterShape* out) {
+#define RASTER_KEYED_TILES 256
+static inline bool raster_shape(int ncls, int rows, int cols, bool with_keys, RasterShape* out) {
   const int64_t per_col = (int64_t)ncls * rows * 4;
   if (per_col > RASTER_MAX_LDS) return false;
+  out->keyed = cols <= RASTER_KEY_MAX_COLS && rows <= RASTER_KEY_MAX_ROWS;
   int cpt = (int)std::max<int64_t>(1, (64 * 1024) / per_col);
   cpt = std::min(cpt, cols);
-  while (cpt > 1 && cdiv(cols, cpt) < 32) cpt = (cpt + 1) / 2;
+  const int want = (with_keys && out->keyed) ? RASTER_KEYED_TILES : 32;
+  while (cpt > 1 && cdiv(cols, cpt) < want) cpt = (cpt + 1) / 2;
   out->cpt = cpt;
   out->lds = (size_t)cpt * per_col;
-  out->keyed = cols <= RASTER_KEY_MAX_COLS && rows <= RASTER_KEY_MAX_ROWS;
   return true;
 }
 static inline hipError_t raster_allow_lds(const void* kernel, size_t lds, bool* attr_set) {
diff --git a/top_down_renderer_amd/csrc/tdr_score.hip b/top_down_renderer_amd/csrc/tdr_score.hip
--- a/top_down_renderer_amd/csrc/tdr_score.hip
+++ b/top_down_renderer_amd/csrc/tdr_score.hip
@@ -569,14 +569,25 @@
   unsigned long long tot[TDR_MAX_CLASSES], norm = 0, known = 0;
 #pragma unroll
   for (int k = 0; k < TDR_MAX_CLASSES; k++) tot[k] = 0;
-  for (int c = t; c < nch; c += 4) {
-    const uint32_t* o = a.ipart + (int64_t)c * rows * a.npad + slot;
+  for (int c = t; c < nch; c += 8) {
+    const bool two = c + 4 < nch;
+    const uint32_t* o0 = a.ipart + (int64_t)c * rows * a.npad + slot;
+    const uint32_t* o1 = a.ipart + (int64_t)(two ? c + 4 : c) * rows * a.npad + slot;
+    uint32_t v0[2 * TDR_MAX_CLASSES], v1[2 * TDR_MAX_CLASSES];
+#pragma unroll
+    for (int k = 0; k < 2 * TDR_MAX_CLASSES; k++)
+      if (k < 2 * a.ncls) { v0[k] = o0[(int64_t)k * a.npad]; v1[k] = o1[(int64_t)k * a.npad]; }
+    const uint32_t n0 = o0[(int64_t)(2 * a.ncls) * a.npad], k0 = o0[(int64_t)(2 * a.ncls + 1) * a.npad];
+    const uint32_t n1 = o1[(int64_t)(2 * a.ncls) * a.npad], k1 = o1[(int64_t)(2 * a.ncls + 1) * a.npad];
 #pragma unroll
     for (int k = 0; k < TDR_MAX_CLASSES; k++)
-      if (k < a.ncls)
-        tot[k] += (unsigned long long)o[(int64_t)(2 * k) * a.npad] | ((unsigned long long)o[(int64_t)(2 * k + 1) * a.npad] << 32);
-    norm += o[(int64_t)(2 * a.ncls) * a.npad];
-    known += o[(int64_t)(2 * a.ncls + 1) * a.npad];
+      if (k < a.ncls) {
+        tot[k] += (unsigned long long)v0[2 * k] | ((unsigned long long)v0[2 * k + 1] << 32);
+        if (two) tot[k] += (unsigned long long)v1[2 * k] | ((unsigned long long)v1[2 * k + 1] << 32);
+      }
+    norm += n0;
+    known += k0;
+    if (two) { norm += n1; known += k1; }
   }
   if (t > 0) {
 #pragma unroll
diff --git a/top_down_renderer_amd/kernels.py b/top_down_renderer_amd/kernels.py
--- a/top_down_renderer_amd/kernels.py
+++ b/top_down_renderer_amd/kernels.py
@@ -561,6 +561,14 @@
     def save_ml_state(self, info, st, n, out12, src_shard=0):
         cap = st.shape[1] if (st.dim() == 2 and src_shard == 0) else 0
         check(self.lib.tdr_k_save_ml_state(_ptr(info), _ptr(st), cap, src_shard, n, _ptr(out12), self.stream()))
+
+    def resample_gather(self, runmax, n, n_new, shift, i_begin, i_end, idx, src, dst, info, out12, src_shard=0):
+        on_dev = hasattr(shift, "data_ptr")
+        src_cap = src.shape[1] if (src.dim() == 2 and src_shard == 0) else 0
+        check(self.lib.tdr_k_resample_gather(_ptr(runmax), n, n_new, _ptr(shift) if on_dev else None,
+                                             C.c_float(0.0 if on_dev else shift), i_begin, i_end, _ptr(idx), _ptr(src),
+                                             src_cap, src_shard, _ptr(dst), dst.shape[1], _ptr(info), _ptr(out12),
+                                             self.stream()))
 
     def mean_cov(self, st, n, about=None):
         out = self.empty((4800,))
@@ -702,6 +710,7 @@
         return C.c_void_p(self.lib.tdr_rng_create(C.c_uint32(seed & 0xFFFFFFFF)))
 
     device_rng = True
+    fused_resample = True
 
     def rng_state_to_device(self, rng):
         words = np.zeros(640, np.uint32)
diff --git a/top_down_renderer_amd/particle_filter.py b/top_down_renderer_amd/particle_filter.py
--- a/top_down_renderer_amd/particle_filter.py
+++ b/top_down_renderer_amd/particle_filter.py
@@ -302,19 +302,27 @@
         i0 = comm.rank * nl_new
         if shift is None and self._rng_on_device:
             self._shift_dev = self._pipe.uniform()
-            k.resample_dev(self.runmax, n, n_new, self._shift_dev, i0, i0 + nl_new, self.idx)
+        elif shift is None:
+            shift = k.rng_uniform(self.gen_)
+        if not comm.active and getattr(k, "fused_resample", False):
+            if self._ml_buf is None:
+                self._ml_buf = k.zeros((12,))
+            k.resample_gather(self.runmax, n, n_new, self._shift_dev if shift is None else float(shift), i0, i0 + nl_new,
+                              self.idx, self.st, self.st_new, self.info, self._ml_buf)
+            self._ml_fields = self._ml_buf[:7]
         else:
             if shift is None:
-                shift = k.rng_uniform(self.gen_)
-            k.resample(self.runmax, n, n_new, float(shift), i0, i0 + nl_new, self.idx)
-        if comm.active:
-            if st_work is not None:
-                st_work.wait()
-            k.gather_states(sa, self.idx, nl_new, self.st_new, src_shard=nl)
-            self._save_ml_state(sa, nl)
-        else:
-            k.gather_states(self.st, self.idx, nl_new, self.st_new)
-            self._save_ml_state(None, nl)
+                k.resample_dev(self.runmax, n, n_new, self._shift_dev, i0, i0 + nl_new, self.idx)
+            else:
+                k.resample(self.runmax, n, n_new, float(shift), i0, i0 + nl_new, self.idx)
+            if comm.active:
+                if st_work is not None:
+                    st_work.wait()
+                k.gather_states(sa, self.idx, nl_new, self.st_new, src_shard=nl)
+                self._save_ml_state(sa, nl)
+            else:
+                k.gather_states(self.st, self.idx, nl_new, self.st_new)
+                self._save_ml_state(None, nl)
         self.st, self.st_new = self.st_new, self.st
         self.num_particles_ = n_new
         self.perm = None if n_new != n else self.perm
```

Measured after the change: 24.01 million (median of 6 runs). +2.0%, better.
